# BimberLab/nimble-aligner

Hardware: AMD Instinct MI355X
Metric: reads/sec aligned (whole job), counts bit-exact vs the CPU path (higher is better)
Workload: dtype u64

## Files before the change

include/nimble_hip.h:

```cpp
#ifndef NIMBLE_HIP_H
#define NIMBLE_HIP_H
#include <stdint.h>

#ifdef __cplusplus
extern "C" {
#endif

#define NIMBLE_ABI_VERSION 1

enum {
  NIMBLE_OK = 0,
  NIMBLE_E_INVALID = -1,
  NIMBLE_E_NO_DEVICE = -2,
  NIMBLE_E_HIP = -3,
  NIMBLE_E_NOMEM = -4,
  NIMBLE_E_OVERFLOW = -5,
  NIMBLE_E_INTERNAL = -6
};

enum {
  NIMBLE_R_SCORE_BELOW_THRESHOLD = 0,
  NIMBLE_R_DISCARDED_MULTIPLE_MATCH = 1,
  NIMBLE_R_DISCARDED_NONZERO_MISMATCH = 2,
  NIMBLE_R_NO_MATCH = 3,
  NIMBLE_R_NOT_MATCHING_PAIR = 6,
  NIMBLE_R_SHORT_READ = 8,
  NIMBLE_R_HIGH_ENTROPY = 10,
  NIMBLE_R_SUCCESSFUL_MATCH = 11,
  NIMBLE_R_ABOVE_MISMATCH_THRESHOLD = 14,
  NIMBLE_R_SKIPPED_ALIGN_DUE_TO_UNPAIRED_DUMMY = 15,
  NIMBLE_R_NONE = 16
};

#define NIMBLE_CLASS_NONE 0xFFFFFFFFu

typedef struct nimble_align_params {
  double score_percent;
  uint64_t score_threshold;
  uint32_t num_mismatches;
  uint32_t discard_nonzero_mismatch;
  uint32_t discard_multiple_matches;
  uint32_t require_valid_pair;
  uint32_t min_read_length;
  uint32_t reserved;
} nimble_align_params;

typedef struct nimble_index nimble_index;
typedef struct nimble_ctx nimble_ctx;

int nimble_abi_version(void);
const char *nimble_last_error(void);
int nimble_device_count(int *count);

int nimble_index_build(const uint8_t *seqs, const uint64_t *seq_off, uint32_t n_seqs, int device,
                       nimble_index **out);
void nimble_index_free(nimble_index *);
int nimble_index_stats(const nimble_index *, uint64_t stats[8]);
int nimble_class_get(const nimble_index *, uint32_t class_id, uint32_t *ids, uint32_t cap, uint32_t *len);
int nimble_class_table_read(const nimble_index *, uint32_t first, uint32_t count, uint32_t *len, uint32_t *pool_off);
int nimble_class_pool_read(const nimble_index *, uint32_t pool_off, uint32_t count, uint32_t *ids);

int nimble_flat_index_stats(const uint8_t *seqs, const uint64_t *seq_off, uint32_t n_seqs, uint64_t stats[5]);
int nimble_flat_index_selfcheck(const uint8_t *seqs, const uint64_t *seq_off, uint32_t n_seqs, uint64_t *n_records);

int nimble_ctx_create(nimble_index *, void *stream, nimble_ctx **out);
void nimble_ctx_free(nimble_ctx *);
void *nimble_ctx_stream(nimble_ctx *);

enum {
  NIMBLE_OPT_COUNTERS = 1,
  NIMBLE_OPT_ALIGN_GRID_PCT = 2,
  NIMBLE_OPT_TAIL_ASIDE = 3
};
int nimble_ctx_set_option(nimble_ctx *, int option, int64_t value);

enum { NIMBLE_MEM_HOST = 0, NIMBLE_MEM_DEVICE = 1, NIMBLE_MEM_HOST_PINNED = 2 };

int nimble_call(nimble_ctx *, const nimble_align_params *, const uint8_t *r1, const uint64_t *r1_off,
                const uint8_t *r2, const uint64_t *r2_off, uint64_t n, uint32_t fixed_len, uint32_t max_len,
                int mem);

int nimble_call_words(nimble_ctx *, const nimble_align_params *, const uint64_t *r1_words, const uint32_t *r1_len,
                      uint32_t r1_stride, const uint64_t *r2_words, const uint32_t *r2_len, uint32_t r2_stride, uint64_t n,
                      uint32_t max_len, int mem);

typedef struct nimble_call_extra {
  const uint32_t *segment;
  uint32_t n_segments;
  uint32_t reserved;
  const uint8_t *qual[2];
  double trim_strictness;
  uint64_t trim_target_length;
  const uint8_t *skip[2];
} nimble_call_extra;
int nimble_call_ex(nimble_ctx *, const nimble_align_params *, const uint8_t *r1, const uint64_t *r1_off,
                   const uint8_t *r2, const uint64_t *r2_off, uint64_t n, uint32_t fixed_len, uint32_t max_len,
                   int mem, const nimble_call_extra *extra);
int nimble_histogram_seg(nimble_ctx *, uint32_t *segment, uint32_t *class_r1, uint32_t *class_r2, uint64_t *count,
                         uint32_t *representative, uint64_t cap, uint64_t *n_entries);
int nimble_read_align_len(nimble_ctx *, int mate, uint32_t *align_len, uint64_t n);

typedef struct nimble_packed {
  uint64_t *keys;
  uint32_t *len[2];
  uint64_t *hash;
  uint8_t *pre[2];
  uint32_t key_words;
  uint32_t paired;
} nimble_packed;
uint32_t nimble_key_words(uint32_t max_len, int paired);
int nimble_pack(nimble_ctx *, const nimble_align_params *, const uint8_t *r1, const uint64_t *r1_off,
                const uint8_t *r2, const uint64_t *r2_off, uint64_t n, uint32_t fixed_len, uint32_t max_len, int mem,
                const nimble_packed *out);
int nimble_call_packed(nimble_ctx *, const nimble_align_params *, const nimble_packed *in, uint64_t n,
                       uint32_t max_len);
int nimble_route_records(nimble_ctx *, const nimble_packed *in, uint64_t n, uint32_t world, uint64_t *records,
                         uint64_t *counts);
int nimble_unpack_records(nimble_ctx *, const uint64_t *records, uint64_t n, const nimble_packed *out);
int nimble_call_records(nimble_ctx *, const nimble_align_params *, const uint64_t *records, uint64_t n,
                        uint32_t max_len, int paired);

int nimble_ctx_defer_dedup(nimble_ctx *, uint32_t world, uint64_t *records, uint32_t *perm);
int nimble_route_counts(nimble_ctx *, uint64_t *counts);
int nimble_dedup_records(nimble_ctx *, const uint64_t *records, uint64_t n, uint32_t key_words, uint8_t *verdict);
int nimble_count_verdicts(nimble_ctx *, const uint8_t *verdict);

int nimble_stream_begin(nimble_ctx *, const nimble_align_params *, int paired, uint32_t max_len,
                        uint64_t capacity_hint);
int nimble_stream_append(nimble_ctx *, const uint8_t *r1, const uint64_t *r1_off, const uint8_t *r2,
                         const uint64_t *r2_off, uint64_t n, uint32_t fixed_len, int mem);
int nimble_stream_append_packed(nimble_ctx *, const uint64_t *r1_words, const uint32_t *r1_len, uint32_t r1_stride,
                                const uint64_t *r2_words, const uint32_t *r2_len, uint32_t r2_stride, uint64_t m);
int nimble_stream_end(nimble_ctx *);
int nimble_pinned_alloc(uint64_t bytes, void **out);
void nimble_pinned_free(void *);
int nimble_pinned_register(void *p, uint64_t bytes);
void nimble_pinned_unregister(void *p);

int nimble_histogram(nimble_ctx *, uint32_t *class_r1, uint32_t *class_r2, uint64_t *count, uint64_t cap,
                     uint64_t *n_entries);

int nimble_read_records(nimble_ctx *, int mate, int32_t *reason, int32_t *score, int32_t *mism, uint32_t *cls,
                        uint8_t *counted, uint64_t n);

int nimble_call_counters(nimble_ctx *, uint64_t c[8]);

int nimble_call_timing(nimble_ctx *, float ms[6]);
int nimble_ctx_synchronize(nimble_ctx *);

int nimble_histogram_dense_se(nimble_ctx *, int64_t *counts_dev, uint32_t n_classes);

typedef struct nimble_comm nimble_comm;
int nimble_comm_create(const int *devices, int n, nimble_comm **out);
void nimble_comm_free(nimble_comm *);
int nimble_comm_size(const nimble_comm *);
int nimble_comm_uses_rccl(const nimble_comm *);
void nimble_comm_abort(nimble_comm *);
int nimble_counts_allreduce(nimble_comm *, int rank, int64_t *counts_dev, uint64_t len, void *stream);
int nimble_counts_allreduce_host(nimble_comm *, int rank, int64_t *counts, uint64_t len);
int nimble_records_alltoall(nimble_comm *, int rank, const uint64_t *send, const uint64_t *send_counts,
                            uint32_t rec_words, uint64_t *recv, uint64_t recv_cap, uint64_t *n_recv, void *stream);
int nimble_sharded_begin(nimble_comm *, int rank, nimble_ctx *, const nimble_align_params *, int paired,
                         uint32_t max_len);
int nimble_sharded_append(nimble_comm *, int rank, const uint8_t *r1, const uint64_t *r1_off, const uint8_t *r2,
                          const uint64_t *r2_off, uint64_t n, uint32_t fixed_len, int mem);
int nimble_sharded_append_packed(nimble_comm *, int rank, const uint64_t *r1_words, const uint32_t *r1_len, uint32_t r1_stride,
                                 const uint64_t *r2_words, const uint32_t *r2_len, uint32_t r2_stride, uint64_t n);
int nimble_sharded_end(nimble_comm *, int rank, uint64_t *n_owned);
int nimble_sharded_grow(nimble_comm *, int rank, uint32_t max_len);
int nimble_sharded_abort(nimble_comm *, int rank);
int nimble_steps_begin(nimble_comm *, int rank, nimble_ctx *call0, nimble_ctx *call1, nimble_ctx *util,
                       const nimble_align_params *, int paired, uint32_t max_len);
int nimble_steps_submit(nimble_comm *, int rank, const uint8_t *r1, const uint64_t *r1_off, const uint8_t *r2,
                        const uint64_t *r2_off, uint64_t n, uint32_t fixed_len, int mem, nimble_ctx **launched);
int nimble_steps_flush(nimble_comm *, int rank, nimble_ctx **launched);
int nimble_steps_end(nimble_comm *, int rank);

#ifdef __cplusplus
}
#endif
#endif
```

nimble-aligner_amd/__init__.py:

```python
import ctypes as C
import os

import numpy as np

_HERE = os.path.dirname(os.path.abspath(__file__))
LIB_DIR = os.environ.get("NIMBLE_LIB_DIR") or os.path.join(_HERE, "lib")
HIP_LIB_PATH = os.environ.get("NIMBLE_HIP_LIB") or os.path.join(LIB_DIR, "libnimble_hip.so")
HOST_LIB_PATH = os.path.join(LIB_DIR, "libnimble_host.so")

CLASS_NONE = 0xFFFFFFFF
OPT_COUNTERS, OPT_ALIGN_GRID_PCT, OPT_TAIL_ASIDE = 1, 2, 3
MEM_HOST, MEM_DEVICE = 0, 1

REASONS = {
    0: "ScoreBelowThreshold", 1: "DiscardedMultipleMatch", 2: "DiscardedNonzeroMismatch", 3: "NoMatch",
    6: "NotMatchingPair", 8: "ShortRead", 10: "HighEntropy", 11: "SuccessfulMatch", 14: "AboveMismatchThreshold",
    16: "None",
}


class NimbleError(RuntimeError):
    def __init__(self, code, msg):
        super().__init__("nimble error %d: %s" % (code, msg))
        self.code = code


class AlignParams(C.Structure):
    _fields_ = [
        ("score_percent", C.c_double),
        ("score_threshold", C.c_uint64),
        ("num_mismatches", C.c_uint32),
        ("discard_nonzero_mismatch", C.c_uint32),
        ("discard_multiple_matches", C.c_uint32),
        ("require_valid_pair", C.c_uint32),
        ("min_read_length", C.c_uint32),
        ("reserved", C.c_uint32),
    ]

    @classmethod
    def make(cls, score_percent, score_threshold, num_mismatches=0, discard_nonzero_mismatch=False,
             discard_multiple_matches=False, require_valid_pair=False, min_read_length=40):
        return cls(float(score_percent), int(score_threshold), int(num_mismatches), int(discard_nonzero_mismatch),
                   int(discard_multiple_matches), int(require_valid_pair), int(min_read_length), 0)


class NimblePacked(C.Structure):
    _fields_ = [
        ("keys", C.c_void_p), ("len", C.c_void_p * 2), ("hash", C.c_void_p), ("pre", C.c_void_p * 2),
        ("key_words", C.c_uint32), ("paired", C.c_uint32),
    ]


class CallExtra(C.Structure):
    _fields_ = [("segment", C.c_void_p), ("n_segments", C.c_uint32), ("reserved", C.c_uint32),
                ("qual", C.c_void_p * 2), ("trim_strictness", C.c_double), ("trim_target_length", C.c_uint64),
                ("skip", C.c_void_p * 2)]


class UmiExtra(C.Structure):
    _fields_ = [("segment", C.c_void_p), ("n_segments", C.c_uint32), ("reserved", C.c_uint32),
                ("qual", C.c_void_p * 2), ("skip", C.c_void_p * 2)]


_hip = None

HIP_SYMBOLS = [
    "nimble_abi_version", "nimble_last_error", "nimble_device_count", "nimble_index_build", "nimble_index_free",
    "nimble_index_stats", "nimble_class_get", "nimble_ctx_create", "nimble_ctx_free", "nimble_ctx_synchronize",
    "nimble_call", "nimble_histogram", "nimble_histogram_dense_se", "nimble_read_records", "nimble_call_counters",
    "nimble_call_timing", "nimble_flat_index_stats", "nimble_flat_index_selfcheck", "nimble_ctx_set_option", "nimble_key_words", "nimble_pack",
    "nimble_call_packed", "nimble_call_words", "nimble_ctx_stream", "nimble_stream_begin", "nimble_stream_append", "nimble_stream_append_packed", "nimble_stream_end",
    "nimble_pinned_alloc", "nimble_pinned_free", "nimble_call_ex", "nimble_histogram_seg", "nimble_read_align_len",
    "nimble_route_records", "nimble_unpack_records", "nimble_pinned_register", "nimble_pinned_unregister",
    "nimble_ctx_defer_dedup", "nimble_route_counts", "nimble_dedup_records", "nimble_count_verdicts",
    "nimble_call_records", "nimble_comm_create", "nimble_comm_free", "nimble_comm_size", "nimble_comm_uses_rccl", "nimble_comm_abort",
    "nimble_counts_allreduce", "nimble_counts_allreduce_host", "nimble_records_alltoall", "nimble_sharded_begin",
    "nimble_sharded_append", "nimble_sharded_append_packed", "nimble_sharded_end", "nimble_sharded_grow", "nimble_sharded_abort",
    "nimble_class_table_read", "nimble_class_pool_read", "nimble_steps_begin", "nimble_steps_submit", "nimble_steps_flush", "nimble_steps_end",
]


def hip_lib():
    global _hip
    if _hip is None:
        if not os.path.exists(HIP_LIB_PATH):
            raise ImportError("nimble-aligner_amd: %s is missing; run `python -c 'import __graft_entry__ as g; "
                              "g.build()'` (needs hipcc)" % HIP_LIB_PATH)
        L = C.CDLL(HIP_LIB_PATH)
        vp, i32, u32, u64 = C.c_void_p, C.c_int, C.c_uint32, C.c_uint64
        L.nimble_abi_version.restype = i32
        L.nimble_last_error.restype = C.c_char_p
        L.nimble_device_count.argtypes = [C.POINTER(i32)]
        L.nimble_index_build.argtypes = [vp, vp, u32, i32, C.POINTER(vp)]
        L.nimble_index_free.argtypes = [vp]
        L.nimble_index_free.restype = None
        L.nimble_flat_index_stats.argtypes = [vp, vp, u32, C.POINTER(u64)]
        L.nimble_flat_index_selfcheck.argtypes = [vp, vp, u32, C.POINTER(u64)]
        L.nimble_index_stats.argtypes = [vp, C.POINTER(u64)]
        L.nimble_class_get.argtypes = [vp, u32, vp, u32, C.POINTER(u32)]
        L.nimble_ctx_create.argtypes = [vp, vp, C.POINTER(vp)]
        L.nimble_ctx_free.argtypes = [vp]
        L.nimble_ctx_free.restype = None
        L.nimble_ctx_synchronize.argtypes = [vp]
        L.nimble_ctx_set_option.argtypes = [vp, i32, C.c_int64]
        L.nimble_call.argtypes = [vp, C.POINTER(AlignParams), vp, vp, vp, vp, u64, u32, u32, i32]
        L.nimble_histogram.argtypes = [vp, vp, vp, vp, u64, C.POINTER(u64)]
        L.nimble_histogram_dense_se.argtypes = [vp, vp, u32]
        L.nimble_read_records.argtypes = [vp, i32, vp, vp, vp, vp, vp, u64]
        L.nimble_call_counters.argtypes = [vp, C.POINTER(u64)]
        L.nimble_call_timing.argtypes = [vp, C.POINTER(C.c_float)]
        L.nimble_key_words.argtypes = [u32, i32]
        L.nimble_key_words.restype = u32
        L.nimble_pack.argtypes = [vp, C.POINTER(AlignParams), vp, vp, vp, vp, u64, u32, u32, i32, C.POINTER(NimblePacked)]
        L.nimble_call_packed.argtypes = [vp, C.POINTER(AlignParams), C.POINTER(NimblePacked), u64, u32]
        L.nimble_stream_begin.argtypes = [vp, C.POINTER(AlignParams), i32, u32, u64]
        L.nimble_stream_append.argtypes = [vp, vp, vp, vp, vp, u64, u32, i32]
        L.nimble_stream_append_packed.argtypes = [vp, vp, vp, u32, vp, vp, u32, u64]
        L.nimble_call_words.argtypes = [vp, vp, vp, vp, u32, vp, vp, u32, u64, u32, i32]
        L.nimble_stream_end.argtypes = [vp]
        L.nimble_pinned_alloc.argtypes = [u64, C.POINTER(vp)]
        L.nimble_pinned_free.argtypes = [vp]
        L.nimble_pinned_free.restype = None
        L.nimble_pinned_register.argtypes = [vp, u64]
        L.nimble_pinned_unregister.argtypes = [vp]
        L.nimble_pinned_unregister.restype = None
        L.nimble_call_ex.argtypes = [vp, C.POINTER(AlignParams), vp, vp, vp, vp, u64, u32, u32, i32, C.POINTER(CallExtra)]
        L.nimble_histogram_seg.argtypes = [vp, vp, vp, vp, vp, vp, u64, C.POINTER(u64)]
        L.nimble_read_align_len.argtypes = [vp, i32, vp, u64]
        L.nimble_route_records.argtypes = [vp, C.POINTER(NimblePacked), u64, u32, vp, vp]
        L.nimble_unpack_records.argtypes = [vp, vp, u64, C.POINTER(NimblePacked)]
        L.nimble_ctx_defer_dedup.argtypes = [vp, u32, vp, vp]
        L.nimble_route_counts.argtypes = [vp, vp]
        L.nimble_dedup_records.argtypes = [vp, vp, u64, u32, vp]
        L.nimble_count_verdicts.argtypes = [vp, vp]
        L.nimble_call_records.argtypes = [vp, C.POINTER(AlignParams), vp, u64, u32, i32]
        L.nimble_ctx_stream.argtypes = [vp]
        L.nimble_ctx_stream.restype = vp
        L.nimble_comm_create.argtypes = [C.POINTER(i32), i32, C.POINTER(vp)]
        L.nimble_comm_free.argtypes = [vp]
        L.nimble_comm_free.restype = None
        L.nimble_comm_size.argtypes = [vp]
        L.nimble_comm_uses_rccl.argtypes = [vp]
        L.nimble_comm_abort.argtypes = [vp]
        L.nimble_comm_abort.restype = None
        L.nimble_counts_allreduce.argtypes = [vp, i32, vp, u64, vp]
        L.nimble_counts_allreduce_host.argtypes = [vp, i32, vp, u64]
        L.nimble_records_alltoall.argtypes = [vp, i32, vp, vp, u32, vp, u64, C.POINTER(u64), vp]
        L.nimble_sharded_begin.argtypes = [vp, i32, vp, C.POINTER(AlignParams), i32, u32]
        L.nimble_sharded_append.argtypes = [vp, i32, vp, vp, vp, vp, u64, u32, i32]
        L.nimble_sharded_append_packed.argtypes = [vp, i32, vp, vp, u32, vp, vp, u32, u64]
        L.nimble_sharded_end.argtypes = [vp, i32, C.POINTER(u64)]
        L.nimble_sharded_grow.argtypes = [vp, i32, u32]
        L.nimble_steps_begin.argtypes = [vp, i32, vp, vp, vp, C.POINTER(AlignParams), i32, u32]
        L.nimble_steps_submit.argtypes = [vp, i32, vp, vp, vp, vp, u64, u32, i32, C.POINTER(vp)]
        L.nimble_steps_flush.argtypes = [vp, i32, C.POINTER(vp)]
        L.nimble_steps_end.argtypes = [vp, i32]
        L.nimble_sharded_abort.argtypes = [vp, i32]
        _hip = L
    return _hip


def _check(rc):
    if rc != 0:
        raise NimbleError(rc, hip_lib().nimble_last_error().decode("utf-8", "replace"))


def device_count():
    n = C.c_int(0)
    rc = hip_lib().nimble_device_count(C.byref(n))
    return n.value if rc == 0 else 0


def pack_reads(reads):
    bs = [r.encode() if isinstance(r, str) else bytes(r) for r in reads]
    off = np.zeros(len(bs) + 1, dtype=np.uint64)
    if bs:
        off[1:] = np.cumsum([len(b) for b in bs], dtype=np.uint64)
    buf = np.frombuffer(b"".join(bs), dtype=np.uint8).copy() if bs else np.zeros(0, dtype=np.uint8)
    return buf, off


def _ptr(x):
    if x is None:
        return None
    if isinstance(x, int):
        return x
    if isinstance(x, np.ndarray):
        return x.ctypes.data
    if hasattr(x, "data_ptr"):
        return x.data_ptr()
    raise TypeError(type(x))


def _off(x):
    if x is None or isinstance(x, int):
        return x
    size = x.dtype.itemsize if isinstance(x, np.ndarray) else (x.element_size() if hasattr(x, "element_size") else 8)
    if size != 8:
        raise TypeError("read offsets must be 64-bit integers (n + 1 of them); got elements of %d bytes -- are the mates in "
                        "the place of the offsets?" % size)
    return _ptr(x)


def key_words(max_len, paired):
    return int(hip_lib().nimble_key_words(int(max_len), int(bool(paired))))


def flat_index_stats(sequences):
    buf, off = pack_reads(sequences)
    s = (C.c_uint64 * 5)()
    _check(hip_lib().nimble_flat_index_stats(buf.ctypes.data, off.ctypes.data, len(sequences), s))
    return dict(kmers=s[0], nodes=s[1], classes=s[2], unitig_bases=s[3], class_entries=s[4])


def flat_index_selfcheck(sequences):
    buf, off = pack_reads(sequences)
    n = C.c_uint64()
    _check(hip_lib().nimble_flat_index_selfcheck(buf.ctypes.data, off.ctypes.data, len(sequences), C.byref(n)))
    return int(n.value)


class Index:

    def __init__(self, sequences, device=0):
        buf, off = pack_reads(sequences)
        h = C.c_void_p()
        _check(hip_lib().nimble_index_build(buf.ctypes.data, off.ctypes.data, len(sequences), device, C.byref(h)))
        self.h = h
        self.device = device
        self._class_cache = {}

    def close(self):
        if getattr(self, "h", None):
            hip_lib().nimble_index_free(self.h)
            self.h = None

    def __del__(self):
        try:
            self.close()
        except Exception:
            pass

    def stats(self):
        s = (C.c_uint64 * 8)()
        _check(hip_lib().nimble_index_stats(self.h, s))
        return dict(kmers=s[0], nodes=s[1], classes=s[2], unitig_bases=s[3], class_entries=s[4], hash_slots=s[5],
                    device_bytes=s[6], dynamic_classes=s[7])

    def eq_class(self, class_id):
        class_id = int(class_id)
        got = self._class_cache.get(class_id)
        if got is None:
            n = C.c_uint32(0)
            _check(hip_lib().nimble_class_get(self.h, class_id, None, 0, C.byref(n)))
            a = np.zeros(max(n.value, 1), dtype=np.uint32)
            _check(hip_lib().nimble_class_get(self.h, class_id, a.ctypes.data, n.value, C.byref(n)))
            got = a[:n.value].tolist()
            self._class_cache[class_id] = got
        return got


class Context:

# ... 35 lines not shown
        self._keep = (r1, r1_off, r2, r2_off)
        _check(hip_lib().nimble_call(self.h, C.byref(params), _ptr(r1), _off(r1_off), _ptr(r2), _off(r2_off), n,
                                     fixed_len, max_len, mem))
        self.n = n

    def call_ex(self, params, r1, r1_off=None, r2=None, r2_off=None, n=None, fixed_len=0, max_len=0, mem=MEM_HOST,
                segment=None, n_segments=0, qual=(None, None), skip=(None, None), trim_strictness=0.0,
                trim_target_length=0):
        if r1_off is not None:
            n = int(len(r1_off) - 1) if n is None else n
        if max_len == 0:
            if r1_off is not None and isinstance(r1_off, np.ndarray):
                max_len = int(np.diff(r1_off.astype(np.int64)).max()) if n else 1
                if r2_off is not None:
                    max_len = max(max_len, int(np.diff(r2_off.astype(np.int64)).max()) if n else 1)
            else:
                max_len = fixed_len
        ex = CallExtra()
        ex.segment = _ptr(segment)
        ex.n_segments = n_segments
        for m in range(2):
            ex.qual[m] = _ptr(qual[m])
            ex.skip[m] = _ptr(skip[m])
        ex.trim_strictness = trim_strictness
        ex.trim_target_length = trim_target_length
        self._keep = (r1, r1_off, r2, r2_off, segment, qual, skip)
        _check(hip_lib().nimble_call_ex(self.h, C.byref(params), _ptr(r1), _off(r1_off), _ptr(r2), _off(r2_off), n,
                                        fixed_len, max_len, mem, C.byref(ex)))
        self.n = n

    def histogram_seg(self):
        ne = C.c_uint64()
        _check(hip_lib().nimble_histogram_seg(self.h, None, None, None, None, None, 0, C.byref(ne)))
        k = ne.value
        sg, c1, c2 = (np.zeros(max(k, 1), dtype=np.uint32) for _ in range(3))
        cnt = np.zeros(max(k, 1), dtype=np.uint64)
        rep = np.zeros(max(k, 1), dtype=np.uint32)
        if k:
            _check(hip_lib().nimble_histogram_seg(self.h, sg.ctypes.data, c1.ctypes.data, c2.ctypes.data,
                                                  cnt.ctypes.data, rep.ctypes.data, k, C.byref(ne)))
        return [(int(sg[i]), int(c1[i]), int(c2[i]), int(cnt[i]), int(rep[i])) for i in range(k)]

    def read_align_len(self, mate=0):
        out = np.zeros(max(self.n, 1), dtype=np.uint32)
        _check(hip_lib().nimble_read_align_len(self.h, mate, out.ctypes.data, self.n))
        return out[:self.n]

    def stream_begin(self, params, paired, max_len, capacity_hint=0):
        _check(hip_lib().nimble_stream_begin(self.h, C.byref(params), int(bool(paired)), max_len, capacity_hint))
        self.n = 0

    def stream_append(self, r1, r1_off=None, r2=None, r2_off=None, n=None, fixed_len=0, mem=MEM_HOST):
        if r1_off is not None and n is None:
            n = int(len(r1_off) - 1)
        self._keep = (r1, r1_off, r2, r2_off)
        _check(hip_lib().nimble_stream_append(self.h, _ptr(r1), _off(r1_off), _ptr(r2), _off(r2_off), n, fixed_len,
                                              mem))
        self.n += n

    def call_words(self, params, w1, len1, stride1, w2=None, len2=None, stride2=0, n=None, max_len=0, mem=MEM_HOST):
        if n is None:
            n = int(len(len1))
        self._keep = (w1, len1, w2, len2)
        _check(hip_lib().nimble_call_words(self.h, C.byref(params), _ptr(w1), _ptr(len1), stride1, _ptr(w2), _ptr(len2),
                                           stride2, n, max(max_len, 1), mem))
        self.n = n

    def stream_append_packed(self, w1, len1, stride1, w2=None, len2=None, stride2=0):
        n = int(len(len1))
        self._keep_packed = getattr(self, "_keep_packed", []) + [(w1, len1, w2, len2)]
        _check(hip_lib().nimble_stream_append_packed(self.h, _ptr(w1), _ptr(len1), stride1, _ptr(w2), _ptr(len2), stride2, n))
        self.n += n

    def stream_end(self):
        _check(hip_lib().nimble_stream_end(self.h))
        self._keep_packed = []

    def call_reads(self, params, reads, mates=None):
        b1, o1 = pack_reads(reads)
        if mates is not None:
            b2, o2 = pack_reads(mates)
            return self.call(params, b1, o1, b2, o2)
        return self.call(params, b1, o1)

    def synchronize(self):
        _check(hip_lib().nimble_ctx_synchronize(self.h))

    def set_option(self, option, value):
        _check(hip_lib().nimble_ctx_set_option(self.h, option, int(value)))

    def stream_ptr(self):
        return int(hip_lib().nimble_ctx_stream(self.h) or 0)

    def defer_dedup(self, world, records, perm):
        if not world:
            _check(hip_lib().nimble_ctx_defer_dedup(self.h, 0, None, None))
            return
        assert records.is_contiguous() and perm.is_contiguous() and perm.element_size() == 4
        self._defer_keep = (records, perm)
        _check(hip_lib().nimble_ctx_defer_dedup(self.h, world, C.c_void_p(records.data_ptr()),
                                                C.c_void_p(perm.data_ptr())))

    def route_counts(self, world):
        counts = np.zeros(256, dtype=np.uint64)
        _check(hip_lib().nimble_route_counts(self.h, counts.ctypes.data))
        return [int(c) for c in counts[:world]]

    def dedup_records(self, records, key_words, verdict):
        n = int(records.shape[0])
        assert records.is_contiguous() and verdict.is_contiguous() and verdict.numel() >= n
        assert n == 0 or records.shape[1] == key_words + 2
        self._dedup_keep = (records, verdict)
        _check(hip_lib().nimble_dedup_records(self.h, C.c_void_p(records.data_ptr()), n, key_words,
                                              C.c_void_p(verdict.data_ptr())))

    def count_verdicts(self, verdict):
        self._verdict_keep = verdict
        _check(hip_lib().nimble_count_verdicts(self.h, C.c_void_p(verdict.data_ptr())))

    def set_counters(self, on):
        _check(hip_lib().nimble_ctx_set_option(self.h, 1, int(bool(on))))

    def histogram(self):
        ne = C.c_uint64(0)
        _check(hip_lib().nimble_histogram(self.h, None, None, None, 0, C.byref(ne)))
        k = ne.value
        c1 = np.zeros(max(k, 1), dtype=np.uint32)
        c2 = np.zeros(max(k, 1), dtype=np.uint32)
        cnt = np.zeros(max(k, 1), dtype=np.uint64)
        if k:
            _check(hip_lib().nimble_histogram(self.h, c1.ctypes.data, c2.ctypes.data, cnt.ctypes.data, k,
                                              C.byref(ne)))
        return [(int(c1[i]), int(c2[i]), int(cnt[i])) for i in range(k)]

    def histogram_dense_se(self, counts_dev_ptr, n_classes):
        _check(hip_lib().nimble_histogram_dense_se(self.h, _ptr(counts_dev_ptr), n_classes))

    def read_records(self, mate=0):
        n = self.n
        reason = np.zeros(max(n, 1), dtype=np.int32)
        score = np.zeros(max(n, 1), dtype=np.int32)
        mism = np.zeros(max(n, 1), dtype=np.int32)
        cls = np.zeros(max(n, 1), dtype=np.uint32)
        counted = np.zeros(max(n, 1), dtype=np.uint8)
        _check(hip_lib().nimble_read_records(self.h, mate, reason.ctypes.data, score.ctypes.data, mism.ctypes.data,
                                             cls.ctypes.data, counted.ctypes.data, n))
        return dict(reason=reason[:n], score=score[:n], mismatches=mism[:n], cls=cls[:n], counted=counted[:n])

    def counters(self):
        c = (C.c_uint64 * 8)()
        _check(hip_lib().nimble_call_counters(self.h, c))
        return dict(reads=c[0], unique_keys=c[1], probes=c[2], nodes=c[3], class_entries=c[4], seeded=c[5],
                    prefiltered=c[6], dynamic_classes=c[7])

    def timing(self):
        t = (C.c_float * 6)()
        _check(hip_lib().nimble_call_timing(self.h, t))
        return dict(pack=t[0], align=t[1], intern=t[2], dedup=t[3], count=t[4], total=t[5])


CHEM = {"unstranded": 0, "fiveprime": 1, "threeprime": 2, "none": 3}

HOST_SYMBOLS = [
    "nimble_host_last_error", "nimble_library_load", "nimble_library_parse", "nimble_library_free",
    "nimble_library_get_config", "nimble_library_set_config", "nimble_library_n_rows", "nimble_library_n_cols",
    "nimble_library_group_on", "nimble_library_set_group_on", "nimble_library_sequence_name_idx",
    "nimble_library_sequence_idx", "nimble_library_header", "nimble_library_cell", "nimble_library_push_column", "nimble_library_from_table",
    "nimble_library_build_index", "nimble_library_index", "nimble_library_ctx", "nimble_score_call",
    "nimble_score_call_fastq", "nimble_rows_free", "nimble_rows_count", "nimble_rows_get", "nimble_fastq_process",
    "nimble_write_to_tsv", "nimble_multi_steps", "nimble_host_coerce", "nimble_host_parse_calls", "nimble_host_unmap", "nimble_host_feature_list",
    "nimble_host_reference_sequence_data", "nimble_host_sort_score_vector", "nimble_host_natural_lexical_cmp", "nimble_host_shannon_entropy",
    "nimble_host_revcomp", "nimble_host_maxinfo", "nimble_host_read_fastq", "nimble_host_filter_reason_text",
    "nimble_library_pack", "nimble_score_call_packed", "nimble_score_call_begin", "nimble_score_call_begin_words", "nimble_score_call_end",
    "nimble_library_ctx_slot", "nimble_library_pack_slot", "nimble_score_call_packed_begin",
    "nimble_score_call_records_begin", "nimble_rows_signature", "nimble_rows_counts", "nimble_host_read_fastq_batched", "nimble_host_read_fastq_packed", "nimble_score_call_umis", "nimble_umi_rows_free",
    "nimble_umi_rows_count", "nimble_umi_rows_get", "nimble_umi_rows_reads", "nimble_umi_rows_filter", "nimble_score_stream_begin", "nimble_score_stream_append", "nimble_score_stream_end",
    "nimble_fastq_process_sharded", "nimble_bam_process", "nimble_host_bam_dump", "nimble_host_pack_reads_2bit", "nimble_host_reverse_comp_if_needed",
    "nimble_host_parse_str_as_bool", "nimble_host_pgzip_decompress",
]


class HostConfig(C.Structure):
    _fields_ = [
        ("reference_genome_size", C.c_uint64), ("score_percent", C.c_double), ("score_threshold", C.c_uint64),
        ("num_mismatches", C.c_uint64), ("discard_nonzero_mismatch", C.c_int32),
        ("discard_multiple_matches", C.c_int32), ("score_filter", C.c_int32), ("intersect_level", C.c_int32),
        ("require_valid_pair", C.c_int32), ("strand_filter", C.c_int32), ("discard_multi_hits", C.c_uint64),
        ("max_hits_to_report", C.c_uint64), ("trim_strictness", C.c_double), ("trim_target_length", C.c_uint64),
    ]


_host = None


def host_lib():
    global _host
    if _host is None:
        if not os.path.exists(HOST_LIB_PATH):
            raise ImportError("nimble-aligner_amd: %s is missing; run __graft_entry__.build()" % HOST_LIB_PATH)
        hip_lib()
        L = C.CDLL(HOST_LIB_PATH)
        vp, i32, u32, u64, cp = C.c_void_p, C.c_int, C.c_uint32, C.c_uint64, C.c_char_p
        pp = C.POINTER(C.c_char_p)
        L.nimble_host_last_error.restype = cp
        L.nimble_library_load.argtypes = [cp, i32, C.POINTER(vp)]
        L.nimble_library_parse.argtypes = [cp, i32, C.POINTER(vp)]
        L.nimble_library_free.argtypes = [vp]
        L.nimble_library_free.restype = None
        L.nimble_library_get_config.argtypes = [vp, C.POINTER(HostConfig)]
        L.nimble_library_set_config.argtypes = [vp, C.POINTER(HostConfig)]
        for f in ("n_rows", "n_cols", "group_on", "sequence_name_idx", "sequence_idx"):
            getattr(L, "nimble_library_" + f).argtypes = [vp]
        L.nimble_library_set_group_on.argtypes = [vp, i32]
        L.nimble_library_set_group_on.restype = None
        L.nimble_library_header.argtypes = [vp, i32]
        L.nimble_library_header.restype = cp
        L.nimble_library_cell.argtypes = [vp, i32, i32]
        L.nimble_library_cell.restype = cp
        L.nimble_library_push_column.argtypes = [vp, cp, pp, i32]
        L.nimble_library_from_table.argtypes = [i32, pp, vp, pp, i32, i32, i32, C.POINTER(vp)]
        L.nimble_library_build_index.argtypes = [vp, i32]
        L.nimble_library_index.argtypes = [vp]
        L.nimble_library_index.restype = vp
        L.nimble_library_ctx.argtypes = [vp]
        L.nimble_library_ctx.restype = vp
        L.nimble_score_call.argtypes = [vp, vp, vp, vp, vp, u64, u32, u32, i32, C.POINTER(vp)]
        L.nimble_score_call_fastq.argtypes = [vp, cp, cp, C.POINTER(vp)]
        L.nimble_score_call_begin.argtypes = [vp, i32, vp, vp, vp, vp, u64, u32, u32, i32]
        L.nimble_score_call_begin_words.argtypes = [vp, i32, vp, vp, u32, vp, vp, u32, u64, u32, i32]
        L.nimble_score_call_end.argtypes = [vp, i32, C.POINTER(vp)]
        L.nimble_library_ctx_slot.argtypes = [vp, i32]
        L.nimble_score_stream_begin.argtypes = [vp, i32, u32, u64]
        L.nimble_library_pack_slot.argtypes = [vp, i32, vp, vp, vp, vp, u64, u32, u32, i32, C.POINTER(NimblePacked)]
        L.nimble_score_call_packed_begin.argtypes = [vp, i32, C.POINTER(NimblePacked), u64, u32]
        L.nimble_score_call_records_begin.argtypes = [vp, i32, vp, u64, u32, i32]
        L.nimble_rows_signature.argtypes = [vp]
        L.nimble_rows_signature.restype = u64
        L.nimble_rows_counts.argtypes = [vp, vp]
        L.nimble_rows_counts.restype = None
        L.nimble_score_call_umis.argtypes = [vp, vp, vp, vp, vp, u64, u32, u32, i32, C.POINTER(UmiExtra), i32,
                                             C.POINTER(vp)]
        L.nimble_umi_rows_free.argtypes = [vp]
        L.nimble_umi_rows_free.restype = None
        L.nimble_umi_rows_count.argtypes = [vp]
        L.nimble_umi_rows_count.restype = u64
        L.nimble_umi_rows_get.argtypes = [vp, u64, C.POINTER(u32), C.POINTER(i32), C.POINTER(u32)]
        L.nimble_umi_rows_get.restype = cp
        L.nimble_umi_rows_reads.argtypes = [vp]
        L.nimble_umi_rows_reads.restype = u64
        L.nimble_umi_rows_filter.argtypes = [vp, u64, C.POINTER(i32 * 5)]
        L.nimble_host_read_fastq_batched.argtypes = [cp, u64, C.POINTER(u64), C.POINTER(u64), C.POINTER(u32),
                                                     C.POINTER(u64), C.POINTER(u64)]
        L.nimble_host_read_fastq_packed.argtypes = [cp, u64, C.POINTER(u64), C.POINTER(u64), C.POINTER(u32),
                                                     C.POINTER(u64), C.POINTER(u64)]
        L.nimble_score_stream_append.argtypes = [vp, vp, vp, vp, vp, u64, u32, i32]
        L.nimble_score_stream_end.argtypes = [vp, C.POINTER(vp)]
        L.nimble_library_ctx_slot.restype = vp
        L.nimble_library_pack.argtypes = [vp, vp, vp, vp, vp, u64, u32, u32, i32, C.POINTER(NimblePacked)]
        L.nimble_score_call_packed.argtypes = [vp, C.POINTER(NimblePacked), u64, u32, C.POINTER(vp)]
        L.nimble_rows_free.argtypes = [vp]
        L.nimble_rows_free.restype = None
        L.nimble_rows_count.argtypes = [vp]
        L.nimble_rows_count.restype = u64
        L.nimble_rows_get.argtypes = [vp, u64, C.POINTER(C.c_int32)]
        L.nimble_rows_get.restype = cp
        L.nimble_fastq_process.argtypes = [i32, pp, i32, C.POINTER(vp), pp]
        L.nimble_fastq_process_sharded.argtypes = [i32, pp, vp, C.POINTER(i32), i32, cp]
        L.nimble_multi_steps.argtypes = [C.POINTER(vp), C.POINTER(i32), i32, C.POINTER(vp), C.POINTER(vp), i32, C.c_uint64,
                                         C.c_uint32, i32, i32, i32, C.POINTER(C.c_double), C.POINTER(i32), C.POINTER(vp)]
        L.nimble_bam_process.argtypes = [cp, i32, C.POINTER(vp), pp, i32, i32]
        L.nimble_host_bam_dump.argtypes = [cp, i32, cp]
        L.nimble_host_reverse_comp_if_needed.argtypes = [cp, i32, cp, u64]
        L.nimble_host_pack_reads_2bit.argtypes = [vp, vp, u64, u32, vp, vp]
        L.nimble_host_parse_str_as_bool.argtypes = [cp, C.POINTER(i32)]
        L.nimble_host_pgzip_decompress.argtypes = [cp, i32, cp, C.POINTER(u64)]
        L.nimble_write_to_tsv.argtypes = [vp, cp]
        L.nimble_host_coerce.argtypes = [vp, i32, vp, i32, i32, vp, i32, cp, i32]
        L.nimble_host_parse_calls.argtypes = [vp, cp, cp, i32]
        L.nimble_host_unmap.argtypes = [vp, cp, vp, i32]
        L.nimble_host_feature_list.argtypes = [vp, vp, i32, i32, cp, i32]
        L.nimble_host_reference_sequence_data.argtypes = [vp, cp, i32]
        L.nimble_host_sort_score_vector.argtypes = [cp, i32, vp]
        L.nimble_host_natural_lexical_cmp.argtypes = [cp, cp]
        L.nimble_host_shannon_entropy.argtypes = [cp]
        L.nimble_host_shannon_entropy.restype = C.c_double
        L.nimble_host_revcomp.argtypes = [cp, cp]
        L.nimble_host_maxinfo.argtypes = [cp, i32, u64, C.c_double]
        L.nimble_host_maxinfo.restype = u64
        L.nimble_host_read_fastq.argtypes = [cp, C.POINTER(u64), C.POINTER(u64), C.POINTER(u32)]
        L.nimble_host_filter_reason_text.argtypes = [i32]
        L.nimble_host_filter_reason_text.restype = cp
        _host = L
    return _host


class Panic(RuntimeError):
    """A Rust panic of the reference, surfaced with its message."""


def _hcheck(rc):
    if rc != 0:
        raise Panic(host_lib().nimble_host_last_error().decode("utf-8", "replace"))


def _cstrs(seq):
    arr = (C.c_char_p * len(seq))()
# ... 535 lines not shown
```

nimble-aligner_amd/csrc/capi.cpp:

```cpp
#include <hip/hip_runtime_api.h>
#include <rccl/rccl.h>

#include <algorithm>
#include <condition_variable>
#include <cmath>
#include <cstdlib>
#include <cstring>
#include <mutex>
#include <new>
#include <stdexcept>
#include <string>
#include <vector>

#include "flat_index.h"
#include "kernels.h"

using namespace nimble;

namespace {

thread_local std::string g_err;

int fail(int code, const std::string &msg) {
  g_err = msg;
// ... 1 lines not shown
}

#define HIPCHK(expr)                                                                                   \
  do {                                                                                                 \
    hipError_t e_ = (expr);                                                                            \
    if (e_ != hipSuccess)                                                                              \
      return fail(NIMBLE_E_HIP, std::string(#expr) + ": " + hipGetErrorString(e_));                    \
  } while (0)

#define DRAIN_STALE_HIP_ERROR() (void)hipGetLastError()

uint64_t env_u64(const char *name, uint64_t dflt) {
  const char *v = getenv(name);
  if (!v || !*v) return dflt;
  return strtoull(v, nullptr, 10);
}

uint64_t pow2_at_least(uint64_t x) {
  uint64_t p = 1;
  while (p < x) p <<= 1;
  return p;
}

struct DevBuf {
  void *p = nullptr;
  size_t cap = 0;
  int ensure(size_t bytes, uint64_t *total) {
    if (bytes <= cap) return NIMBLE_OK;
    if (p) {
      (void)hipFree(p);
      if (total) *total -= cap;
      p = nullptr;
      cap = 0;
    }
    size_t want = bytes + 64;
    hipError_t e = hipMalloc(&p, want);
    if (e != hipSuccess) return fail(NIMBLE_E_NOMEM, std::string("hipMalloc failed: ") + hipGetErrorString(e));
    cap = bytes;
    if (total) *total += cap;
    return NIMBLE_OK;
  }
  void release() {
    if (p) (void)hipFree(p);
    p = nullptr;
    cap = 0;
  }
  template <class T>
  T *as() const { return reinterpret_cast<T *>(p); }
};

}

struct nimble_index {
  int device = 0;
  hipStream_t copy_stream = nullptr;
  int n_ctx = 0;
  std::mutex intern_mu;
  hipEvent_t ev_intern = nullptr;
  bool intern_chained = false;
  hipStream_t intern_last = nullptr;
  bool released = false;
  DevIndex dev{};
  DevBuf b_ht, b_bitmap, b_l1, b_mleft, b_rec, b_ledge, b_unitig, b_cls_desc, b_cls_off, b_cls_ids, b_cls_bits, b_intern, b_dyn_state,
      b_srec, b_srec_first, b_srec_base, b_srec_many;
  uint64_t device_bytes = 0;
  uint64_t n_kmers = 0, n_nodes = 0, n_static = 0, unitig_bases = 0, static_entries = 0, ht_slots = 0;
  std::vector<uint32_t> h_col_off, h_col_ids;
  ~nimble_index() {
    if (copy_stream) (void)hipStreamDestroy(copy_stream);
    if (ev_intern) (void)hipEventDestroy(ev_intern);
    for (DevBuf *b : {&b_ht, &b_bitmap, &b_l1, &b_mleft, &b_rec, &b_ledge, &b_unitig, &b_cls_desc, &b_cls_off, &b_cls_ids, &b_cls_bits, &b_intern,
                      &b_dyn_state, &b_srec, &b_srec_first, &b_srec_base, &b_srec_many})
      b->release();
  }
};

struct nimble_ctx {
  nimble_index *ix = nullptr;
  hipStream_t stream = nullptr;
  bool own_stream = false;
  hipStream_t copy_stream = nullptr;
  uint64_t *p_state = nullptr;
  uint32_t *p_dyn = nullptr;
  CallBuffers cb{};
  uint64_t bytes = 0;
  bool streaming = false;
  uint64_t stream_n = 0, stream_cap = 0;
  uint32_t stream_max_len = 0;
  hipStream_t h2d_stream = nullptr;
  DevBuf b_stage[2][2], b_stage_off[2][2];
  hipEvent_t ev_h2d[2] = {}, ev_used[2] = {};
  bool stage_busy[2] = {false, false};
  int stage_k = 0;
  uint64_t align_from = 0;
  bool h2d_pending[2] = {false, false};
  DevBuf b_keys, b_len[2], b_hash, b_pre[2], b_reason[2], b_score[2], b_mism[2], b_cls[2], b_dyn_off[2], b_dyn_len[2],
      b_dyn_hash[2], b_dyn_pos[2], b_slot, b_counted, b_scratch, b_ws, b_dedup, b_hist_keys, b_hist_cnt, b_state;
  DevBuf b_tile_ctr;
  DevBuf b_in[2], b_in_off[2];
  DevBuf b_plog;
  uint32_t plog_max_len = 0;
  DevBuf b_min_cov;
  double min_cov_percent = -1.0;
  uint32_t min_cov_len = 0;
  DevBuf b_out_c1, b_out_c2, b_out_cnt, b_out_seg, b_out_rep;
  struct HostOut {
    void *base = nullptr;
    uint64_t cap = 0;
    uint32_t *c1 = nullptr, *c2 = nullptr, *seg = nullptr, *rep = nullptr;
    uint64_t *cnt = nullptr;
  } hout;
  bool out_pinned = false;
  bool tail_aside = false;
  uint32_t tail_aside_grid = 0;
  DevBuf b_route;
  struct Defer {
    uint32_t world = 0;
    uint32_t world_of_call = 0;
    uint32_t counts_world = 0;
    uint64_t *records = nullptr;
    uint32_t *perm = nullptr;
    const uint8_t *verdict = nullptr;
    bool active = false;
    bool routed = false;
    bool counted = false;
    hipEvent_t ev_route = nullptr;
    uint64_t *p_counts = nullptr;
  } defer;
  DevBuf b_seg, b_alen[2], b_skip[2], b_qual[2], b_trim_ls, b_trim_qp, b_hist_rep, b_hot;
  double trim_strictness = -1.0;
  uint64_t trim_target = ~0ULL;
  std::vector<uint32_t> h_seg, h_rep;
  uint64_t scratch_cap = 0;
  uint64_t hist_slots = 0;
  hipEvent_t ev[7] = {};
  bool have_events = false;
  bool called = false;
  int want_counters = 0;
  int align_grid_pct = 100;
  int stream_cus = 0;
  uint32_t dyn_before = 0, dyn_after = 0;
  nimble_align_params prm{};
  const uint8_t *in_r[2] = {nullptr, nullptr};
  const uint64_t *in_off[2] = {nullptr, nullptr};
  uint32_t in_fixed_len = 0, in_max_len = 0;
  const uint64_t *in_words[2] = {nullptr, nullptr};
  const uint32_t *in_len32[2] = {nullptr, nullptr};
  uint32_t in_stride[2] = {0, 0};
  uint64_t dslots = 0;
  uint64_t dedup_clean_slots = 0;
  bool finished = true;
  bool skip_pack = false;
  bool counted_marked = true;
  int attempt = 0;
  std::vector<uint64_t> h_state = std::vector<uint64_t>(16, 0);
  std::vector<uint32_t> h_c1, h_c2;
  std::vector<uint64_t> h_cnt;
  ~nimble_ctx() {
    for (DevBuf *b : {&b_keys, &b_len[0], &b_len[1], &b_hash, &b_pre[0], &b_pre[1], &b_reason[0], &b_reason[1],
                      &b_score[0], &b_score[1], &b_mism[0], &b_mism[1], &b_cls[0], &b_cls[1], &b_dyn_off[0],
                      &b_dyn_off[1], &b_dyn_len[0], &b_dyn_len[1], &b_dyn_hash[0], &b_dyn_hash[1], &b_dyn_pos[0],
                      &b_dyn_pos[1], &b_slot, &b_counted, &b_scratch, &b_ws, &b_dedup, &b_hist_keys, &b_hist_cnt,
                      &b_state, &b_tile_ctr, &b_in[0], &b_in[1], &b_in_off[0], &b_in_off[1], &b_plog, &b_min_cov, &b_out_c1, &b_out_c2,
                      &b_out_cnt, &b_out_seg, &b_out_rep, &b_seg, &b_alen[0], &b_alen[1], &b_skip[0], &b_skip[1], &b_qual[0],
                      &b_qual[1], &b_route, &b_trim_ls, &b_trim_qp, &b_hist_rep, &b_hot, &b_stage[0][0], &b_stage[0][1], &b_stage[1][0], &b_stage[1][1], &b_stage_off[0][0],
                      &b_stage_off[0][1], &b_stage_off[1][0], &b_stage_off[1][1]})
      b->release();
    if (h2d_stream) {
      (void)hipStreamDestroy(h2d_stream);
      for (int k = 0; k < 2; ++k) {
        (void)hipEventDestroy(ev_h2d[k]);
        (void)hipEventDestroy(ev_used[k]);
      }
    }
    if (have_events)
      for (auto &e : ev) (void)hipEventDestroy(e);
    if (own_stream && stream) (void)hipStreamDestroy(stream);
    if (p_state) (void)hipHostFree(p_state);
    if (hout.base) (void)hipHostFree(hout.base);
    if (p_dyn) (void)hipHostFree(p_dyn);
    if (defer.ev_route) (void)hipEventDestroy(defer.ev_route);
    if (defer.p_counts) (void)hipHostFree(defer.p_counts);
  }
};

namespace {

template <class T>
int upload(DevBuf &b, const std::vector<T> &v, uint64_t *total, size_t min_elems = 0) {
  size_t n = std::max(v.size(), min_elems);
  int rc = b.ensure(std::max<size_t>(n * sizeof(T), 16), total);
  if (rc) return rc;
  if (!v.empty()) HIPCHK(hipMemcpy(b.p, v.data(), v.size() * sizeof(T), hipMemcpyHostToDevice));
  return NIMBLE_OK;
}

int ensure_plog(nimble_ctx *c, uint32_t max_len) {
  if (c->b_plog.p && c->plog_max_len >= max_len) return NIMBLE_OK;
  uint32_t m = std::max<uint32_t>(max_len, 256);
  std::vector<double> t(((size_t)m + 1) * (m + 2) / 2, 0.0);
  for (uint32_t L = 1; L <= m; ++L) {
    double *row = t.data() + ((size_t)L * (L + 1)) / 2;
    for (uint32_t k = 1; k <= L; ++k) {
      double f = (double)k / (double)L;
      row[k] = f * std::log2(f);
    }
  }
  int rc = upload(c->b_plog, t, &c->bytes);
  if (rc) return rc;
  c->plog_max_len = m;
  return NIMBLE_OK;
}

int ensure_trim_tables(nimble_ctx *c, uint64_t target_length, double strictness) {
  if (c->b_trim_ls.p && c->trim_target == target_length && c->trim_strictness == strictness) return NIMBLE_OK;
  const size_t LONGEST_READ = 1000, MAXQUAL = 60;
  std::vector<double> ls(LONGEST_READ), qp(MAXQUAL + 1);
  for (size_t i = 0; i < LONGEST_READ; ++i) {
    const double pow1 = std::exp((double)target_length - (double)i - 1.0);
    ls[i] = std::log(1.0 / (1.0 + pow1)) + std::log((double)(i + 1)) * (1.0 - strictness);
  }
  for (size_t i = 0; i <= MAXQUAL; ++i)
    qp[i] = std::log(1.0 - std::pow(10.0, -((0.5 + (double)i) / 10.0))) * strictness;
  auto norm_ratio = [](const std::vector<double> &a, size_t margin) {
    double mx = std::fabs(a[0]);
    for (size_t i = 1; i < a.size(); ++i) mx = std::max(mx, std::fabs(a[i]));
    return (double)INT64_MAX / (mx * (double)margin);
  };
  auto as_i64 = [](double v) -> int64_t {
    if (std::isnan(v)) return 0;
    if (v >= 9223372036854775807.0) return INT64_MAX;
    if (v <= -9223372036854775808.0) return INT64_MIN;
    return (int64_t)v;
  };
  const double ratio = std::max(norm_ratio(ls, LONGEST_READ * 2), norm_ratio(qp, LONGEST_READ * 2));
  std::vector<int64_t> lsi(LONGEST_READ), qpi(MAXQUAL + 1);
  for (size_t i = 0; i < LONGEST_READ; ++i) lsi[i] = as_i64(ls[i] * ratio);
  for (size_t i = 0; i <= MAXQUAL; ++i) qpi[i] = as_i64(qp[i] * ratio);
  int rc = upload(c->b_trim_ls, lsi, &c->bytes);
  if (!rc) rc = upload(c->b_trim_qp, qpi, &c->bytes);
  if (rc) return rc;
  c->trim_target = target_length;
  c->trim_strictness = strictness;
  return NIMBLE_OK;
}

int ensure_min_cov(nimble_ctx *c, double percent, uint32_t max_len) {
  if (c->b_min_cov.p && c->min_cov_percent == percent && c->min_cov_len >= max_len) return NIMBLE_OK;
  uint32_t m = std::max<uint32_t>(max_len, 256);
  std::vector<uint32_t> t(m + 1, 0xFFFFFFFFu);
  for (uint32_t L = 1; L <= m; ++L) {
    uint32_t lo = 0, hi = 4 * L + 1;
    while (lo < hi) {
      uint32_t mid = lo + (hi - lo) / 2;
      if ((double)mid / (double)L >= percent) hi = mid;
      else lo = mid + 1;
    }
    t[L] = lo <= 4 * L ? lo : 0xFFFFFFFFu;
  }
  t[0] = percent <= 0.0 ? 0u : 0xFFFFFFFFu;
  int rc = upload(c->b_min_cov, t, &c->bytes);
  if (rc) return rc;
  c->min_cov_percent = percent;
  c->min_cov_len = m;
  return NIMBLE_OK;
}

int mark_done(nimble_ctx *c, hipStream_t on = nullptr) {
  hipStream_t s = on ? on : c->stream;
  launch_publish_state(s, c->b_state.as<uint64_t>(), c->p_state);
  HIPCHK(hipGetLastError());
  HIPCHK(hipEventRecord(c->ev[6], s));
  return NIMBLE_OK;
}

int fetch_state(nimble_ctx *c) {
  HIPCHK(hipEventSynchronize(c->ev[6]));
  std::copy(c->p_state, c->p_state + 16, c->h_state.begin());
  return NIMBLE_OK;
}

int ensure_host_out(nimble_ctx *c, uint64_t cap) {
  if (c->hout.cap >= cap) return NIMBLE_OK;
  HIPCHK(hipStreamSynchronize(c->stream));
  if (c->copy_stream) HIPCHK(hipStreamSynchronize(c->copy_stream));
  if (c->hout.base) (void)hipHostFree(c->hout.base);
  c->hout = nimble_ctx::HostOut();
  void *p = nullptr;
  if (hipHostMalloc(&p, cap * 24, hipHostMallocDefault) != hipSuccess)
    return fail(NIMBLE_E_NOMEM, "page-locked result buffer");
  c->hout.base = p;
  c->hout.cap = cap;
  c->hout.cnt = static_cast<uint64_t *>(p);
  c->hout.c1 = reinterpret_cast<uint32_t *>(c->hout.cnt + cap);
  c->hout.c2 = c->hout.c1 + cap;
  c->hout.seg = c->hout.c2 + cap;
  c->hout.rep = c->hout.seg + cap;
  return NIMBLE_OK;
}

int enqueue_compact(nimble_ctx *c, hipStream_t on = nullptr) {
  hipStream_t st = on ? on : c->stream;
  const uint64_t slots = c->hist_slots;
  c->out_pinned = slots <= (1ULL << 22);
  HIPCHK(hipMemsetAsync((uint64_t *)c->b_state.p + 11, 0, 8, st));
  if (c->out_pinned) {
    int rc = ensure_host_out(c, slots);
    if (rc) return rc;
    launch_hist_compact(st, c->cb, c->hout.c1, c->hout.c2, c->hout.cnt, slots, c->hout.seg, c->hout.rep);
    return NIMBLE_OK;
  }
  int rc = c->b_out_c1.ensure(slots * 4, &c->bytes);
  if (!rc) rc = c->b_out_c2.ensure(slots * 4, &c->bytes);
  if (!rc) rc = c->b_out_cnt.ensure(slots * 8, &c->bytes);
  if (!rc) rc = c->b_out_seg.ensure(slots * 4, &c->bytes);
  if (!rc) rc = c->b_out_rep.ensure(slots * 4, &c->bytes);
  if (rc) return rc;
  launch_hist_compact(st, c->cb, c->b_out_c1.as<uint32_t>(), c->b_out_c2.as<uint32_t>(),
                      c->b_out_cnt.as<uint64_t>(), slots, c->b_out_seg.as<uint32_t>(), c->b_out_rep.as<uint32_t>());
  return NIMBLE_OK;
}

int enqueue_count_verdicts(nimble_ctx *c) {
  hipStream_t s = c->stream;
  launch_count_verdicts(s, c->prm, c->cb, c->defer.perm, c->defer.verdict);
  HIPCHK(hipEventRecord(c->ev[4], s));
  HIPCHK(hipEventRecord(c->ev[5], s));
  c->counted_marked = true;
  int rc = enqueue_compact(c);
  if (rc) return rc;
  HIPCHK(hipGetLastError());
  return mark_done(c);
}

int enqueue_route(nimble_ctx *c) {
  const uint32_t world = c->defer.world_of_call;
  const uint64_t cells = (uint64_t)route_grid() * world;
  uint64_t *block_first = c->b_route.as<uint64_t>();
  uint64_t *totals = block_first + cells;
  uint32_t *block_counts = reinterpret_cast<uint32_t *>(totals + 256);
  launch_route(c->stream, c->cb, world, block_counts, block_first, totals, c->defer.records, c->defer.perm);
  HIPCHK(hipGetLastError());
  HIPCHK(hipMemcpyAsync(c->defer.p_counts, totals, world * 8, hipMemcpyDeviceToHost, c->stream));
  HIPCHK(hipMemcpyAsync(c->defer.p_counts + 256, (uint64_t *)c->b_state.p + 14, 8, hipMemcpyDeviceToHost, c->stream));
  HIPCHK(hipEventRecord(c->defer.ev_route, c->stream));
  c->defer.counts_world = world;
  c->defer.routed = true;
  return NIMBLE_OK;
}

int enqueue_intern_round(nimble_ctx *c, int round, hipStream_t on = nullptr) {
  nimble_index *ix = c->ix;
  hipStream_t s = on ? on : c->stream;
  std::lock_guard<std::mutex> lock(ix->intern_mu);
  if (!ix->ev_intern) HIPCHK(hipEventCreateWithFlags(&ix->ev_intern, hipEventDisableTiming));
  if (ix->intern_chained) HIPCHK(hipStreamWaitEvent(s, ix->ev_intern, 0));
  launch_intern_claim(s, ix->dev, c->cb, round);
  launch_intern_verify(s, ix->dev, c->cb);
  HIPCHK(hipEventRecord(ix->ev_intern, s));
  ix->intern_chained = true;
  ix->intern_last = s;
  return NIMBLE_OK;
}

int enqueue_head(nimble_ctx *c) {
  hipStream_t s = c->stream;
  CallBuffers &cb = c->cb;
  if (c->tail_aside) {
    HIPCHK(hipStreamWaitEvent(s, c->ev[6], 0));
    c->tail_aside = false;
  }
  if (c->dedup_clean_slots < c->dslots) HIPCHK(hipMemsetAsync(c->b_dedup.p, 0, c->dslots * 8, s));
  c->dedup_clean_slots = c->defer.active ? c->dslots : 0;
  launch_clear_call(s, cb, !c->skip_pack);
  HIPCHK(hipGetLastError());
  HIPCHK(hipEventRecord(c->ev[0], s));
  return NIMBLE_OK;
}

int enqueue_tail(nimble_ctx *c) {
  hipStream_t s = c->stream;
  CallBuffers &cb = c->cb;
  HIPCHK(hipEventRecord(c->ev[2], s));
  {
    int rc = enqueue_intern_round(c, 0);
    if (rc) return rc;
  }
  HIPCHK(hipEventRecord(c->ev[3], s));
  if (c->defer.active) {
    HIPCHK(hipGetLastError());
    return c->defer.counted ? enqueue_count_verdicts(c) : mark_done(c);
  }
  const uint32_t aside_grid = c->tail_aside_grid;
  hipStream_t t = s;
  c->tail_aside = aside_grid != 0 && c->ix->n_ctx > 1 && !c->streaming && c->copy_stream != nullptr;
  if (c->tail_aside) {
    t = c->copy_stream;
    HIPCHK(hipStreamWaitEvent(t, c->ev[3], 0));
  }
  launch_dedup(t, c->prm, cb, c->tail_aside ? aside_grid : 0u);
  HIPCHK(hipEventRecord(c->ev[4], t));
  if (!cb.fuse_count) launch_count(t, cb);
  c->counted_marked = !cb.fuse_count;
  HIPCHK(hipEventRecord(c->ev[5], t));
  int rc = enqueue_compact(c, t);
  if (rc) return rc;
  HIPCHK(hipGetLastError());
  return mark_done(c, t);
}

int enqueue_call(nimble_ctx *c) {
  hipStream_t s = c->stream;
  CallBuffers &cb = c->cb;
  int rc = enqueue_head(c);
  if (rc) return rc;
  if (!c->skip_pack) {
    if (c->in_words[0])
      launch_pack_words(s, c->in_words[0], c->in_len32[0], c->in_stride[0], c->in_words[1], c->in_len32[1], c->in_stride[1],
                        c->in_max_len, c->prm.min_read_length, c->b_plog.as<double>(), cb);
    else
      launch_pack(s, c->in_r[0], c->in_off[0], c->in_r[1], c->in_off[1], c->in_fixed_len, c->in_max_len,
                  c->prm.min_read_length, c->b_plog.as<double>(), c->plog_max_len, cb);
  }
  HIPCHK(hipEventRecord(c->ev[1], s));
  if (c->defer.active && !c->defer.routed) {
    rc = enqueue_route(c);
    if (rc) return rc;
  }
  launch_align(s, c->ix->dev, c->prm, cb, c->want_counters, c->align_grid_pct, c->stream_cus);
  return enqueue_tail(c);
}

int redo_dedup_count(nimble_ctx *c) {
  hipStream_t s = c->stream;
  if (c->cb.hot) HIPCHK(hipMemsetAsync(c->cb.hot, 0, (size_t)HOT_KEYS * 8, s));
  HIPCHK(hipMemsetAsync(c->b_dedup.p, 0, c->dslots * 8, s));
  HIPCHK(hipMemsetAsync(c->b_hist_keys.p, 0xFF, c->hist_slots * 8, s));
  HIPCHK(hipMemsetAsync(c->b_hist_cnt.p, 0, c->hist_slots * 8, s));
  if (c->cb.hist_rep) HIPCHK(hipMemsetAsync(c->cb.hist_rep, 0, c->hist_slots * 4, s));
  HIPCHK(hipMemsetAsync((uint64_t *)c->b_state.p + 10, 0, 8, s));
  HIPCHK(hipEventRecord(c->ev[3], s));
  if (c->defer.active) return enqueue_count_verdicts(c);
  launch_dedup(s, c->prm, c->cb);
  HIPCHK(hipEventRecord(c->ev[4], s));
  if (!c->cb.fuse_count) launch_count(s, c->cb);
  c->counted_marked = !c->cb.fuse_count;
  HIPCHK(hipEventRecord(c->ev[5], s));
  int rc = enqueue_compact(c);
  return rc ? rc : mark_done(c);
}

int finish_call(nimble_ctx *c) {
  if (c->finished) return NIMBLE_OK;
  if (c->defer.active && !c->defer.counted)
    return fail(NIMBLE_E_INVALID, "the call defers its dedup: nimble_count_verdicts has not been called yet");
  for (;;) {
    int rc = fetch_state(c);
    if (rc) return rc;
    const uint64_t err = c->h_state[10];
    if (c->h_state[14] != 0) {
      HIPCHK(hipMemsetAsync((uint64_t *)c->b_state.p + 14, 0, 8, c->stream));
      HIPCHK(hipStreamSynchronize(c->stream));
      c->finished = true;
      c->h_c1.clear();
      c->h_c2.clear();
      c->h_cnt.clear();
      c->h_seg.clear();
      c->h_rep.clear();
      return fail(NIMBLE_E_INVALID, "offsets not monotone or a read longer than max_len (found on the device)");
    }
    if (err & ERR_SCRATCH) {
      if (c->attempt >= 3 || c->scratch_cap >= 0xFFFFFF00ULL)
        return fail(NIMBLE_E_OVERFLOW, "class scratch pool overflow (raise NIMBLE_SCRATCH_PER_READ)");
      c->attempt++;
      c->scratch_cap = std::min<uint64_t>(c->scratch_cap * 4, 0xFFFFFF00ULL);
      rc = c->b_scratch.ensure(c->scratch_cap * 4, &c->bytes);
      if (rc) return rc;
      c->cb.scratch = c->b_scratch.as<uint32_t>();
      c->cb.scratch_cap = (uint32_t)c->scratch_cap;
      rc = enqueue_call(c);
      if (rc) return rc;
      continue;
    }
    if (err & ERR_CLASS_CAP) return fail(NIMBLE_E_OVERFLOW, "dynamic class table full (raise NIMBLE_DYN_CLASSES)");
    if (err & ERR_IDS_CAP) return fail(NIMBLE_E_OVERFLOW, "dynamic class id pool full (raise NIMBLE_DYN_IDS)");
    if (c->h_state[9] != 0) {
      for (int round = 1; c->h_state[9] != 0; ++round) {
        if (round > 64) return fail(NIMBLE_E_INTERNAL, "class interning did not converge");
        HIPCHK(hipMemsetAsync((uint64_t *)c->b_state.p + 9, 0, 8, c->stream));
        rc = enqueue_intern_round(c, round);
        if (!rc) rc = mark_done(c);
        if (!rc) rc = fetch_state(c);
        if (rc) return rc;
        if (c->h_state[10] & (ERR_CLASS_CAP | ERR_IDS_CAP))
          return fail(NIMBLE_E_OVERFLOW, "dynamic class table full (raise NIMBLE_DYN_CLASSES / NIMBLE_DYN_IDS)");
      }
      rc = redo_dedup_count(c);
      if (rc) return rc;
      continue;
    }
    if (err & ERR_HIST) {
      if (c->hist_slots >= (1ULL << 30)) return fail(NIMBLE_E_OVERFLOW, "histogram table overflow");
      c->hist_slots *= 16;
      rc = c->b_hist_keys.ensure(c->hist_slots * 8, &c->bytes);
      if (!rc) rc = c->b_hist_cnt.ensure(c->hist_slots * 8, &c->bytes);
      if (rc) return rc;
      c->cb.hist_keys = c->b_hist_keys.as<uint64_t>();
      c->cb.hist_cnt = c->b_hist_cnt.as<uint64_t>();
      c->cb.hist_mask = c->hist_slots - 1;
      if (c->cb.hist_rep) {
        rc = c->b_hist_rep.ensure(c->hist_slots * 4, &c->bytes);
        if (rc) return rc;
        c->cb.hist_rep = c->b_hist_rep.as<uint32_t>();
      }
      rc = redo_dedup_count(c);
      if (rc) return rc;
      continue;
    }
    break;
  }
  {
    const uint64_t ne = c->h_state[11];
    c->h_c1.resize(ne);
    c->h_c2.resize(ne);
    c->h_cnt.resize(ne);
    c->h_seg.resize(ne);
    c->h_rep.resize(ne);
    if (ne) {
      std::vector<uint32_t> a(ne), b(ne), sg(ne), rp(ne);
      std::vector<uint64_t> k(ne);
      if (c->out_pinned) {
        std::copy(c->hout.c1, c->hout.c1 + ne, a.begin());
        std::copy(c->hout.c2, c->hout.c2 + ne, b.begin());
        std::copy(c->hout.cnt, c->hout.cnt + ne, k.begin());
        std::copy(c->hout.seg, c->hout.seg + ne, sg.begin());
        std::copy(c->hout.rep, c->hout.rep + ne, rp.begin());
      } else {
        HIPCHK(hipMemcpyAsync(a.data(), c->b_out_c1.p, ne * 4, hipMemcpyDeviceToHost, c->copy_stream));
        HIPCHK(hipMemcpyAsync(b.data(), c->b_out_c2.p, ne * 4, hipMemcpyDeviceToHost, c->copy_stream));
        HIPCHK(hipMemcpyAsync(k.data(), c->b_out_cnt.p, ne * 8, hipMemcpyDeviceToHost, c->copy_stream));
        HIPCHK(hipMemcpyAsync(sg.data(), c->b_out_seg.p, ne * 4, hipMemcpyDeviceToHost, c->copy_stream));
        HIPCHK(hipMemcpyAsync(rp.data(), c->b_out_rep.p, ne * 4, hipMemcpyDeviceToHost, c->copy_stream));
        HIPCHK(hipStreamSynchronize(c->copy_stream));
      }
      std::vector<uint32_t> idx(ne), tmp(ne);
      for (uint64_t i = 0; i < ne; ++i) idx[i] = (uint32_t)i;
      const std::vector<uint32_t> *cols[3] = {&b, &a, &sg};
      std::vector<uint32_t> hist(65536);
      for (int col = 0; col < 3; ++col) {
        const std::vector<uint32_t> &v = *cols[col];
        for (int shift = 0; shift < 32; shift += 16) {
          std::fill(hist.begin(), hist.end(), 0u);
          for (uint64_t i = 0; i < ne; ++i) hist[(v[i] >> shift) & 0xFFFFu]++;
          if (hist[(v[0] >> shift) & 0xFFFFu] == ne) continue;
          uint32_t run = 0;
          for (uint32_t d = 0; d < 65536; ++d) {
            const uint32_t c0 = hist[d];
            hist[d] = run;
            run += c0;
          }
          for (uint64_t i = 0; i < ne; ++i) tmp[hist[(v[idx[i]] >> shift) & 0xFFFFu]++] = idx[i];
          idx.swap(tmp);
        }
      }
      for (uint64_t i = 0; i < ne; ++i) {
        c->h_c1[i] = a[idx[i]];
        c->h_c2[i] = b[idx[i]];
        c->h_cnt[i] = k[idx[i]];
        c->h_seg[i] = sg[idx[i]];
        c->h_rep[i] = rp[idx[i]];
      }
    }
  }
  c->dyn_before = c->p_dyn[0];
  c->finished = true;
  return NIMBLE_OK;
}

}

extern "C" {

int nimble_abi_version(void) { return NIMBLE_ABI_VERSION; }
const char *nimble_last_error(void) { return g_err.c_str(); }

int nimble_device_count(int *count) {
  if (!count) return fail(NIMBLE_E_INVALID, "count is NULL");
  int n = 0;
  hipError_t e = hipGetDeviceCount(&n);
  if (e != hipSuccess) {
    *count = 0;
    return fail(NIMBLE_E_NO_DEVICE, std::string("hipGetDeviceCount: ") + hipGetErrorString(e));
  }
  *count = n;
  return NIMBLE_OK;
// ... 354 lines not shown
          return fail(NIMBLE_E_INVALID, "nimble_call: offsets not monotone or a read longer than max_len");
    }
    int rc = c->b_in[m].ensure(std::max<uint64_t>(bytes, 16), &c->bytes);
    if (rc) return rc;
    const uint64_t lo = off && n ? off[0] : 0;
    if (bytes > lo) HIPCHK(hipMemcpyAsync(c->b_in[m].as<uint8_t>() + lo, src + lo, bytes - lo, hipMemcpyHostToDevice, c->stream));
    c->in_r[m] = c->b_in[m].as<uint8_t>();
    if (off) {
      rc = c->b_in_off[m].ensure((n + 1) * 8, &c->bytes);
      if (rc) return rc;
      HIPCHK(hipMemcpyAsync(c->b_in_off[m].p, off, (n + 1) * 8, hipMemcpyHostToDevice, c->stream));
      c->in_off[m] = c->b_in_off[m].as<uint64_t>();
    }
  }
  return NIMBLE_OK;
}

static int check_read_args(const uint8_t *r1, const uint64_t *r1_off, const uint8_t *r2, const uint64_t *r2_off,
                           uint64_t n, uint32_t fixed_len, uint32_t &max_len, int mem) {
  if (n && !r1) return fail(NIMBLE_E_INVALID, "nimble_call: r1 is NULL");
  if (!r1_off && fixed_len == 0 && n) return fail(NIMBLE_E_INVALID, "nimble_call: neither offsets nor fixed_len given");
  if (r2 && ((r1_off == nullptr) != (r2_off == nullptr)))
    return fail(NIMBLE_E_INVALID, "nimble_call: R1 and R2 must both use offsets or both be fixed length");
  if (n >= 0xFFFFFFF0ULL) return fail(NIMBLE_E_INVALID, "nimble_call: more than 2^32 reads in one call");
  if (!r1_off && fixed_len > max_len) max_len = fixed_len;
  if (max_len == 0) max_len = 1;
  if (max_len > 65535) return fail(NIMBLE_E_INVALID, "nimble_call: max_len above 65535 is not supported");
  if (mem != NIMBLE_MEM_HOST && mem != NIMBLE_MEM_DEVICE && mem != NIMBLE_MEM_HOST_PINNED)
    return fail(NIMBLE_E_INVALID, "nimble_call: bad mem");
  return NIMBLE_OK;
}

static int setup_call(nimble_ctx *c, const nimble_align_params *p, uint64_t n, bool paired, uint32_t max_len,
                      const nimble_packed *ext, const uint64_t *records = nullptr) {
  const int nm = paired ? 2 : 1;
  const uint32_t kw = (max_len * (uint32_t)nm + 31u) / 32u;
  const size_t window_bytes = c->ix->dev.all_local ? 0 : (size_t)c->ix->dev.window_words * 256 * 8;
  if ((size_t)(kw + 1) * 256 * 8 + (size_t)align_lds_cols() * 256 * 4 + 4096 + window_bytes > 160 * 1024)
    return fail(NIMBLE_E_INVALID, window_bytes ? "nimble_call: reads too long for the LDS-resident walk beside this index's row "
                                                 "window (set NIMBLE_LDS_WINDOW_WORDS lower, or NIMBLE_LDS_WINDOW=0)"
                                               : "nimble_call: reads too long for the LDS-resident walk (max_len * mates > ~2400)");
  if (ext && ext->key_words != kw) return fail(NIMBLE_E_INVALID, "packed buffers: key_words does not match max_len");
  CallBuffers &cb = c->cb;
  cb.n = n;
  cb.key_stride = n;
  cb.key_words = kw;
  cb.paired = paired ? 1 : 0;
  cb.fuse_count = paired ? 0u : 1u;
  const size_t nn = std::max<uint64_t>(n, 1);
  int rc = NIMBLE_OK;
  auto need = [&](DevBuf &b, size_t bytes) {
    if (rc == NIMBLE_OK) rc = b.ensure(bytes, &c->bytes);
  };
  if (!ext && !records) {
    need(c->b_keys, nn * kw * 8);
    need(c->b_hash, nn * 8);
  }
  need(c->b_slot, nn * 4);
  need(c->b_counted, nn);
  need(c->b_tile_ctr, (size_t)TILE_COUNTERS * TILE_COUNTER_STRIDE);
  for (int m = 0; m < 2; ++m) {
    if (!records && (!ext || (m == 1 && !ext->len[1]))) {
      need(c->b_len[m], nn * 4);
      need(c->b_pre[m], nn);
    }
    need(c->b_reason[m], nn);
    need(c->b_score[m], nn * 4);
    need(c->b_mism[m], nn * 4);
    need(c->b_cls[m], nn * 4);
    need(c->b_dyn_off[m], nn * 4);
    need(c->b_dyn_len[m], nn * 4);
    need(c->b_dyn_hash[m], nn * 8);
    need(c->b_dyn_pos[m], nn * 4);
  }
  if (c->scratch_cap == 0) c->scratch_cap = std::max<uint64_t>(1ULL << 20, env_u64("NIMBLE_SCRATCH_PER_READ", 4) * n);
  c->scratch_cap = std::min<uint64_t>(std::max<uint64_t>(c->scratch_cap, env_u64("NIMBLE_SCRATCH_PER_READ", 4) * n),
                                      0xFFFFFF00ULL);
  need(c->b_scratch, c->scratch_cap * 4);
  const uint32_t ws_rows = (!c->ix->dev.all_local && max_len > align_lds_cols()) ? max_len - align_lds_cols() : 0;
  need(c->b_ws, std::max<size_t>((size_t)ws_rows * align_ws_lanes() * 4, 16));
  static const uint64_t slots_pct = std::min<uint64_t>(std::max<uint64_t>(env_u64("NIMBLE_DEDUP_SLOTS_PCT", 150), 110), 400);
  const uint64_t dslots = std::min<uint64_t>(std::max<uint64_t>(n * slots_pct / 100, 1024), 0xFFFFFFF0ULL);
  {
    const void *before = c->b_dedup.p;
    need(c->b_dedup, dslots * 8);
    if (c->b_dedup.p != before) c->dedup_clean_slots = 0;
  }
  if (c->hist_slots == 0) c->hist_slots = pow2_at_least(env_u64("NIMBLE_HIST_SLOTS", 1ULL << 18));
  need(c->b_hist_keys, c->hist_slots * 8);
  need(c->b_hist_cnt, c->hist_slots * 8);
  {
    const void *before = c->b_state.p;
    need(c->b_state, 16 * 8);
    if (rc == NIMBLE_OK && c->b_state.p != before) HIPCHK(hipMemsetAsync(c->b_state.p, 0, 16 * 8, c->stream));
  }
  static const bool hot_keys = env_u64("NIMBLE_HOT_KEYS", 1) != 0;
  if (hot_keys) need(c->b_hot, (size_t)HOT_KEYS * 8);
  if (rc != NIMBLE_OK) return rc;
  rc = ensure_plog(c, max_len);
  if (rc != NIMBLE_OK) return rc;
  rc = ensure_min_cov(c, p->score_percent, max_len);
  if (rc != NIMBLE_OK) return rc;

  cb.rec = records;
  cb.rec_words = kw + 2;
  cb.keys = records ? nullptr : ext ? ext->keys : c->b_keys.as<uint64_t>();
  cb.key_hash = records ? nullptr : ext ? ext->hash : c->b_hash.as<uint64_t>();
  cb.slot = c->b_slot.as<uint32_t>();
  cb.counted = c->b_counted.as<uint8_t>();
  for (int m = 0; m < 2; ++m) {
    const bool use_ext = ext && ext->len[m];
    cb.len[m] = records ? nullptr : use_ext ? ext->len[m] : c->b_len[m].as<uint32_t>();
    cb.pre[m] = records ? nullptr : use_ext ? ext->pre[m] : c->b_pre[m].as<uint8_t>();
    cb.reason[m] = c->b_reason[m].as<uint8_t>();
    cb.score[m] = c->b_score[m].as<uint32_t>();
    cb.mism[m] = c->b_mism[m].as<uint32_t>();
    cb.cls[m] = c->b_cls[m].as<uint32_t>();
    cb.dyn_off[m] = c->b_dyn_off[m].as<uint32_t>();
    cb.dyn_len[m] = c->b_dyn_len[m].as<uint32_t>();
    cb.dyn_hash[m] = c->b_dyn_hash[m].as<uint64_t>();
    cb.dyn_pos[m] = c->b_dyn_pos[m].as<uint32_t>();
  }
  for (int m = 0; m < 2; ++m) {
    cb.alen[m] = cb.len[m];
    cb.skip[m] = nullptr;
  }
  cb.seg = nullptr;
  cb.cls_bits = 0;
  cb.hist_rep = nullptr;
  cb.min_cov = c->b_min_cov.as<uint32_t>();
  cb.scratch = c->b_scratch.as<uint32_t>();
  cb.scratch_cap = (uint32_t)c->scratch_cap;
  cb.ws_cols = c->b_ws.as<uint32_t>();
  cb.ws_rows = ws_rows;
  cb.ws_lanes = align_ws_lanes();
  cb.dedup = c->b_dedup.as<uint64_t>();
  cb.hot = c->b_hot.p ? c->b_hot.as<uint64_t>() : nullptr;
  cb.dedup_slots = (uint32_t)dslots;
  cb.hist_keys = c->b_hist_keys.as<uint64_t>();
  cb.hist_cnt = c->b_hist_cnt.as<uint64_t>();
  cb.hist_mask = c->hist_slots - 1;
  cb.state = c->b_state.as<uint64_t>();
  cb.tile_ctr = c->b_tile_ctr.as<uint64_t>();
  c->prm = *p;
  if (c->prm.min_read_length == 0) c->prm.min_read_length = 40;
  c->dslots = dslots;
  return NIMBLE_OK;
}

static int start_call(nimble_ctx *c) {
  HIPCHK(hipMemcpyAsync(c->p_dyn, c->ix->b_dyn_state.p, 4 * sizeof(uint32_t), hipMemcpyDeviceToHost, c->stream));
  c->finished = false;
  c->attempt = 0;
  c->defer.active = c->defer.world != 0;
  c->defer.routed = c->defer.counted = false;
  c->defer.verdict = nullptr;
  if (c->defer.active) {
    if (c->streaming || c->cb.seg || !c->cb.fuse_count) {
      c->defer.active = false;
      c->defer.world = 0;
      return fail(NIMBLE_E_INVALID, "deferred dedup needs a plain call whose classes follow from the key "
                                    "(single-end or fixed-length mates)");
    }
    c->defer.world_of_call = c->defer.world;
    c->defer.world = 0;
  }
  int rc = enqueue_call(c);
  if (rc) return rc;
  c->called = true;
  return NIMBLE_OK;
}

int nimble_call(nimble_ctx *c, const nimble_align_params *p, const uint8_t *r1, const uint64_t *r1_off,
                const uint8_t *r2, const uint64_t *r2_off, uint64_t n, uint32_t fixed_len, uint32_t max_len, int mem) {
  DRAIN_STALE_HIP_ERROR();
  if (!c || !p) return fail(NIMBLE_E_INVALID, "nimble_call: NULL argument");
  int rc = check_read_args(r1, r1_off, r2, r2_off, n, fixed_len, max_len, mem);
  if (rc) return rc;
  HIPCHK(hipSetDevice(c->ix->device));
  rc = stage_inputs(c, r1, r1_off, r2, r2_off, n, fixed_len, max_len, mem);
  if (rc) return rc;
  rc = setup_call(c, p, n, r2 != nullptr, max_len, nullptr);
  if (rc) return rc;
  c->cb.fuse_count = (!r2 || !r1_off) ? 1u : 0u;
  c->skip_pack = false;
  return start_call(c);
}

int nimble_call_words(nimble_ctx *c, const nimble_align_params *p, const uint64_t *r1_words, const uint32_t *r1_len,
                      uint32_t r1_stride, const uint64_t *r2_words, const uint32_t *r2_len, uint32_t r2_stride, uint64_t n,
                      uint32_t max_len, int mem) {
  DRAIN_STALE_HIP_ERROR();
  if (!c || !p) return fail(NIMBLE_E_INVALID, "nimble_call_words: NULL argument");
  if (mem == NIMBLE_MEM_HOST_PINNED) mem = NIMBLE_MEM_HOST;
  if (mem != NIMBLE_MEM_HOST && mem != NIMBLE_MEM_DEVICE) return fail(NIMBLE_E_INVALID, "nimble_call_words: bad mem");
  const bool paired = r2_words != nullptr;
  if ((r2_len != nullptr) != paired) return fail(NIMBLE_E_INVALID, "nimble_call_words: mate words and mate lengths go together");
  if (n && (!r1_words || !r1_len || r1_stride == 0 || (paired && r2_stride == 0)))
    return fail(NIMBLE_E_INVALID, "nimble_call_words: NULL buffer or zero stride");
  if (n >= 0xFFFFFFF0ULL) return fail(NIMBLE_E_INVALID, "nimble_call_words: more than 2^32 reads in one call");
  if (max_len == 0) max_len = 1;
  if (max_len > 65535) return fail(NIMBLE_E_INVALID, "nimble_call_words: max_len above 65535 is not supported");
  HIPCHK(hipSetDevice(c->ix->device));
  c->in_r[0] = c->in_r[1] = nullptr;
  c->in_off[0] = c->in_off[1] = nullptr;
  c->in_fixed_len = 0;
  c->in_max_len = max_len;
  const uint64_t *w[2] = {r1_words, r2_words};
  const uint32_t *l[2] = {r1_len, r2_len};
  const uint32_t st[2] = {r1_stride, r2_stride};
  for (int m = 0; m < (paired ? 2 : 1); ++m) {
    if (mem == NIMBLE_MEM_HOST) {
      const uint64_t cap = std::min<uint64_t>(max_len, 32ULL * st[m]);
      for (uint64_t i = 0; i < n; ++i)
        if (l[m][i] > cap) return fail(NIMBLE_E_INVALID, "nimble_call_words: a read longer than max_len or than its words");
      int rc = c->b_in[m].ensure(std::max<uint64_t>(n * st[m] * 8, 16), &c->bytes);
      if (rc) return rc;
      rc = c->b_in_off[m].ensure(std::max<uint64_t>(n * 4, 16), &c->bytes);
      if (rc) return rc;
      if (n) {
        HIPCHK(hipMemcpyAsync(c->b_in[m].p, w[m], n * st[m] * 8, hipMemcpyHostToDevice, c->stream));
        HIPCHK(hipMemcpyAsync(c->b_in_off[m].p, l[m], n * 4, hipMemcpyHostToDevice, c->stream));
      }
      c->in_words[m] = c->b_in[m].as<uint64_t>();
      c->in_len32[m] = c->b_in_off[m].as<uint32_t>();
    } else {
      c->in_words[m] = w[m];
      c->in_len32[m] = l[m];
    }
    c->in_stride[m] = st[m];
  }
  if (!paired) {
    c->in_words[1] = nullptr;
    c->in_len32[1] = nullptr;
    c->in_stride[1] = 0;
  }
  int rc = setup_call(c, p, n, paired, max_len, nullptr);
  if (rc) return rc;
  c->cb.fuse_count = paired ? 0u : 1u;
  c->skip_pack = false;
  return start_call(c);
}

int nimble_call_ex(nimble_ctx *c, const nimble_align_params *p, const uint8_t *r1, const uint64_t *r1_off,
                   const uint8_t *r2, const uint64_t *r2_off, uint64_t n, uint32_t fixed_len, uint32_t max_len, int mem,
                   const nimble_call_extra *ex) {
  DRAIN_STALE_HIP_ERROR();
  if (!ex) return nimble_call(c, p, r1, r1_off, r2, r2_off, n, fixed_len, max_len, mem);
  if (!c || !p) return fail(NIMBLE_E_INVALID, "nimble_call_ex: NULL argument");
  int rc = check_read_args(r1, r1_off, r2, r2_off, n, fixed_len, max_len, mem);
  if (rc) return rc;
  if (!r2 && (ex->qual[1] || ex->skip[1])) return fail(NIMBLE_E_INVALID, "nimble_call_ex: mate extras without mates");
  HIPCHK(hipSetDevice(c->ix->device));
  rc = stage_inputs(c, r1, r1_off, r2, r2_off, n, fixed_len, max_len, mem);
  if (rc) return rc;
  rc = setup_call(c, p, n, r2 != nullptr, max_len, nullptr);
  if (rc) return rc;
  CallBuffers &cb = c->cb;
  const size_t nn = std::max<uint64_t>(n, 1);
  const bool host = mem == NIMBLE_MEM_HOST;
  auto stage = [&](DevBuf &b, const void *src, size_t bytes, const void *&dev) -> int {
    if (!host) {
      dev = src;
      return NIMBLE_OK;
    }
    int r = b.ensure(std::max<size_t>(bytes, 16), &c->bytes);
    if (r) return r;
    if (bytes) HIPCHK(hipMemcpyAsync(b.p, src, bytes, hipMemcpyHostToDevice, c->stream));
    dev = b.p;
    return NIMBLE_OK;
  };
  if (ex->segment) {
    uint64_t nseg = ex->n_segments;
    if (nseg == 0) {
      if (!host) return fail(NIMBLE_E_INVALID, "nimble_call_ex: n_segments is required for device-resident segment ids");
      for (uint64_t i = 0; i < n; ++i) nseg = std::max<uint64_t>(nseg, (uint64_t)ex->segment[i] + 1);
    }
    uint32_t b = 1;
    while (b < 32 && (1ULL << b) <= (uint64_t)c->ix->dev.cls_cap) ++b;
    if (2 * b >= 64 || nseg >= (1ULL << (64 - 2 * b)))
      return fail(NIMBLE_E_OVERFLOW, "nimble_call_ex: too many segments for one call (split the batch)");
    const void *dev = nullptr;
    rc = stage(c->b_seg, ex->segment, n * 4, dev);
    if (rc) return rc;
    cb.seg = (const uint32_t *)dev;
    cb.cls_bits = b;
  }
  rc = c->b_hist_rep.ensure(c->hist_slots * 4, &c->bytes);
  if (rc) return rc;
  cb.hist_rep = c->b_hist_rep.as<uint32_t>();
  for (int m = 0; m < (r2 ? 2 : 1); ++m)
    if (ex->skip[m]) {
      const void *dev = nullptr;
      rc = stage(c->b_skip[m], ex->skip[m], n, dev);
      if (rc) return rc;
      cb.skip[m] = (const uint8_t *)dev;
    }
  bool trimmed = false;
  for (int m = 0; m < (r2 ? 2 : 1); ++m)
    if (ex->qual[m]) {
      rc = ensure_trim_tables(c, ex->trim_target_length, ex->trim_strictness);
      if (rc) return rc;
      const uint64_t *off_h = m ? r2_off : r1_off;
      const uint64_t bytes = !host ? 0 : (off_h ? off_h[n] : n * (uint64_t)fixed_len);
      const void *dev = nullptr;
      rc = stage(c->b_qual[m], ex->qual[m], bytes, dev);
// ... 143 lines not shown
    HIPCHK(hipMemsetAsync((uint64_t *)c->b_state.p + 14, 0, 8, c->stream));
    return fail(NIMBLE_E_INVALID, "offsets not monotone or a read longer than max_len (found on the device)");
  }
  return NIMBLE_OK;
}

int nimble_dedup_records(nimble_ctx *c, const uint64_t *records, uint64_t n, uint32_t key_words, uint8_t *verdict) {
  DRAIN_STALE_HIP_ERROR();
  if (!c || (n && (!records || !verdict))) return fail(NIMBLE_E_INVALID, "nimble_dedup_records: NULL argument");
  if (n >= 0xFFFFFFF0ULL) return fail(NIMBLE_E_INVALID, "nimble_dedup_records: more than 2^32 records");
  if (key_words == 0) return fail(NIMBLE_E_INVALID, "nimble_dedup_records: key_words is 0");
  if (c->called && !c->finished)
    return fail(NIMBLE_E_INVALID, "nimble_dedup_records: the context holds a call in flight (use another context)");
  HIPCHK(hipSetDevice(c->ix->device));
  const uint64_t slots = std::max<uint64_t>(n + n / 2, 1024);
  int rc = c->b_dedup.ensure(slots * 8, &c->bytes);
  if (rc) return rc;
  c->dedup_clean_slots = 0;
  HIPCHK(hipMemsetAsync(c->b_dedup.p, 0, slots * 8, c->stream));
  launch_dedup_records(c->stream, records, n, key_words, c->b_dedup.as<uint64_t>(), (uint32_t)slots, verdict);
  HIPCHK(hipGetLastError());
  return NIMBLE_OK;
}

int nimble_count_verdicts(nimble_ctx *c, const uint8_t *verdict) {
  DRAIN_STALE_HIP_ERROR();
  if (!c) return fail(NIMBLE_E_INVALID, "nimble_count_verdicts: NULL context");
  if (!c->defer.active || c->finished)
    return fail(NIMBLE_E_INVALID, "nimble_count_verdicts: no call with deferred dedup in flight");
  if (c->defer.counted) return fail(NIMBLE_E_INVALID, "nimble_count_verdicts: already called for this call");
  if (c->cb.n && !verdict) return fail(NIMBLE_E_INVALID, "nimble_count_verdicts: NULL verdicts");
  HIPCHK(hipSetDevice(c->ix->device));
  c->defer.verdict = verdict;
  c->defer.counted = true;
  return enqueue_count_verdicts(c);
}

int nimble_call_packed(nimble_ctx *c, const nimble_align_params *p, const nimble_packed *in, uint64_t n,
                       uint32_t max_len) {
  DRAIN_STALE_HIP_ERROR();
  if (!c || !p || !in) return fail(NIMBLE_E_INVALID, "nimble_call_packed: NULL argument");
  if (n && (!in->keys || !in->hash || !in->len[0] || !in->pre[0]))
    return fail(NIMBLE_E_INVALID, "nimble_call_packed: packed arrays missing");
  if (n >= 0xFFFFFFF0ULL) return fail(NIMBLE_E_INVALID, "nimble_call_packed: more than 2^32 reads in one call");
  if (max_len == 0 || max_len > 65535) return fail(NIMBLE_E_INVALID, "nimble_call_packed: bad max_len");
  HIPCHK(hipSetDevice(c->ix->device));
  int rc = setup_call(c, p, n, in->paired != 0, max_len, in);
  if (rc) return rc;
  c->cb.fuse_count = in->paired ? 0u : 1u;
  c->skip_pack = true;
  return start_call(c);
}


static int stream_grow(nimble_ctx *c, uint64_t newcap) {
  HIPCHK(hipStreamSynchronize(c->stream));
  const uint64_t oldcap = c->stream_cap, used = c->stream_n;
  const uint32_t kw = c->cb.key_words;
  auto fresh = [&](DevBuf &nb, size_t bytes) -> int {
    int rc = nb.ensure(std::max<size_t>(bytes, 16), &c->bytes);
    if (rc) return rc;
    HIPCHK(hipMemset(nb.p, 0, bytes));
    return NIMBLE_OK;
  };
  auto swap_in = [&](DevBuf &b, DevBuf &nb) {
    if (c->bytes >= b.cap) c->bytes -= b.cap;
    b.release();
    b = nb;
    nb.p = nullptr;
    nb.cap = 0;
  };
  {
    DevBuf nk;
    int rc = fresh(nk, newcap * kw * 8);
    if (rc) return rc;
    if (used)
      HIPCHK(hipMemcpy2D(nk.p, newcap * 8, c->b_keys.p, oldcap * 8, used * 8, kw, hipMemcpyDeviceToDevice));
    swap_in(c->b_keys, nk);
  }
  auto regrow = [&](DevBuf &b, size_t elem) -> int {
    DevBuf nb;
    int rc = fresh(nb, newcap * elem);
    if (rc) return rc;
    if (used) HIPCHK(hipMemcpy(nb.p, b.p, used * elem, hipMemcpyDeviceToDevice));
    swap_in(b, nb);
    return NIMBLE_OK;
  };
  int rc = regrow(c->b_hash, 8);
  for (int m = 0; m < 2 && !rc; ++m) {
    rc = regrow(c->b_len[m], 4);
    if (!rc) rc = regrow(c->b_pre[m], 1);
    if (!rc) rc = regrow(c->b_reason[m], 1);
    if (!rc) rc = regrow(c->b_score[m], 4);
    if (!rc) rc = regrow(c->b_mism[m], 4);
    if (!rc) rc = regrow(c->b_cls[m], 4);
    if (!rc) rc = regrow(c->b_dyn_off[m], 4);
    if (!rc) rc = regrow(c->b_dyn_len[m], 4);
    if (!rc) rc = regrow(c->b_dyn_hash[m], 8);
    if (!rc) rc = regrow(c->b_dyn_pos[m], 4);
  }
  if (rc) return rc;
  {
    const uint64_t want = std::min<uint64_t>(std::max<uint64_t>(c->scratch_cap, env_u64("NIMBLE_SCRATCH_PER_READ", 4) * newcap),
                                             0xFFFFFF00ULL);
    if (want > c->scratch_cap) {
      DevBuf nb;
      rc = fresh(nb, want * 4);
      if (rc) return rc;
      HIPCHK(hipMemcpy(nb.p, c->b_scratch.p, c->scratch_cap * 4, hipMemcpyDeviceToDevice));
      swap_in(c->b_scratch, nb);
      c->scratch_cap = want;
    }
  }
  rc = setup_call(c, &c->prm, newcap, c->cb.paired != 0, c->stream_max_len, nullptr);
  if (rc) return rc;
  HIPCHK(hipMemsetAsync(c->b_dedup.p, 0, c->dslots * 8, c->stream));
  c->dedup_clean_slots = 0;
  c->stream_cap = newcap;
  return NIMBLE_OK;
}

int nimble_stream_begin(nimble_ctx *c, const nimble_align_params *p, int paired, uint32_t max_len,
                        uint64_t capacity_hint) {
  DRAIN_STALE_HIP_ERROR();
  if (!c || !p) return fail(NIMBLE_E_INVALID, "nimble_stream_begin: NULL argument");
  if (c->streaming) return fail(NIMBLE_E_INVALID, "nimble_stream_begin: a streamed call is already open");
  if (max_len == 0 || max_len > 65535) return fail(NIMBLE_E_INVALID, "nimble_stream_begin: bad max_len");
  HIPCHK(hipSetDevice(c->ix->device));
  if (!c->h2d_stream) {
    HIPCHK(hipStreamCreateWithFlags(&c->h2d_stream, hipStreamNonBlocking));
    for (int k = 0; k < 2; ++k) {
      HIPCHK(hipEventCreateWithFlags(&c->ev_h2d[k], hipEventDisableTiming));
      HIPCHK(hipEventCreateWithFlags(&c->ev_used[k], hipEventDisableTiming));
    }
  }
  const uint64_t cap = std::min<uint64_t>(std::max<uint64_t>(capacity_hint, 1ULL << 16), 0xFFFFFFEFULL);
  int rc = setup_call(c, p, cap, paired != 0, max_len, nullptr);
  if (rc) return rc;
  c->prm = *p;
  c->stream_cap = cap;
  c->stream_n = 0;
  c->stream_max_len = max_len;
  c->stage_busy[0] = c->stage_busy[1] = false;
  c->stage_k = 0;
  c->h2d_pending[0] = c->h2d_pending[1] = false;
  c->align_from = 0;
  HIPCHK(hipMemcpyAsync(c->p_dyn, c->ix->b_dyn_state.p, 4 * sizeof(uint32_t), hipMemcpyDeviceToHost, c->stream));
  c->defer.active = false;
  c->defer.world = 0;
  c->skip_pack = false;
  rc = enqueue_head(c);
  if (rc) return rc;
  c->streaming = true;
  c->finished = true;
  c->called = false;
  return NIMBLE_OK;
}

static CallBuffers stream_view(const nimble_ctx *c, uint64_t from, uint64_t count) {
  CallBuffers v = c->cb;
  v.n = count;
  v.key_stride = c->stream_cap;
  v.keys += from;
  v.key_hash += from;
  v.slot += from;
  v.counted += from;
  for (int mt = 0; mt < 2; ++mt) {
    v.len[mt] += from;
    v.alen[mt] += from;
    v.pre[mt] += from;
    v.reason[mt] += from;
    v.score[mt] += from;
    v.mism[mt] += from;
    v.cls[mt] += from;
    v.dyn_off[mt] += from;
    v.dyn_len[mt] += from;
    v.dyn_hash[mt] += from;
    v.dyn_pos[mt] += from;
  }
  return v;
}

constexpr uint64_t STREAM_ALIGN_READS = 1u << 18;
static int stream_flush_align(nimble_ctx *c, bool force) {
  const uint64_t pending = c->stream_n - c->align_from;
  if (pending == 0 || (!force && pending < STREAM_ALIGN_READS)) return NIMBLE_OK;
  launch_align(c->stream, c->ix->dev, c->prm, stream_view(c, c->align_from, pending), c->want_counters, c->align_grid_pct, c->stream_cus);
  HIPCHK(hipGetLastError());
  c->align_from = c->stream_n;
  return NIMBLE_OK;
}

int nimble_stream_append(nimble_ctx *c, const uint8_t *r1, const uint64_t *r1_off, const uint8_t *r2,
                         const uint64_t *r2_off, uint64_t m, uint32_t fixed_len, int mem) {
  DRAIN_STALE_HIP_ERROR();
  if (!c) return fail(NIMBLE_E_INVALID, "nimble_stream_append: NULL context");
  if (!c->streaming) return fail(NIMBLE_E_INVALID, "nimble_stream_append: no streamed call is open");
  if ((r2 != nullptr) != (c->cb.paired != 0))
    return fail(NIMBLE_E_INVALID, "nimble_stream_append: mates given for a single-end stream or missing for a paired one");
  uint32_t max_len = c->stream_max_len;
  if (!r1_off && fixed_len > max_len)
    return fail(NIMBLE_E_INVALID, "nimble_stream_append: a read longer than the stream's max_len");
  int rc = check_read_args(r1, r1_off, r2, r2_off, m, fixed_len, max_len, mem);
  if (rc) return rc;
  if (m == 0) return NIMBLE_OK;
  if (c->stream_n + m >= 0xFFFFFFF0ULL) return fail(NIMBLE_E_INVALID, "nimble_stream_append: more than 2^32 reads");
  HIPCHK(hipSetDevice(c->ix->device));
  if (c->stream_n + m > c->stream_cap) {
    rc = stream_grow(c, std::min<uint64_t>(std::max<uint64_t>(2 * c->stream_cap, c->stream_n + m), 0xFFFFFFEFULL));
    if (rc) return rc;
  }
  const uint8_t *in_r[2] = {r1, r2};
  const uint64_t *in_off[2] = {r1_off, r2_off};
  const int k = c->stage_k;
  const bool lazy = mem == NIMBLE_MEM_HOST_PINNED;
  for (int q = 0; q < 2; ++q)
    if (c->h2d_pending[q] && (q == k || !lazy)) {
      HIPCHK(hipEventSynchronize(c->ev_h2d[q]));
      c->h2d_pending[q] = false;
    }
  if (lazy) mem = NIMBLE_MEM_HOST;
  if (mem == NIMBLE_MEM_HOST) {
    if (c->stage_busy[k]) HIPCHK(hipEventSynchronize(c->ev_used[k]));
    for (int mt = 0; mt < (r2 ? 2 : 1); ++mt) {
      const uint64_t *off = in_off[mt];
      const uint64_t bytes = off ? off[m] - off[0] : m * (uint64_t)fixed_len;
      if (off)
        for (uint64_t i = 0; i < m; ++i)
          if (off[i + 1] < off[i] || off[i + 1] - off[i] > max_len)
            return fail(NIMBLE_E_INVALID, "nimble_stream_append: offsets not monotone or a read longer than max_len");
      rc = c->b_stage[k][mt].ensure(std::max<uint64_t>((off ? off[m] : bytes), 16), &c->bytes);
      if (rc) return rc;
      const uint64_t lo = off ? off[0] : 0;
      if (bytes)
        HIPCHK(hipMemcpyAsync(c->b_stage[k][mt].as<uint8_t>() + lo, in_r[mt] + lo, bytes, hipMemcpyHostToDevice,
                              c->h2d_stream));
      in_r[mt] = c->b_stage[k][mt].as<uint8_t>();
      if (off) {
        rc = c->b_stage_off[k][mt].ensure((m + 1) * 8, &c->bytes);
        if (rc) return rc;
        HIPCHK(hipMemcpyAsync(c->b_stage_off[k][mt].p, off, (m + 1) * 8, hipMemcpyHostToDevice, c->h2d_stream));
        in_off[mt] = c->b_stage_off[k][mt].as<uint64_t>();
      }
    }
    HIPCHK(hipEventRecord(c->ev_h2d[k], c->h2d_stream));
    HIPCHK(hipStreamWaitEvent(c->stream, c->ev_h2d[k], 0));
  }
  const CallBuffers v = stream_view(c, c->stream_n, m);
  launch_pack(c->stream, in_r[0], in_off[0], in_r[1], in_off[1], fixed_len, max_len, c->prm.min_read_length,
              c->b_plog.as<double>(), c->plog_max_len, v);
  HIPCHK(hipGetLastError());
  if (mem == NIMBLE_MEM_HOST) {
    HIPCHK(hipEventRecord(c->ev_used[k], c->stream));
    c->stage_busy[k] = true;
    c->stage_k ^= 1;
    if (lazy) c->h2d_pending[k] = true;
    else HIPCHK(hipEventSynchronize(c->ev_h2d[k]));
  }
  c->stream_n += m;
  return stream_flush_align(c, false);
}

int nimble_stream_append_packed(nimble_ctx *c, const uint64_t *r1_words, const uint32_t *r1_len, uint32_t r1_stride,
                                const uint64_t *r2_words, const uint32_t *r2_len, uint32_t r2_stride, uint64_t m) {
  DRAIN_STALE_HIP_ERROR();
  if (!c) return fail(NIMBLE_E_INVALID, "nimble_stream_append_packed: NULL context");
  if (!c->streaming) return fail(NIMBLE_E_INVALID, "nimble_stream_append_packed: no streamed call is open");
  const bool paired = c->cb.paired != 0;
  if ((r2_words != nullptr) != paired || (r2_len != nullptr) != paired)
    return fail(NIMBLE_E_INVALID, "nimble_stream_append_packed: mates given for a single-end stream or missing for a paired one");
  if (m == 0) return NIMBLE_OK;
  if (!r1_words || !r1_len || r1_stride == 0 || (paired && r2_stride == 0))
    return fail(NIMBLE_E_INVALID, "nimble_stream_append_packed: NULL buffer or zero stride");
  const uint32_t max_len = c->stream_max_len;
  for (int mt = 0; mt < (paired ? 2 : 1); ++mt) {
    const uint32_t *len = mt ? r2_len : r1_len;
    const uint64_t cap = std::min<uint64_t>(max_len, 32ULL * (mt ? r2_stride : r1_stride));
    for (uint64_t i = 0; i < m; ++i)
      if (len[i] > cap)
        return fail(NIMBLE_E_INVALID, "nimble_stream_append_packed: a read longer than the stream's max_len or than its words");
  }
  if (c->stream_n + m >= 0xFFFFFFF0ULL) return fail(NIMBLE_E_INVALID, "nimble_stream_append_packed: more than 2^32 reads");
  HIPCHK(hipSetDevice(c->ix->device));
  int rc;
  if (c->stream_n + m > c->stream_cap) {
    rc = stream_grow(c, std::min<uint64_t>(std::max<uint64_t>(2 * c->stream_cap, c->stream_n + m), 0xFFFFFFEFULL));
    if (rc) return rc;
  }
  const int k = c->stage_k;
  if (c->h2d_pending[k]) {
    HIPCHK(hipEventSynchronize(c->ev_h2d[k]));
    c->h2d_pending[k] = false;
  }
  if (c->stage_busy[k]) HIPCHK(hipEventSynchronize(c->ev_used[k]));
  const uint64_t *d_words[2] = {nullptr, nullptr};
  const uint32_t *d_len[2] = {nullptr, nullptr};
  for (int mt = 0; mt < (paired ? 2 : 1); ++mt) {
    const uint64_t wbytes = m * (uint64_t)(mt ? r2_stride : r1_stride) * 8;
    rc = c->b_stage[k][mt].ensure(std::max<uint64_t>(wbytes, 16), &c->bytes);
    if (rc) return rc;
    rc = c->b_stage_off[k][mt].ensure(std::max<uint64_t>(m * 4, 16), &c->bytes);
    if (rc) return rc;
    HIPCHK(hipMemcpyAsync(c->b_stage[k][mt].p, mt ? r2_words : r1_words, wbytes, hipMemcpyHostToDevice, c->h2d_stream));
    HIPCHK(hipMemcpyAsync(c->b_stage_off[k][mt].p, mt ? r2_len : r1_len, m * 4, hipMemcpyHostToDevice, c->h2d_stream));
    d_words[mt] = c->b_stage[k][mt].as<uint64_t>();
    d_len[mt] = c->b_stage_off[k][mt].as<uint32_t>();
// ... 53 lines not shown
int nimble_pinned_register(void *p, uint64_t bytes) {
  if (!p || !bytes) return fail(NIMBLE_E_INVALID, "nimble_pinned_register: NULL argument");
  hipError_t e = hipHostRegister(p, bytes, hipHostRegisterDefault);
  if (e != hipSuccess) {
    (void)hipGetLastError();
    return fail(NIMBLE_E_HIP, std::string("hipHostRegister failed: ") + hipGetErrorString(e));
  }
  return NIMBLE_OK;
}

void nimble_pinned_unregister(void *p) {
  if (p && hipHostUnregister(p) != hipSuccess) (void)hipGetLastError();
}

static int finish_count_stage(nimble_ctx *c) { return finish_call(c); }

int nimble_histogram(nimble_ctx *c, uint32_t *class_r1, uint32_t *class_r2, uint64_t *count, uint64_t cap,
                     uint64_t *n_entries) {
  DRAIN_STALE_HIP_ERROR();
  if (!c || !n_entries) return fail(NIMBLE_E_INVALID, "nimble_histogram: NULL argument");
  if (!c->called) return fail(NIMBLE_E_INVALID, "nimble_histogram: no call has been made on this context");
  HIPCHK(hipSetDevice(c->ix->device));
  int rc = finish_count_stage(c);
  if (rc) return rc;
  const uint64_t ne = c->h_cnt.size();
  *n_entries = ne;
  if (cap == 0 || ne == 0) return NIMBLE_OK;
  if (!class_r1 || !class_r2 || !count) return fail(NIMBLE_E_INVALID, "nimble_histogram: NULL output");
  const uint64_t m = std::min(ne, cap);
  memcpy(class_r1, c->h_c1.data(), m * 4);
  memcpy(class_r2, c->h_c2.data(), m * 4);
  memcpy(count, c->h_cnt.data(), m * 8);
  return NIMBLE_OK;
}

int nimble_histogram_seg(nimble_ctx *c, uint32_t *segment, uint32_t *class_r1, uint32_t *class_r2, uint64_t *count,
                         uint32_t *representative, uint64_t cap, uint64_t *n_entries) {
  DRAIN_STALE_HIP_ERROR();
  if (!c || !n_entries) return fail(NIMBLE_E_INVALID, "nimble_histogram_seg: NULL argument");
  if (!c->called) return fail(NIMBLE_E_INVALID, "nimble_histogram_seg: no call has been made on this context");
  HIPCHK(hipSetDevice(c->ix->device));
  int rc = finish_count_stage(c);
  if (rc) return rc;
  const uint64_t ne = c->h_cnt.size();
  *n_entries = ne;
  if (cap == 0 || ne == 0) return NIMBLE_OK;
  const uint64_t m = std::min(ne, cap);
  if (segment) memcpy(segment, c->h_seg.data(), m * 4);
  if (class_r1) memcpy(class_r1, c->h_c1.data(), m * 4);
  if (class_r2) memcpy(class_r2, c->h_c2.data(), m * 4);
  if (count) memcpy(count, c->h_cnt.data(), m * 8);
  if (representative) memcpy(representative, c->h_rep.data(), m * 4);
  return NIMBLE_OK;
}

int nimble_read_align_len(nimble_ctx *c, int mate, uint32_t *align_len, uint64_t n) {
  DRAIN_STALE_HIP_ERROR();
  if (!c || !align_len) return fail(NIMBLE_E_INVALID, "nimble_read_align_len: NULL argument");
  if (!c->called || n != c->cb.n) return fail(NIMBLE_E_INVALID, "nimble_read_align_len: n does not match the last call");
  if (mate < 0 || mate > 1) return fail(NIMBLE_E_INVALID, "nimble_read_align_len: mate must be 0 or 1");
  HIPCHK(hipSetDevice(c->ix->device));
  int rc = finish_count_stage(c);
  if (rc) return rc;
  if (n == 0) return NIMBLE_OK;
  if (mate == 1 && !c->cb.paired) {
    memset(align_len, 0, n * 4);
    return NIMBLE_OK;
  }
  if (c->cb.rec) return fail(NIMBLE_E_INVALID, "nimble_read_align_len: the call read exchange records (lengths are in them)");
  HIPCHK(hipMemcpy(align_len, c->cb.alen[mate], n * 4, hipMemcpyDeviceToHost));
  return NIMBLE_OK;
}

int nimble_histogram_dense_se(nimble_ctx *c, int64_t *counts_dev, uint32_t n_classes) {
  DRAIN_STALE_HIP_ERROR();
  if (!c || !counts_dev) return fail(NIMBLE_E_INVALID, "nimble_histogram_dense_se: NULL argument");
  if (!c->called) return fail(NIMBLE_E_INVALID, "nimble_histogram_dense_se: no call has been made");
  HIPCHK(hipSetDevice(c->ix->device));
  int rc = finish_count_stage(c);
  if (rc) return rc;
  if (c->cb.cls_bits) return fail(NIMBLE_E_INVALID, "nimble_histogram_dense_se: the last call was segmented");
  HIPCHK(hipMemsetAsync(counts_dev, 0, (size_t)n_classes * 8, c->stream));
  launch_hist_dense_se(c->stream, c->cb, counts_dev, n_classes);
  HIPCHK(hipGetLastError());
  return NIMBLE_OK;
}

int nimble_read_records(nimble_ctx *c, int mate, int32_t *reason, int32_t *score, int32_t *mism, uint32_t *cls,
                        uint8_t *counted, uint64_t n) {
  DRAIN_STALE_HIP_ERROR();
  if (!c) return fail(NIMBLE_E_INVALID, "NULL context");
  if (!c->called || n != c->cb.n) return fail(NIMBLE_E_INVALID, "nimble_read_records: n does not match the last call");
  if (mate < 0 || mate > 1) return fail(NIMBLE_E_INVALID, "nimble_read_records: mate must be 0 or 1");
  HIPCHK(hipSetDevice(c->ix->device));
  int rc = finish_count_stage(c);
  if (rc) return rc;
  if (n == 0) return NIMBLE_OK;
  if (counted && !c->counted_marked) {
    launch_count(c->stream, c->cb);
    HIPCHK(hipStreamSynchronize(c->stream));
    c->counted_marked = true;
  }
  if (mate == 1 && !c->cb.paired) {
    for (uint64_t i = 0; i < n; ++i) {
      if (reason) reason[i] = NIMBLE_R_SUCCESSFUL_MATCH;
      if (score) score[i] = 0;
      if (mism) mism[i] = 0;
      if (cls) cls[i] = NIMBLE_CLASS_NONE;
    }
    if (counted) HIPCHK(hipMemcpy(counted, c->cb.counted, n, hipMemcpyDeviceToHost));
    return NIMBLE_OK;
  }
  if (reason) {
    std::vector<uint8_t> t(n);
    HIPCHK(hipMemcpy(t.data(), c->cb.reason[mate], n, hipMemcpyDeviceToHost));
    for (uint64_t i = 0; i < n; ++i) reason[i] = t[i];
  }
  if (score) HIPCHK(hipMemcpy(score, c->cb.score[mate], n * 4, hipMemcpyDeviceToHost));
  if (mism) HIPCHK(hipMemcpy(mism, c->cb.mism[mate], n * 4, hipMemcpyDeviceToHost));
  if (cls) HIPCHK(hipMemcpy(cls, c->cb.cls[mate], n * 4, hipMemcpyDeviceToHost));
  if (counted) HIPCHK(hipMemcpy(counted, c->cb.counted, n, hipMemcpyDeviceToHost));
  return NIMBLE_OK;
}

extern "C" int nimble_debug_sections(uint64_t out[16], int reset) { return debug_sections(out, reset); }
extern "C" int nimble_debug_stale_error(void) { return (int)hipSetDevice(999); }

extern "C" int nimble_debug_state(nimble_ctx *c, uint64_t out[16]) {
  if (!c || !out || !c->called) return NIMBLE_E_INVALID;
  int rc = finish_count_stage(c);
  if (rc) return rc;
  for (int i = 0; i < 16; ++i) out[i] = c->h_state[i];
  return NIMBLE_OK;
}

int nimble_call_counters(nimble_ctx *c, uint64_t out[8]) {
  DRAIN_STALE_HIP_ERROR();
  if (!c || !out) return fail(NIMBLE_E_INVALID, "NULL argument");
  if (!c->called) return fail(NIMBLE_E_INVALID, "nimble_call_counters: no call has been made");
  HIPCHK(hipSetDevice(c->ix->device));
  int rc = finish_count_stage(c);
  if (rc) return rc;
  uint64_t ne = 0;
  rc = nimble_histogram(c, nullptr, nullptr, nullptr, 0, &ne);
  if (rc) return rc;
  uint64_t uniq = 0;
  for (uint64_t v : c->h_cnt) uniq += v;
  uint32_t dst[4];
  HIPCHK(hipMemcpy(dst, c->ix->b_dyn_state.p, sizeof(dst), hipMemcpyDeviceToHost));
  out[0] = c->cb.n;
  out[1] = uniq;
  for (int i = 2; i <= 6; ++i) out[i] = c->h_state[i];
  out[7] = dst[0] - c->dyn_before;
  return NIMBLE_OK;
}

int nimble_call_timing(nimble_ctx *c, float ms[6]) {
  if (!c || !ms) return fail(NIMBLE_E_INVALID, "NULL argument");
  if (!c->called) return fail(NIMBLE_E_INVALID, "nimble_call_timing: no call has been made");
  HIPCHK(hipSetDevice(c->ix->device));
  HIPCHK(hipEventSynchronize(c->ev[5]));
  for (int i = 0; i < 5; ++i) HIPCHK(hipEventElapsedTime(&ms[i], c->ev[i], c->ev[i + 1]));
  HIPCHK(hipEventElapsedTime(&ms[5], c->ev[0], c->ev[5]));
  return NIMBLE_OK;
}

}

struct nimble_comm {
  int n = 0;
  std::vector<int> devices;
  bool rccl = false;
  std::vector<ncclComm_t> comms;
  std::mutex mu;
  std::condition_variable cv;
  int arrived = 0;
  uint64_t generation = 0;
  std::vector<uint64_t> counts;
  std::vector<const uint64_t *> send_ptr;
  std::vector<void *> vec_ptr;
  std::vector<int> status;
  struct Shard {
    nimble_ctx *ctx = nullptr;
    nimble_align_params prm{};
    int paired = 0;
    uint32_t max_len = 0, rec_words = 0;
    DevBuf send, acc, vec;
    uint64_t n_acc = 0, acc_cap = 0;
    bool open = false;
    struct Steps {
      bool open = false;
      nimble_ctx *call[2] = {nullptr, nullptr}, *util = nullptr;
      hipStream_t xstream = nullptr;
      hipEvent_t ev_routed = nullptr, ev_x[2] = {nullptr, nullptr};
      DevBuf send[2], recv[2];
      uint64_t recv_cap[2] = {0, 0}, n_recv[2] = {0, 0};
      uint64_t *p_counts = nullptr;
      uint64_t b = 0;
      bool pending = false;
    } st;
  };
  std::vector<Shard> shard;
  bool aborted = false;
  void barrier() {
    std::unique_lock<std::mutex> lock(mu);
    if (aborted) return;
    const uint64_t gen = generation;
    if (++arrived == n) {
      arrived = 0;
      ++generation;
      cv.notify_all();
    } else {
      cv.wait(lock, [&] { return generation != gen || aborted; });
    }
  }
  int agree(int rank, int rc) {
    status[rank] = rc;
    barrier();
    int worst = NIMBLE_OK;
    for (int r = 0; r < n; ++r)
      if (status[r] != NIMBLE_OK) worst = status[r];
    barrier();
    {
      std::lock_guard<std::mutex> lock(mu);
      if (aborted && worst == NIMBLE_OK) worst = NIMBLE_E_INTERNAL;
    }
    return worst;
  }
};

#define NCCLCHK(expr)                                                                                  \
  do {                                                                                                 \
    ncclResult_t r_ = (expr);                                                                          \
    if (r_ != ncclSuccess) return fail(NIMBLE_E_HIP, std::string(#expr) + ": " + ncclGetErrorString(r_)); \
  } while (0)

extern "C" {

int nimble_comm_create(const int *devices, int n, nimble_comm **out) {
  if (!devices || !out || n < 1 || n > 256) return fail(NIMBLE_E_INVALID, "nimble_comm_create: bad argument");
  *out = nullptr;
  int ndev = 0;
  if (hipGetDeviceCount(&ndev) != hipSuccess || ndev <= 0)
    return fail(NIMBLE_E_NO_DEVICE, "nimble_comm_create: no HIP device (this library has no CPU path)");
  std::vector<int> sorted(devices, devices + n);
  for (int d : sorted)
    if (d < 0 || d >= ndev) return fail(NIMBLE_E_INVALID, "nimble_comm_create: bad device ordinal");
  std::sort(sorted.begin(), sorted.end());
  const bool distinct = std::adjacent_find(sorted.begin(), sorted.end()) == sorted.end();
  if (!distinct && sorted.front() != sorted.back())
    return fail(NIMBLE_E_INVALID, "nimble_comm_create: ranks must be on distinct devices, or all on one");
  nimble_comm *c = new (std::nothrow) nimble_comm();
  if (!c) return fail(NIMBLE_E_NOMEM, "out of memory");
  c->n = n;
  c->devices.assign(devices, devices + n);
  c->rccl = distinct;
  c->counts.assign((size_t)n * n, 0);
  c->send_ptr.assign(n, nullptr);
  c->vec_ptr.assign(n, nullptr);
  c->status.assign(n, NIMBLE_OK);
  c->shard.resize(n);
  if (c->rccl) {
    c->comms.resize(n);
    ncclResult_t r = ncclCommInitAll(c->comms.data(), n, c->devices.data());
    if (r != ncclSuccess) {
      delete c;
      return fail(NIMBLE_E_HIP, std::string("ncclCommInitAll: ") + ncclGetErrorString(r));
    }
  }
  *out = c;
  return NIMBLE_OK;
}

void nimble_comm_free(nimble_comm *c) {
  if (!c) return;
  for (int r = 0; r < c->n; ++r) {
    (void)hipSetDevice(c->devices[r]);
    c->shard[r].send.release();
    c->shard[r].acc.release();
    c->shard[r].vec.release();
    nimble_comm::Shard::Steps &st = c->shard[r].st;
    for (int k = 0; k < 2; ++k) {
      st.send[k].release();
      st.recv[k].release();
      if (st.ev_x[k]) (void)hipEventDestroy(st.ev_x[k]);
    }
    if (st.ev_routed) (void)hipEventDestroy(st.ev_routed);
    if (st.xstream) (void)hipStreamDestroy(st.xstream);
    if (st.p_counts) (void)hipHostFree(st.p_counts);
  }
  for (ncclComm_t m : c->comms) (void)ncclCommDestroy(m);
  delete c;
}

int nimble_comm_size(const nimble_comm *c) { return c ? c->n : 0; }
void nimble_comm_abort(nimble_comm *c) {
  if (!c) return;
  {
    std::lock_guard<std::mutex> lock(c->mu);
    c->aborted = true;
  }
  c->cv.notify_all();
}
int nimble_comm_uses_rccl(const nimble_comm *c) { return c && c->rccl ? 1 : 0; }

int nimble_counts_allreduce(nimble_comm *c, int rank, int64_t *counts_dev, uint64_t len, void *stream) {
// ... 473 lines not shown
```

nimble-aligner_amd/csrc/kernels.h:

```cpp
#pragma once
#include <hip/hip_runtime_api.h>

#include <cstdint>

#include "../../include/nimble_hip.h"

namespace nimble {

constexpr uint32_t CLS_NONE = 0xFFFFFFFFu;
constexpr uint32_t CLS_PENDING = 0xFFFFFFFEu;
constexpr uint32_t SLOT_NONE = 0xFFFFFFFFu;
constexpr uint32_t HOT_KEYS = 4096;
constexpr uint64_t HIST_EMPTY = ~0ULL;
constexpr uint32_t R_TODO = 255;

struct DevIndex {
  const uint4 *ht;
  uint64_t ht_mask;
  uint32_t ht_log2;
  const uint4 *bitmap;
  uint32_t bm_lines_log2;
  const uint32_t *l1;
  const uint64_t *mleft;
  uint32_t mleft_log2;
  const uint4 *node_rec;
  const uint4 *node_ledge;
  const uint4 *srec;
  const uint32_t *srec_node;
  const uint32_t *srec_base;
  const uint4 *srec_many;
  const uint64_t *unitig;
  uint4 *cls_desc;
  uint32_t *cls_off;
  uint32_t *cls_ids;
  const uint64_t *cls_bits;
  uint32_t all_local;
  uint32_t uniform_windows;
  uint32_t all_bitmaps;
  uint32_t window_words;
  uint32_t n_static;
  uint32_t cls_cap;
  uint32_t ids_cap;
  uint64_t *intern;
  uint64_t intern_mask;
  uint32_t *dyn_state;
};

struct CallBuffers {
  uint64_t n;
  uint64_t key_stride;
  uint32_t key_words;
  uint32_t paired;
  uint64_t *keys;
  const uint64_t *rec;
  uint32_t rec_words;
  uint32_t *len[2];
  uint32_t *alen[2];
  const uint8_t *skip[2];
  const uint32_t *seg;
  uint32_t cls_bits;
  uint32_t *hist_rep;
  uint64_t *key_hash;
  uint8_t *pre[2];
  const uint32_t *min_cov;
  uint8_t *reason[2];
  uint32_t *score[2];
  uint32_t *mism[2];
  uint32_t *cls[2];
  uint32_t *dyn_off[2];
  uint32_t *dyn_len[2];
  uint64_t *dyn_hash[2];
  uint32_t *dyn_pos[2];
  uint32_t *slot;
  uint8_t *counted;
  uint32_t fuse_count;
  uint32_t *scratch;
  uint32_t scratch_cap;
  uint32_t *ws_cols;
  uint32_t ws_rows;
  uint32_t ws_lanes;
  uint64_t *dedup;
  uint64_t *hot;
  uint32_t dedup_slots;
  uint64_t *hist_keys;
  uint64_t *hist_cnt;
  uint64_t hist_mask;
  uint64_t *state;
  uint64_t *tile_ctr;
};
constexpr uint32_t TILE_COUNTERS = 64, TILE_COUNTER_STRIDE = 128;

enum { ERR_SCRATCH = 1, ERR_CLASS_CAP = 2, ERR_IDS_CAP = 4, ERR_HIST = 8 };

void launch_pack(hipStream_t s, const uint8_t *r1, const uint64_t *off1, const uint8_t *r2, const uint64_t *off2,
                 uint32_t fixed_len, uint32_t max_len, uint32_t min_len, const double *plog, uint32_t plog_max_len,
                 const CallBuffers &cb);
void launch_pack_words(hipStream_t s, const uint64_t *w1, const uint32_t *len1, uint32_t stride1, const uint64_t *w2,
                       const uint32_t *len2, uint32_t stride2, uint32_t max_len, uint32_t min_len, const double *plog,
                       const CallBuffers &cb);
void launch_align(hipStream_t s, const DevIndex &ix, const nimble_align_params &p, const CallBuffers &cb,
                  int want_counters, int grid_pct = 100, int n_cus = 0);
void launch_intern_claim(hipStream_t s, const DevIndex &ix, const CallBuffers &cb, int round);
void launch_intern_verify(hipStream_t s, const DevIndex &ix, const CallBuffers &cb);
void launch_dedup(hipStream_t s, const nimble_align_params &p, const CallBuffers &cb, uint32_t grid = 0);
void launch_count(hipStream_t s, const CallBuffers &cb);
void launch_hist_compact(hipStream_t s, const CallBuffers &cb, uint32_t *c1, uint32_t *c2, uint64_t *cnt,
                         uint64_t cap, uint32_t *seg = nullptr, uint32_t *rep = nullptr);
void launch_maxinfo(hipStream_t s, const uint8_t *qual, const uint64_t *off, uint32_t fixed_len, uint64_t n,
                    const int64_t *length_scores, const int64_t *qual_probs, uint32_t *out);
void launch_hist_dense_se(hipStream_t s, const CallBuffers &cb, int64_t *counts, uint32_t n_classes);
uint32_t route_grid();
void launch_route(hipStream_t s, const CallBuffers &cb, uint32_t world, uint32_t *block_counts, uint64_t *block_first,
                  uint64_t *totals, uint64_t *rec, uint32_t *perm = nullptr);
void launch_dedup_records(hipStream_t s, const uint64_t *rec, uint64_t n, uint32_t key_words, uint64_t *table,
                          uint32_t slots, uint8_t *verdict);
void launch_count_verdicts(hipStream_t s, const nimble_align_params &p, const CallBuffers &cb, const uint32_t *perm,
                           const uint8_t *verdict);
void launch_records_unpack(hipStream_t s, const uint64_t *rec, const CallBuffers &cb);
void launch_clear_call(hipStream_t s, const CallBuffers &cb, bool clear_latch);
void launch_publish_state(hipStream_t s, const uint64_t *state, uint64_t *host);
void launch_fill_u64(hipStream_t s, uint64_t *p, uint64_t v, uint64_t n);

int debug_sections(uint64_t out[16], int reset);
uint32_t align_ws_lanes();
uint32_t align_lds_cols();

}
```

nimble-aligner_amd/csrc/kernels.hip:

```cpp
#include <hip/hip_runtime.h>

#include <cstdlib>
#include <map>
#include <mutex>
#include <tuple>

#include "flat_index.h"
#include "kernels.h"

namespace nimble {

namespace {

#ifndef NIMBLE_TENT
#define NIMBLE_TENT 1
#endif
constexpr int PACK_BLOCK = 256;
#ifndef NIMBLE_ALIGN_BLOCK
#define NIMBLE_ALIGN_BLOCK 256
#endif
constexpr int ALIGN_BLOCK = NIMBLE_ALIGN_BLOCK;
constexpr int ALIGN_GRID = 2048 * 256 / ALIGN_BLOCK;
constexpr int LDS_COLS = 4;
constexpr int ALIGN_LDS_EXTRA = 16 + 64 + ALIGN_BLOCK * 2 + ALIGN_BLOCK * 8;
// ... 1155 lines not shown
  }
  if (bitmaps) {
    for (uint32_t row0 = lo; lo <= hi && row0 <= hi; row0 += 64u) {
      uint64_t acc = hi - row0 >= 63u ? ~0ULL : ((1ULL << (hi - row0 + 1u)) - 1ULL);
      for (uint32_t j = 0; j < n_cols && acc; ++j) {
        const uint32_t c = j < LDS_COLS ? lc[j * ALIGN_BLOCK] : ws[(uint64_t)(j - LDS_COLS) * ws_lanes];
        acc &= class_rows64(cls_desc[c], cls_bits, row0);
      }
      for (; acc; acc &= acc - 1) {
        const uint32_t id = row0 + (uint32_t)__ffsll((long long)acc) - 1u;
        if (out) out[count] = id;
        h = class_hash_step(h, id);
        if (count == 0) first_id = id;
        last_id = id;
        if (id - first_id < 64u) gmask |= 1ULL << (id - first_id);
        ++count;
      }
      if (row0 > 0xFFFFFFFFu - 64u) break;
    }
  } else {
    const uint32_t *bids = cls_ids + cls_off[best];
    for (uint32_t t = 0; t < bl; ++t) {
      const uint32_t id = bids[t];
      bool ok = true;
      for (uint32_t j = 0; j < n_cols && ok; ++j) {
        const uint32_t c = j < LDS_COLS ? lc[j * ALIGN_BLOCK] : ws[(uint64_t)(j - LDS_COLS) * ws_lanes];
        if (c == best) continue;
        const uint4 d = cls_desc[c];
        if (desc_is_mask(d)) {
          const uint32_t off = id - d.y;
          ok = id >= d.y && off < 64u && ((desc_mask(d) >> off) & 1ULL);
        } else {
          const uint32_t len = desc_len(d);
          const uint32_t *__restrict__ ids = cls_ids + cls_off[c];
          uint32_t blo = 0, bhi = len;
          while (blo < bhi) {
            uint32_t mid = (blo + bhi) >> 1;
            if (ids[mid] < id) blo = mid + 1;
            else bhi = mid;
          }
          ok = blo < len && ids[blo] == id;
        }
      }
      if (ok) {
        if (out) out[count] = id;
        h = class_hash_step(h, id);
        if (count == 0) first_id = id;
        last_id = id;
        if (id - first_id < 64u) gmask |= 1ULL << (id - first_id);
        ++count;
      }
    }
  }
  IRes r;
  r.count = count;
  r.hash = class_hash_final(h, count);
  if (count && last_id - first_id < 64u) r.hash = class_hash_mask(count, first_id, gmask);
  return r;
}

struct MaskRes {
  bool is_mask;
  uint32_t base;
  uint64_t mask;
};
template <bool WIDE>
__device__ uint32_t finish_class(const DevIndex &ix, const Lane &ln, uint64_t &hash, uint32_t *out, MaskRes &mr) {
  mr.is_mask = !WIDE || ln.all_mask;
  mr.base = 0;
  mr.mask = 0;
  if (WIDE && !ln.all_mask) {
    if (ln.window_ok) {
      uint32_t count = 0, first_id = 0, last_id = 0;
      uint64_t gmask = 0;
      uint64_t h = class_hash_init();
      auto take = [&](uint32_t q, uint64_t word) {
        for (uint64_t m = word; m; m &= m - 1) {
          const uint32_t id = ln.wbase + 64u * q + (uint32_t)__ffsll((long long)m) - 1u;
          if (out) out[count] = id;
          h = class_hash_step(h, id);
          if (count == 0) first_id = id;
          last_id = id;
          if (id - first_id < 64u) gmask |= 1ULL << (id - first_id);
          ++count;
        }
      };
      if (ln.wl) {
        for (uint32_t q = 0; q < ln.wn; ++q) take(q, ln.wl[q * ALIGN_BLOCK]);
      } else {
#pragma unroll
        for (int q = 0; q < 4; ++q) take((uint32_t)q, ln.wacc[q]);
      }
      hash = class_hash_final(h, count);
      if (count && last_id - first_id < 64u) {
        hash = class_hash_mask(count, first_id, gmask);
        mr.is_mask = true;
        mr.base = first_id;
        mr.mask = gmask;
      }
      return count;
    }
    const IRes r = intersect_general(ix.cls_desc, ix.cls_off, ix.cls_ids, ix.cls_bits, ln.lc, ln.ws, ln.ws_lanes, ln.n_cols,
                                     ln.min_col, ln.min_len, out);
    hash = r.hash;
    return r.count;
  }
  const uint64_t acc = ln.acc;
  const uint32_t count = (uint32_t)__popcll(acc);
  if (acc) {
    const uint32_t tz = (uint32_t)__ffsll((long long)acc) - 1u;
    mr.base = ln.fbase + tz;
    mr.mask = acc >> tz;
  }
  hash = class_hash_mask(count, mr.base, mr.mask);
  if (out) {
    uint32_t k = 0;
    for (uint64_t m = acc; m; m &= m - 1) out[k++] = ln.fbase + (uint32_t)__ffsll((long long)m) - 1u;
  }
  return count;
}

__device__ __forceinline__ uint32_t window_count(const Lane &ln) {
  if (ln.wl) {
    uint32_t c = 0;
    for (uint32_t q = 0; q < ln.wn; ++q) c += (uint32_t)__popcll(ln.wl[q * ALIGN_BLOCK]);
    return c;
  }
  return (uint32_t)(__popcll(ln.wacc[0]) + __popcll(ln.wacc[1]) + __popcll(ln.wacc[2]) + __popcll(ln.wacc[3]));
}
__device__ __forceinline__ bool window_equals_class(const DevIndex &ix, const Lane &ln, uint32_t id, uint32_t count) {
  const uint32_t *__restrict__ ids = ix.cls_ids + ix.cls_off[id];
  if (ln.wl) {
    for (uint32_t t = 0; t < count; ++t) {
      const uint32_t off = ids[t] - ln.wbase, q = off >> 6;
      if (q >= ln.wn || !((ln.wl[q * ALIGN_BLOCK] >> (off & 63u)) & 1ULL)) return false;
    }
    return true;
  }
  for (uint32_t t = 0; t < count; ++t) {
    const uint32_t off = ids[t] - ln.wbase;
    const uint32_t q = off >> 6;
    const uint64_t w = q == 0 ? ln.wacc[0] : (q == 1 ? ln.wacc[1] : (q == 2 ? ln.wacc[2] : ln.wacc[3]));
    if (off >= WIDE_ROWS || !((w >> (off & 63u)) & 1ULL)) return false;
  }
  return true;
}

#ifndef NIMBLE_ALIGN_WAVES
#define NIMBLE_ALIGN_WAVES 8
#endif
#ifndef NIMBLE_RESULT_STAGED
#define NIMBLE_RESULT_STAGED 1
#endif
template <bool PAIRED, bool COUNTERS, bool WIDE, int MODE>
#ifndef NIMBLE_FAST_WAVES
#define NIMBLE_FAST_WAVES 7
#endif
#ifndef NIMBLE_WIDE_WAVES
#define NIMBLE_WIDE_WAVES ((NIMBLE_ALIGN_WAVES * 3) / 4)
#endif
#ifndef NIMBLE_FAST_WAVES_PAIRED
#define NIMBLE_FAST_WAVES_PAIRED (NIMBLE_FAST_WAVES - 2)
#endif
__global__ __launch_bounds__(ALIGN_BLOCK, MODE == 1 ? (COUNTERS ? NIMBLE_FAST_WAVES / 2 : (PAIRED ? NIMBLE_FAST_WAVES_PAIRED : NIMBLE_FAST_WAVES))
                                                    : (WIDE ? NIMBLE_WIDE_WAVES : NIMBLE_ALIGN_WAVES)) void k_align(DevIndex ix, nimble_align_params p,
                                                                           CallBuffers cb) {
  static_assert(!(WIDE && MODE == 1), "the fast walk is for indexes whose classes all have the mask form");
  constexpr int want_counters = COUNTERS ? 1 : 0;
  extern __shared__ __attribute__((aligned(16))) uint64_t lds64[];
  const uint32_t tid = threadIdx.x;
  const uint32_t kw = cb.key_words;
  uint64_t *col = lds64 + tid;
  constexpr int nm = PAIRED ? 2 : 1;
  const uint32_t krows = kw + 1u > (uint32_t)nm + 1u ? kw + 1u : (uint32_t)nm + 1u;
  constexpr int LIST_COLS = MODE == 1 ? 0 : LDS_COLS;
  Lane ln;
  ln.rd = col;
  ln.lc = reinterpret_cast<uint32_t *>(lds64 + (size_t)krows * ALIGN_BLOCK) + tid;
  ln.ws_lanes = cb.ws_lanes;
  ln.ws_rows = cb.ws_rows;
  ln.ws = cb.ws_cols + ((uint64_t)blockIdx.x * ALIGN_BLOCK + tid);
  ln.want_counters = want_counters;
  ln.probes = ln.nodes = 0;
  ln.entries = 0;
  ln.overflow = 0;
  ln.n_cols = ln.last_col = ln.walk_nodes = 0;
  ln.acc = 0;
  ln.fbase = ln.min_len = ln.min_col = 0;
  ln.last_rec = 0;
  ln.all_mask = true;
  ln.keep_list = WIDE;
  ln.window_ok = false;
  ln.use_window = WIDE && ix.all_bitmaps != 0;
  ln.uniform = !WIDE && ix.uniform_windows != 0;
  ln.wbase = 0;
  ln.wacc[0] = ln.wacc[1] = ln.wacc[2] = ln.wacc[3] = 0;
  ln.wcap = WIDE ? ix.window_words : 0u;
  ln.wn = 0;
  ln.wl = ln.wcap ? reinterpret_cast<uint64_t *>(reinterpret_cast<uint8_t *>(reinterpret_cast<uint32_t *>(lds64 + (size_t)krows * ALIGN_BLOCK) + LIST_COLS * ALIGN_BLOCK) + ALIGN_LDS_EXTRA) + tid
                  : nullptr;
  ln.cls_bits = ix.cls_bits;
  uint32_t c_seeded = 0, c_pre = 0;
  const uint64_t n = cb.n;
  const uint64_t n_tiles = (n + ALIGN_BLOCK - 1) / ALIGN_BLOCK;
  unsigned long long *const tile_counter = (unsigned long long *)cb.tile_ctr;

  uint8_t *extra = reinterpret_cast<uint8_t *>(reinterpret_cast<uint32_t *>(lds64 + (size_t)krows * ALIGN_BLOCK) +
                                               LIST_COLS * ALIGN_BLOCK);
  unsigned long long &s_tile = *reinterpret_cast<unsigned long long *>(extra);
  uint32_t *s_cnt = reinterpret_cast<uint32_t *>(extra + 16);
  uint64_t *s_seed = reinterpret_cast<uint64_t *>(extra + 16 + 64);
  uint16_t *s_perm = reinterpret_cast<uint16_t *>(extra + 16 + 64 + ALIGN_BLOCK * 8);
  uint64_t *s_meta = reinterpret_cast<uint64_t *>(extra + 16 + 64 + ALIGN_BLOCK * 8 + ALIGN_BLOCK * 2);
  uint64_t prev_tile = ~0ULL;
  const unsigned long long tiles_per_counter = (n_tiles + TILE_COUNTERS - 1) / TILE_COUNTERS;
  unsigned long long &s_next = *reinterpret_cast<unsigned long long *>(extra + 8);
  constexpr unsigned long long NO_TILE = (1ULL << 48) - 1ULL;
  auto fetch_tile = [&](bool first_call) {
    uint32_t my_counter = first_call ? blockIdx.x % TILE_COUNTERS : (uint32_t)(s_next >> 48) & 0xFFu;
    uint32_t counters_tried = first_call ? 0u : (uint32_t)(s_next >> 56);
    unsigned long long got = NO_TILE;
    while (counters_tried < TILE_COUNTERS) {
      const unsigned long long first = (unsigned long long)my_counter * tiles_per_counter;
      if (first < n_tiles) {
        const unsigned long long t = atomicAdd(tile_counter + (size_t)my_counter * (TILE_COUNTER_STRIDE / 8), 1ULL);
        if (t < tiles_per_counter && first + t < n_tiles) {
          got = first + t;
          break;
        }
      }
      my_counter = my_counter + 1 == TILE_COUNTERS ? 0u : my_counter + 1;
      ++counters_tried;
    }
    s_next = got | ((unsigned long long)my_counter << 48) | ((unsigned long long)counters_tried << 56);
  };
  static_assert(TILE_COUNTERS <= 128, "the counter's number and the count of used-up ones share 16 bits of a word");
#ifndef NIMBLE_STATIC_TILES
  if (tid == 0) fetch_tile(true);
#endif
  PROF_DECL
  for (;;) {
    PROF(7)
    __syncthreads();
    PROF(0)
#if NIMBLE_RESULT_STAGED
    if (prev_tile != ~0ULL) {
      const uint64_t rp = prev_tile * ALIGN_BLOCK + tid;
#ifndef NIMBLE_SKEL_NOSTORE
      if (rp < n) {
        const uint64_t rs = col[nm * ALIGN_BLOCK];
#pragma unroll
        for (int m = 0; m < nm; ++m) {
          const uint64_t v = col[m * ALIGN_BLOCK];
          st_stream(&cb.reason[m][rp], (uint8_t)(rs >> (8 * m)));
          st_stream(&cb.score[m][rp], (uint32_t)(v & 0xFFFFu));
          st_stream(&cb.mism[m][rp], (uint32_t)((v >> 16) & 0xFFFFu));
          st_stream(&cb.cls[m][rp], (uint32_t)(v >> 32));
        }
      }
#endif
    }
#endif
    if (tid == 0) {
#ifdef NIMBLE_STATIC_TILES
      s_tile = prev_tile == ~0ULL ? (unsigned long long)blockIdx.x : prev_tile + gridDim.x;
      (void)tile_counter;
#else
      s_tile = (s_next & NO_TILE) == NO_TILE ? n_tiles : (s_next & NO_TILE);
#endif
    }
    __syncthreads();
    const uint64_t tile = s_tile;
    PROF(0)
    if (tile >= n_tiles) break;
    WCOUNT(0)
#ifndef NIMBLE_STATIC_TILES
    if (tid == 0) fetch_tile(false);
#endif
    prev_tile = tile;
    const uint64_t r_own = tile * ALIGN_BLOCK + tid;
    uint32_t kind = 2;
    uint64_t seedv = ~0ULL;
    uint64_t metav = 0;
    if (r_own < n) {
      const uint32_t pre0 = rd_pre(cb, 0, r_own);
      const uint32_t k0 = rd_len(cb, 0, r_own);
      const uint32_t l1 = nm == 2 ? rd_len(cb, 1, r_own) : 0u;
      const uint32_t l0 = rd_alen(cb, 0, r_own);
      metav = (uint64_t)l0 | ((uint64_t)k0 << 32) | ((uint64_t)pre0 << 48);
      if (nm == 2) metav |= ((uint64_t)rd_alen(cb, 1, r_own) << 16) | ((uint64_t)rd_pre(cb, 1, r_own) << 56);
      constexpr uint32_t KCH = 8;
      const uint64_t *row = cb.rec ? cb.rec + r_own * cb.rec_words : nullptr;
      for (uint32_t w0 = 0; w0 < kw; w0 += KCH) {
        uint64_t v[KCH];
#pragma unroll
        for (uint32_t j = 0; j < KCH; ++j)
#ifdef NIMBLE_SKEL_NOKEYS
          v[j] = 0ULL;
#else
          v[j] = w0 + j < kw ? (row ? row[w0 + j] : ld_stream(cb.keys + (uint64_t)(w0 + j) * cb.key_stride + r_own)) : 0ULL;
#endif
        const uint32_t nw = (k0 + l1 + 31u) >> 5;
#pragma unroll
        for (uint32_t j = 0; j < KCH; ++j)
          if (w0 + j < kw) col[(w0 + j) * ALIGN_BLOCK] = w0 + j < nw ? v[j] : 0ULL;
      }
      col[kw * ALIGN_BLOCK] = 0ULL;
      if (pre0 == R_TODO && l0 >= KMER) {
        uint32_t nd = 0, of = 0;
        ln.rd = col;
        if (probe_direct(ix, ln, 0u, 0u, nd, of, MODE != 1)) {
          kind = 1;
          seedv = u64of(of, nd);
        } else {
          kind = 0;
        }
      }
    }
    PROF(1)
    s_seed[tid] = seedv;
    if (MODE == 1) s_meta[tid] = metav;
    {
      const uint64_t b0 = __ballot(kind == 0), b1 = __ballot(kind == 1);
      const uint32_t wv = tid >> 6, lane = tid & 63u;
      if (lane == 0) {
        s_cnt[wv * 2] = (uint32_t)__popcll(b0);
        s_cnt[wv * 2 + 1] = (uint32_t)__popcll(b1);
      }
      __syncthreads();
      uint32_t tot0 = 0, tot1 = 0, pre0 = 0, pre1 = 0;
#pragma unroll
      for (uint32_t w = 0; w < ALIGN_BLOCK / 64; ++w) {
        const uint32_t c0 = s_cnt[w * 2], c1 = s_cnt[w * 2 + 1];
        if (w < wv) { pre0 += c0; pre1 += c1; }
        tot0 += c0;
        tot1 += c1;
      }
      const uint64_t below = (1ULL << lane) - 1ULL;
      const uint32_t r0 = (uint32_t)__popcll(b0 & below), r1 = (uint32_t)__popcll(b1 & below);
      const uint32_t r2 = lane - r0 - r1;
      const uint32_t pre2 = wv * 64u - pre0 - pre1;
      const uint32_t pos = kind == 0 ? pre0 + r0 : (kind == 1 ? tot0 + pre1 + r1 : tot0 + tot1 + pre2 + r2);
      s_perm[pos] = (uint16_t)tid;
      __syncthreads();
    }
    PROF(2)
    const uint32_t slot = s_perm[tid];
    const uint64_t r = tile * ALIGN_BLOCK + slot;
    const bool active = r < n;
    ln.rd = lds64 + slot;
    const uint64_t pre_seed = s_seed[slot];
    uint32_t L[2] = {0, 0};
    uint32_t mate1_at = 0;
    uint64_t meta = 0;
    if (MODE == 1) {
      meta = s_meta[slot];
    } else if (active) {
      meta = (uint64_t)rd_alen(cb, 0, r) | ((uint64_t)rd_pre(cb, 0, r) << 48);
      if (nm == 2)
        meta |= ((uint64_t)rd_alen(cb, 1, r) << 16) | ((uint64_t)rd_len(cb, 0, r) << 32) | ((uint64_t)rd_pre(cb, 1, r) << 56);
    }
    if (active) {
      L[0] = (uint32_t)meta & 0xFFFFu;
      if (nm == 2) {
        L[1] = (uint32_t)(meta >> 16) & 0xFFFFu;
        mate1_at = (uint32_t)(meta >> 32) & 0xFFFFu;
      }
    }
    bool any_walk = false;
    uint64_t res_v[2] = {0, 0}, res_r = 0;
    for (int m = 0; m < nm; ++m) {
      uint32_t reason = NIMBLE_R_NONE, score = 0, mm = 0, cls = CLS_NONE;
      uint32_t need = 0, best_col = 0, best_len = 0;
      uint64_t dhash = 0;
      MaskRes mres;
      mres.is_mask = false;
      mres.base = 0;
      mres.mask = 0;
      if (active) {
        const uint32_t pre = (uint32_t)(meta >> (48 + 8 * m)) & 0xFFu;
        if (pre != R_TODO) {
          reason = pre;
          if (m == 0) c_pre++;
        } else {
          uint32_t cov = 0, mis = 0;
          const uint32_t pre_state = m == 0 ? (pre_seed != ~0ULL ? 2u : 1u) : 0u;
          PROF(3)
          bool some;
          if (MODE == 1) {
            const uint32_t base0 = m ? mate1_at : 0u;
            some = p.num_mismatches == 0 ? walk_fast<true>(ix, ln, base0, L[m], 0u, pre_state, pre_seed, cov, mis PROF_PASS)
                                         : walk_fast<false>(ix, ln, base0, L[m], p.num_mismatches, pre_state, pre_seed, cov, mis PROF_PASS);
          } else {
            some = walk(ix, ln, m ? mate1_at : 0u, L[m], p.num_mismatches, cov, mis, pre_state, pre_seed PROF_PASS);
          }
          PROF(3)
          if (!some) {
            reason = NIMBLE_R_NO_MATCH;
          } else {
            any_walk = true;
            score = cov;
            mm = mis;
            uint32_t count;
            best_col = ln.min_col;
            best_len = ln.min_len;
            const bool windowed = WIDE && !ln.all_mask && ln.window_ok;
            count = MODE == 1 ? (uint32_t)__popcll(ln.acc)
                              : (windowed ? window_count(ln) : finish_class<WIDE>(ix, ln, dhash, nullptr, mres));
            if (p.discard_nonzero_mismatch && mis != 0) {
              reason = NIMBLE_R_DISCARDED_NONZERO_MISMATCH;
            } else if ((uint64_t)cov >= p.score_threshold && cov >= cb.min_cov[L[m]] && count != 0) {
              if (p.discard_multiple_matches && count > 1) reason = NIMBLE_R_DISCARDED_MULTIPLE_MATCH;
              else if (mis > p.num_mismatches) reason = NIMBLE_R_ABOVE_MISMATCH_THRESHOLD;
              else {
                reason = NIMBLE_R_SUCCESSFUL_MATCH;
                if (count == best_len) {
                  cls = best_col;
                } else {
                  cls = CLS_PENDING;
                  if (MODE == 1) {
                    WCOUNT(13)
                    ln.fbase = ix.srec_base[ln.last_rec];
                    finish_class<WIDE>(ix, ln, dhash, nullptr, mres);
                  }
                  if (windowed) finish_class<WIDE>(ix, ln, dhash, nullptr, mres);
                  if (mres.is_mask || windowed) {
                    const uint32_t tag = intern_tag(dhash);
                    uint64_t pos = dhash & ix.intern_mask;
                    for (;;) {
                      const uint64_t slot = ix.intern[pos];
                      WCOUNT(14)
                      if (slot == 0) break;
                      const uint32_t id = (uint32_t)slot;
                      if ((uint32_t)(slot >> 32) == tag && id != INTERN_PENDING && id < ix.cls_cap) {
                        const uint4 d = ix.cls_desc[id];
                        if (mres.is_mask) {
                          if (d.x == (count | CLS_MASK_FLAG) && d.y == mres.base && desc_mask(d) == mres.mask) {
                            cls = id;
                            break;
                          }
                        } else if (d.x == count && window_equals_class(ix, ln, id, count)) {
                          cls = id;
                          break;
                        }
                      }
                      pos = (pos + 1) & ix.intern_mask;
                    }
                  }
                  if (cls == CLS_PENDING) need = count;
                }
              }
            } else {
              reason = NIMBLE_R_SCORE_BELOW_THRESHOLD;
            }
          }
        }
      }
      PROF(6)
      uint32_t total;
      uint32_t ofs = wave_excl_scan(need, total);
      unsigned long long base = 0;
      if (total) {
        if ((tid & 63u) == 0) base = atomicAdd((unsigned long long *)&cb.state[8], (unsigned long long)total);
        base = __shfl(base, 0, 64);
      }
      if (need) {
        if (base + ofs + need <= (unsigned long long)cb.scratch_cap) {
          uint64_t hh;
          MaskRes m2;
          finish_class<WIDE>(ix, ln, hh, cb.scratch + base + ofs, m2);
          cb.dyn_off[m][r] = (uint32_t)base + ofs;
          cb.dyn_len[m][r] = need;
          cb.dyn_hash[m][r] = dhash;
        } else {
          atomicOr((unsigned long long *)&cb.state[10], (unsigned long long)ERR_SCRATCH);
          cls = CLS_NONE;
        }
      }
#if NIMBLE_RESULT_STAGED
      res_v[m] = (uint64_t)score | ((uint64_t)mm << 16) | ((uint64_t)cls << 32);
      res_r |= (uint64_t)reason << (8 * m);
#else
      if (active) {
        st_stream(&cb.reason[m][r], (uint8_t)reason);
        st_stream(&cb.score[m][r], score);
        st_stream(&cb.mism[m][r], mm);
        st_stream(&cb.cls[m][r], cls);
      }
#endif
    }
#if NIMBLE_RESULT_STAGED
    if (active) {
      uint64_t *c = lds64 + slot;
#pragma unroll
      for (int m = 0; m < nm; ++m) c[m * ALIGN_BLOCK] = res_v[m];
      c[nm * ALIGN_BLOCK] = res_r;
    }
#endif
    if (any_walk) c_seeded++;
  }
#if NIMBLE_PROFILE_SECTIONS == 1
  if ((tid & 63u) == 0)
    for (int i = 0; i < 10; ++i) atomicAdd(&g_prof[i], prof_acc[i]);
#endif
  if (ln.overflow) atomicOr((unsigned long long *)&cb.state[10], (unsigned long long)ERR_SCRATCH);
  if (want_counters) {
    uint64_t v2 = wave_sum64(ln.probes), v3 = wave_sum64(ln.nodes), v4 = wave_sum64(ln.entries);
    uint64_t v5 = wave_sum64(c_seeded), v6 = wave_sum64(c_pre);
    if ((tid & 63u) == 0) {
      atomicAdd((unsigned long long *)&cb.state[2], (unsigned long long)v2);
      atomicAdd((unsigned long long *)&cb.state[3], (unsigned long long)v3);
      atomicAdd((unsigned long long *)&cb.state[4], (unsigned long long)v4);
      atomicAdd((unsigned long long *)&cb.state[5], (unsigned long long)v5);
      atomicAdd((unsigned long long *)&cb.state[6], (unsigned long long)v6);
    }
  }
}

__device__ void intern_claim_one(const DevIndex &ix, const CallBuffers &cb, int round, uint64_t i, int m) {
  if (cb.cls[m][i] != CLS_PENDING) return;
  const uint64_t h = cb.dyn_hash[m][i];
  const uint32_t tag = intern_tag(h);
  uint64_t pos = round == 0 ? (h & ix.intern_mask) : (((uint64_t)cb.dyn_pos[m][i] + 1) & ix.intern_mask);
  for (;;) {
    uint64_t cur = atomicCAS((unsigned long long *)&ix.intern[pos], 0ULL,
                             ((unsigned long long)tag << 32) | INTERN_PENDING);
    if (cur == 0) {
      const uint32_t len = cb.dyn_len[m][i];
      uint32_t id = atomicAdd(&ix.dyn_state[0], 1u);
      uint32_t off = atomicAdd(&ix.dyn_state[1], len);
      if (id >= ix.cls_cap || (uint64_t)off + len > ix.ids_cap) {
        atomicOr((unsigned long long *)&cb.state[10],
                 (unsigned long long)(id >= ix.cls_cap ? ERR_CLASS_CAP : ERR_IDS_CAP));
        ix.intern[pos] = ((uint64_t)tag << 32) | 0u;
        cb.dyn_pos[m][i] = (uint32_t)pos;
        return;
      }
      const uint32_t *src = cb.scratch + cb.dyn_off[m][i];
      for (uint32_t t = 0; t < len; ++t) ix.cls_ids[off + t] = src[t];
      uint32_t desc[4];
      make_class_desc(src, len, desc);
      ix.cls_off[id] = off;
      ix.cls_desc[id] = make_uint4(desc[0], desc[1], desc[2], desc[3]);
      __threadfence();
      __hip_atomic_store(&ix.intern[pos], ((uint64_t)tag << 32) | id, __ATOMIC_RELAXED, __HIP_MEMORY_SCOPE_AGENT);
      cb.dyn_pos[m][i] = (uint32_t)pos;
      return;
    }
    if ((uint32_t)(cur >> 32) == tag) {
      cb.dyn_pos[m][i] = (uint32_t)pos;
      return;
    }
    pos = (pos + 1) & ix.intern_mask;
  }
}

__global__ void k_intern_claim(DevIndex ix, CallBuffers cb, int round) {
  if (cb.state[8] == 0) return;
  const int m = (int)blockIdx.y;
  for (uint64_t i = (uint64_t)blockIdx.x * blockDim.x + threadIdx.x; i < cb.n; i += (uint64_t)gridDim.x * blockDim.x)
    intern_claim_one(ix, cb, round, i, m);
}

__device__ void intern_verify_one(const DevIndex &ix, const CallBuffers &cb, uint64_t i, int m) {
  if (cb.cls[m][i] != CLS_PENDING) return;
  const uint32_t id = (uint32_t)__hip_atomic_load(&ix.intern[cb.dyn_pos[m][i]], __ATOMIC_RELAXED, __HIP_MEMORY_SCOPE_AGENT);
  if (id == INTERN_PENDING) {
    cb.dyn_pos[m][i] = (uint32_t)(((uint64_t)cb.dyn_pos[m][i] + ix.intern_mask) & ix.intern_mask);
    atomicAdd((unsigned long long *)&cb.state[9], 1ULL);
    return;
  }
  const uint32_t len = cb.dyn_len[m][i];
  uint4 d0 = make_uint4(0, 0, 0, 0);
  if (id < ix.cls_cap) d0 = ix.cls_desc[id];
  bool same = id < ix.cls_cap && desc_len(d0) == len;
  if (same) {
    const uint32_t *a = cb.scratch + cb.dyn_off[m][i];
    const uint32_t *b = ix.cls_ids + ix.cls_off[id];
    for (uint32_t t = 0; t < len; ++t)
      if (a[t] != b[t]) { same = false; break; }
  }
  if (same) cb.cls[m][i] = id;
  else atomicAdd((unsigned long long *)&cb.state[9], 1ULL);
}

__global__ void k_intern_verify(DevIndex ix, CallBuffers cb) {
  if (cb.state[8] == 0) return;
  const int m = (int)blockIdx.y;
  for (uint64_t i = (uint64_t)blockIdx.x * blockDim.x + threadIdx.x; i < cb.n; i += (uint64_t)gridDim.x * blockDim.x)
    intern_verify_one(ix, cb, i, m);
}

__device__ __forceinline__ uint64_t hist_key(const CallBuffers &cb, uint32_t seg, uint32_t c1, uint32_t c2) {
  if (cb.cls_bits == 0) return ((uint64_t)c1 << 32) | c2;
  const uint32_t b = cb.cls_bits;
  return ((uint64_t)seg << (2u * b)) | ((uint64_t)(uint32_t)(c1 + 1u) << b) | (uint64_t)(uint32_t)(c2 + 1u);
}

__device__ __forceinline__ void hist_add_n(const CallBuffers &cb, uint64_t key, uint64_t count, uint32_t read) {
  uint64_t pos = mix64(key) & cb.hist_mask;
  for (uint64_t probes = 0; probes <= cb.hist_mask; ++probes) {
    uint64_t cur = cb.hist_keys[pos];
    if (cur != key)
      cur = atomicCAS((unsigned long long *)&cb.hist_keys[pos], (unsigned long long)HIST_EMPTY, (unsigned long long)key);
    if (cur == HIST_EMPTY || cur == key) {
      atomicAdd((unsigned long long *)&cb.hist_cnt[pos], (unsigned long long)count);
      if (cb.hist_rep) atomicMax(&cb.hist_rep[pos], read);
      return;
    }
    pos = (pos + 1) & cb.hist_mask;
  }
  atomicOr((unsigned long long *)&cb.state[10], (unsigned long long)ERR_HIST);
}

__device__ __forceinline__ void hist_add(const CallBuffers &cb, uint32_t seg, uint32_t c1, uint32_t c2, uint32_t read) {
  hist_add_n(cb, hist_key(cb, seg, c1, c2), 1ULL, read);
}

constexpr uint32_t HCLS_ENTRIES = 64;
struct HotCls {
  uint32_t state, pad;
  uint64_t key;
  unsigned long long count;
};
__device__ __forceinline__ void hist_add_block(const CallBuffers &cb, HotCls *hcls, uint32_t seg, uint32_t c1,
                                               uint32_t c2, uint32_t read) {
  const uint64_t key = hist_key(cb, seg, c1, c2);
  if (hcls) {
    volatile HotCls *e = hcls + (mix64(key) & (uint64_t)(HCLS_ENTRIES - 1));
    uint32_t st = e->state;
    if (st == 0u && atomicCAS((uint32_t *)&e->state, 0u, 1u) == 0u) {
      e->key = key;
      e->count = 1ULL;
      __threadfence_block();
      e->state = 2u;
      return;
    }
    if (st == 2u && e->key == key) {
      atomicAdd((unsigned long long *)&e->count, 1ULL);
      return;
    }
  }
  hist_add_n(cb, key, 1ULL, read);
}

constexpr uint32_t HC_ENTRIES = 64, HC_WORDS = 10;
struct HotEntry {
  uint32_t state, j, pos, total;
  uint64_t h;
  uint32_t seg, pad;
  uint64_t key[HC_WORDS];
};

__device__ __forceinline__ void dedup_one(const nimble_align_params &p, const CallBuffers &cb, uint64_t i,
                                          HotEntry *hc, HotCls *hcls, int mode) {
  uint32_t c1 = cb.cls[0][i];
  uint32_t c2 = cb.paired ? cb.cls[1][i] : CLS_NONE;
  cb.counted[i] = 0;
  if (cb.paired && p.require_valid_pair) {
    if (!(c1 != CLS_NONE && c2 != CLS_NONE && c1 == c2)) {
      cb.reason[0][i] = NIMBLE_R_NOT_MATCHING_PAIR;
      cb.reason[1][i] = NIMBLE_R_NOT_MATCHING_PAIR;
      cb.slot[i] = SLOT_NONE;
      return;
    }
  }
  if (c1 == CLS_NONE && c2 == CLS_NONE) {
    cb.slot[i] = SLOT_NONE;
    return;
  }
  const uint32_t seg = cb.seg ? cb.seg[i] : 0u;
  const uint64_t h0 = rd_hash(cb, i);
  const uint64_t h = cb.seg ? mix64(h0 ^ ((uint64_t)seg * 0x9E3779B97F4A7C15ULL)) : h0;
  const uint32_t tag = (uint32_t)(h >> 32) | 1u;
  const uint64_t mine = ((uint64_t)tag << 32) | (uint32_t)i;
  const uint32_t total = rd_len(cb, 0, i) + (cb.paired ? rd_len(cb, 1, i) : 0u);
  const uint32_t nw = (total + 31u) >> 5;
  uint32_t pos = __umulhi((uint32_t)h, cb.dedup_slots);
  const uint64_t hot_slot = h & (uint64_t)(HOT_KEYS - 1);
  volatile HotEntry *he = hc ? hc + (h & (uint64_t)(HC_ENTRIES - 1)) : nullptr;
  if (he && nw <= HC_WORDS && he->state == 2u && he->h == h && he->total == total && he->seg == seg && he->j > i) {
    uint64_t diff = 0;
    for (uint32_t w = 0; w < nw; ++w) diff |= rd_key(cb, w, i) ^ he->key[w];
    if (diff == 0) {
      cb.slot[i] = he->pos;
      return;
    }
  }
  bool look = mode == 2 && cb.hot[hot_slot] == h;
  for (;;) {
    uint64_t cur;
    if (look) cur = cb.dedup[pos];
    else cur = atomicCAS((unsigned long long *)&cb.dedup[pos], 0ULL, (unsigned long long)mine);
    if (cur == 0) {
      if (look) {
        look = false;
        continue;
      }
      if (cb.fuse_count) hist_add_block(cb, hcls, seg, c1, c2, (uint32_t)i);
      break;
    }
    if ((uint32_t)(cur >> 32) == tag) {
      const uint64_t j = (uint32_t)cur;
      uint64_t diff = (uint64_t)((rd_len(cb, 0, j) + (cb.paired ? rd_len(cb, 1, j) : 0u)) ^ total);
      if (cb.seg) diff |= (uint64_t)(cb.seg[j] ^ seg);
      for (uint32_t w = 0; w < nw; ++w) diff |= rd_key(cb, w, i) ^ rd_key(cb, w, j);
      if (diff == 0) {
        if (mode == 1) {
          const unsigned long long was = atomicExch((unsigned long long *)&cb.hot[hot_slot], (unsigned long long)h);
          if (was == h) atomicAdd((unsigned long long *)&cb.state[13], 1ULL);
          atomicAdd((unsigned long long *)&cb.state[15], 1ULL);
        } else if (mode != 0 && !look) {
          cb.hot[hot_slot] = h;
        }
        if (j < i) atomicMax((unsigned long long *)&cb.dedup[pos], (unsigned long long)mine);
        else if (look && he && nw <= HC_WORDS && atomicCAS((uint32_t *)&he->state, 0u, 1u) == 0u) {
          he->h = h;
          he->total = total;
          he->seg = seg;
          he->j = (uint32_t)j;
          he->pos = pos;
          for (uint32_t w = 0; w < nw; ++w) he->key[w] = rd_key(cb, w, i);
          __threadfence_block();
          he->state = 2u;
        }
        break;
      }
    }
    pos = pos + 1 == cb.dedup_slots ? 0u : pos + 1;
  }
  cb.slot[i] = (uint32_t)pos;
}

__global__ __launch_bounds__(256) void k_dedup(nimble_align_params p, CallBuffers cb, uint64_t g_begin,
                                               uint64_t g_end, int block_counters) {
  __shared__ HotEntry s_hot[HC_ENTRIES];
  for (uint32_t e = threadIdx.x; e < HC_ENTRIES; e += blockDim.x) s_hot[e].state = 0u;
  __syncthreads();
  const uint64_t n = cb.n;
  const bool is_sample = cb.hot && g_begin == 0 && g_end < n;
  const int mode = !cb.hot ? 0 : is_sample ? 1 : (g_begin != 0 && cb.state[13] >= 4 ? 2 : 0);
  HotEntry *hc = mode == 2 ? s_hot : nullptr;
  __shared__ HotCls s_cls[HCLS_ENTRIES];
  HotCls *hcls = (block_counters && cb.fuse_count && !cb.hist_rep && !is_sample) ? s_cls : nullptr;
  for (uint32_t e = threadIdx.x; e < HCLS_ENTRIES; e += blockDim.x) s_cls[e].state = 0u;
  __syncthreads();
  for (uint64_t g = g_begin + (uint64_t)blockIdx.x * blockDim.x + threadIdx.x; g < g_end;
       g += (uint64_t)gridDim.x * blockDim.x)
    dedup_one(p, cb, n - 1 - g, hc, hcls, mode);
  if (hcls) {
    __syncthreads();
    for (uint32_t e = threadIdx.x; e < HCLS_ENTRIES; e += blockDim.x)
      if (s_cls[e].state == 2u) hist_add_n(cb, s_cls[e].key, s_cls[e].count, 0u);
  }
}

__global__ void k_count(CallBuffers cb) {
  const uint64_t i = (uint64_t)blockIdx.x * blockDim.x + threadIdx.x;
  if (i >= cb.n) return;
  const uint32_t s = cb.slot[i];
  if (s == SLOT_NONE) return;
  if ((uint32_t)cb.dedup[s] != (uint32_t)i) return;
  cb.counted[i] = 1;
  if (cb.fuse_count) return;
  hist_add(cb, cb.seg ? cb.seg[i] : 0u, cb.cls[0][i], cb.paired ? cb.cls[1][i] : CLS_NONE, (uint32_t)i);
}

__global__ void k_hist_compact(CallBuffers cb, uint32_t *c1, uint32_t *c2, uint64_t *cnt, uint64_t cap, uint32_t *seg,
                               uint32_t *rep) {
  const uint64_t i = (uint64_t)blockIdx.x * blockDim.x + threadIdx.x;
  if (i > cb.hist_mask) return;
  const uint64_t key = cb.hist_keys[i];
  if (key == HIST_EMPTY) return;
  uint64_t o = atomicAdd((unsigned long long *)&cb.state[11], 1ULL);
  if (o < cap) {
    if (cb.cls_bits == 0) {
      c1[o] = (uint32_t)(key >> 32);
      c2[o] = (uint32_t)key;
      if (seg) seg[o] = 0;
    } else {
      const uint32_t b = cb.cls_bits;
      const uint64_t m = (1ULL << b) - 1ULL;
      c1[o] = (uint32_t)((key >> b) & m) - 1u;
      c2[o] = (uint32_t)(key & m) - 1u;
      if (seg) seg[o] = (uint32_t)(key >> (2u * b));
    }
    cnt[o] = cb.hist_cnt[i];
    if (rep) rep[o] = cb.hist_rep ? cb.hist_rep[i] : 0u;
  }
}

__global__ void k_maxinfo(const uint8_t *__restrict__ qual, const uint64_t *__restrict__ off, uint32_t fixed_len,
                          uint64_t n, const int64_t *__restrict__ length_scores, const int64_t *__restrict__ qual_probs,
                          uint32_t *__restrict__ out) {
  const uint64_t r = (uint64_t)blockIdx.x * blockDim.x + threadIdx.x;
  if (r >= n) return;
  const uint64_t s = off ? off[r] : r * fixed_len;
  const uint32_t len = off ? (uint32_t)(off[r + 1] - s) : fixed_len;
  const uint8_t *q = qual + s;
  int64_t accum = 0;
  double max_score = -1.7976931348623157e308;
  uint32_t pos = 0;
  for (uint32_t i = 0; i < len; ++i) {
    uint32_t c = q[i];
    c = c > 60u ? 60u : c;
    accum += qual_probs[c];
    const int64_t score = (i < 1000u ? length_scores[i] : 0) + accum;
    const double sf = (double)score;
    if (sf >= max_score) {
      max_score = sf;
      pos = i + 1;
    }
  }
  uint32_t t;
  if (pos < 1 || max_score == 0.0) t = 0;
  else t = pos < len ? pos : len;
  out[r] = t;
}

__global__ void k_hist_dense_se(CallBuffers cb, int64_t *counts, uint32_t n_classes) {
  const uint64_t i = (uint64_t)blockIdx.x * blockDim.x + threadIdx.x;
  if (i > cb.hist_mask) return;
  const uint64_t key = cb.hist_keys[i];
  if (key == HIST_EMPTY) return;
  const uint32_t c1 = (uint32_t)(key >> 32), c2 = (uint32_t)key;
  if (c2 == CLS_NONE && c1 < n_classes) counts[c1] = (int64_t)cb.hist_cnt[i];
}

__device__ __forceinline__ uint32_t route_of(uint64_t h, uint32_t world) {
  return (uint32_t)((h & 0x7FFFFFFFFFFFFFFFULL) % world);
}

constexpr uint32_t ROUTE_GRID = 2048;

__global__ void k_route_count(const uint64_t *__restrict__ hash, uint64_t n, uint32_t world, uint32_t *block_counts) {
  __shared__ uint32_t s_c[256];
  if (threadIdx.x < world) s_c[threadIdx.x] = 0;
  __syncthreads();
  const uint32_t lane = threadIdx.x & 63u;
  for (uint64_t tile = blockIdx.x; tile * 256 < n; tile += gridDim.x) {
    const uint64_t i = tile * 256 + threadIdx.x;
    const uint32_t d = i < n ? route_of(hash[i], world) : 0xFFFFFFFFu;
    for (uint32_t t = 0; t < world; ++t) {
      const uint64_t m = __ballot(d == t);
      if (lane == 0 && m) atomicAdd(&s_c[t], (uint32_t)__popcll(m));
    }
  }
  __syncthreads();
  if (threadIdx.x < world) block_counts[(uint64_t)blockIdx.x * world + threadIdx.x] = s_c[threadIdx.x];
}

__global__ void k_route_scan(const uint32_t *__restrict__ block_counts, uint32_t n_blocks, uint32_t world,
                             uint64_t *totals, uint64_t *block_first) {
  __shared__ uint64_t s_part[256];
  __shared__ uint64_t s_start;
  const uint32_t j = threadIdx.x;
  const uint32_t per = (n_blocks + 255u) / 256u;
  if (j == 0) s_start = 0;
  __syncthreads();
  for (uint32_t t = 0; t < world; ++t) {
    uint64_t mine = 0;
    for (uint32_t k = 0; k < per; ++k) {
      const uint32_t b = j * per + k;
      if (b < n_blocks) mine += block_counts[(uint64_t)b * world + t];
    }
    s_part[j] = mine;
    __syncthreads();
    for (uint32_t d = 1; d < 256; d <<= 1) {
      const uint64_t v = j >= d ? s_part[j - d] : 0;
      __syncthreads();
      s_part[j] += v;
      __syncthreads();
    }
    uint64_t run = s_start + s_part[j] - mine;
    for (uint32_t k = 0; k < per; ++k) {
      const uint32_t b = j * per + k;
      if (b < n_blocks) {
        block_first[(uint64_t)b * world + t] = run;
        run += block_counts[(uint64_t)b * world + t];
      }
    }
    __syncthreads();
    if (j == 255) {
      totals[t] = s_part[255];
      s_start += s_part[255];
    }
    __syncthreads();
  }
}

__global__ void k_route_scatter(CallBuffers cb, uint32_t world, const uint64_t *__restrict__ block_first,
                                uint64_t *__restrict__ rec, uint32_t *__restrict__ perm) {
  __shared__ unsigned long long s_cur[256];
  if (threadIdx.x < world) s_cur[threadIdx.x] = block_first[(uint64_t)blockIdx.x * world + threadIdx.x];
  __syncthreads();
  const uint32_t kw = cb.key_words;
  const uint32_t lane = threadIdx.x & 63u;
  for (uint64_t tile = blockIdx.x; tile * 256 < cb.n; tile += gridDim.x) {
    const uint64_t i = tile * 256 + threadIdx.x;
    const bool live = i < cb.n;
    const uint64_t h = live ? cb.key_hash[i] : 0;
    const uint32_t d = live ? route_of(h, world) : 0xFFFFFFFFu;
// ... 98 lines not shown
}


template <bool STAGED>
__global__ void k_dedup_records(const uint64_t *__restrict__ rec, uint64_t n, uint32_t kw, uint64_t *table,
                                uint32_t slots, uint8_t *__restrict__ verdict) {
  extern __shared__ __attribute__((aligned(16))) uint64_t s_rec[];
  const uint32_t rw = kw + 2;
  const uint64_t first_rec = (uint64_t)blockIdx.x * blockDim.x;
  const uint64_t j = first_rec + threadIdx.x;
  const uint64_t *o = rec + j * rw;
  if (STAGED) {
    const uint64_t live = n - first_rec < blockDim.x ? n - first_rec : blockDim.x;
    const uint64_t *src = rec + first_rec * rw;
    for (uint64_t w = threadIdx.x; w < live * rw; w += blockDim.x) s_rec[w] = src[w];
    __syncthreads();
    o = s_rec + (uint64_t)threadIdx.x * rw;
  }
  if (j >= n) return;
  const uint64_t h = o[kw];
  const uint64_t meta = o[kw + 1];
  const uint32_t total = (uint32_t)(meta & 0xFFFF) + (uint32_t)((meta >> 16) & 0xFFFF);
  const uint32_t nw = (total + 31u) >> 5;
  const uint32_t tag = (uint32_t)(h >> 32) | 1u;
  const uint64_t mine = ((uint64_t)tag << 32) | (uint32_t)j;
  uint32_t pos = __umulhi((uint32_t)h, slots);
  uint8_t first = 0;
  bool look = true;
  for (;;) {
    uint64_t cur;
    if (look) cur = table[pos];
    else cur = atomicCAS((unsigned long long *)&table[pos], 0ULL, (unsigned long long)mine);
    if (cur == 0) {
      if (look) {
        look = false;
        continue;
      }
      first = 1;
      break;
    }
    look = true;
    if ((uint32_t)(cur >> 32) == tag) {
      const uint64_t *q = rec + (uint64_t)(uint32_t)cur * rw;
      const uint64_t m2 = q[kw + 1];
      bool same = ((uint32_t)(m2 & 0xFFFF) + (uint32_t)((m2 >> 16) & 0xFFFF)) == total;
      for (uint32_t w = 0; same && w < nw; ++w) same = q[w] == o[w];
      if (same) break;
    }
    pos = pos + 1 == slots ? 0u : pos + 1;
  }
  verdict[j] = first;
}

__global__ void k_count_verdicts(nimble_align_params p, CallBuffers cb, const uint32_t *__restrict__ perm,
                                 const uint8_t *__restrict__ verdict) {
  const uint64_t i = (uint64_t)blockIdx.x * blockDim.x + threadIdx.x;
  if (i >= cb.n) return;
  const uint32_t c1 = cb.cls[0][i];
  const uint32_t c2 = cb.paired ? cb.cls[1][i] : CLS_NONE;
  uint8_t counted = 0;
  bool live = true;
  if (cb.paired && p.require_valid_pair) {
    if (!(c1 != CLS_NONE && c2 != CLS_NONE && c1 == c2)) {
      cb.reason[0][i] = NIMBLE_R_NOT_MATCHING_PAIR;
      cb.reason[1][i] = NIMBLE_R_NOT_MATCHING_PAIR;
      live = false;
    }
  }
  if (live && !(c1 == CLS_NONE && c2 == CLS_NONE) && verdict[perm[i]]) {
    counted = 1;
    hist_add(cb, 0u, c1, c2, (uint32_t)i);
  }
  cb.counted[i] = counted;
}

__global__ void k_clear_call(CallBuffers cb, int clear_latch) {
  const uint64_t i = (uint64_t)blockIdx.x * blockDim.x + threadIdx.x;
  if (i <= cb.hist_mask) {
    cb.hist_keys[i] = HIST_EMPTY;
    cb.hist_cnt[i] = 0;
    if (cb.hist_rep) cb.hist_rep[i] = 0;
  }
  if (i < 16 && (i != 14 || clear_latch)) cb.state[i] = 0;
  if (cb.hot && i < HOT_KEYS) cb.hot[i] = 0;
}

__global__ void k_publish_state(const uint64_t *__restrict__ state, uint64_t *__restrict__ host) {
  if (threadIdx.x < 16) host[threadIdx.x] = state[threadIdx.x];
}

__global__ void k_fill_u64(uint64_t *p, uint64_t v, uint64_t n) {
  uint64_t i = (uint64_t)blockIdx.x * blockDim.x + threadIdx.x;
  const uint64_t stride = (uint64_t)gridDim.x * blockDim.x;
  for (; i < n; i += stride) p[i] = v;
}

inline uint32_t blocks_for(uint64_t n, uint32_t b) { return (uint32_t)((n + b - 1) / b); }

}

int debug_sections(uint64_t out[16], int reset) {
#if NIMBLE_PROFILE_SECTIONS
  unsigned long long h[16];
  if (hipMemcpyFromSymbol(h, HIP_SYMBOL(g_prof), sizeof(h)) != hipSuccess) return -1;
  for (int i = 0; i < 16; ++i) out[i] = h[i];
  if (reset) {
    for (int i = 0; i < 16; ++i) h[i] = 0;
    if (hipMemcpyToSymbol(HIP_SYMBOL(g_prof), h, sizeof(h)) != hipSuccess) return -1;
  }
  return 1;
#else
  (void)out;
  (void)reset;
  return 0;
#endif
}

uint32_t align_ws_lanes() { return (uint32_t)ALIGN_GRID * ALIGN_BLOCK; }
uint32_t align_lds_cols() { return LDS_COLS; }

void launch_pack(hipStream_t s, const uint8_t *r1, const uint64_t *off1, const uint8_t *r2, const uint64_t *off2,
                 uint32_t fixed_len, uint32_t max_len, uint32_t min_len, const double *plog, uint32_t plog_max_len,
                 const CallBuffers &cb) {
  (void)plog_max_len;
  if (cb.n == 0) return;
  const uint32_t budget = 64 * 1024;
  const uint32_t nm = cb.paired ? 2 : 1;
  uint32_t rpb = PACK_BLOCK;
  while (rpb > 1 && (uint64_t)nm * ((uint64_t)rpb * max_len + 48) > budget) rpb >>= 1;
  uint32_t tile_bytes = (uint32_t)((((uint64_t)rpb * max_len + 32) + 15) & ~15ULL);
  uint32_t grid = blocks_for(cb.n, rpb);
  hipLaunchKernelGGL(k_pack, dim3(grid), dim3(PACK_BLOCK), nm * tile_bytes, s, r1, off1, r2, off2, fixed_len, max_len,
                     rpb, tile_bytes, min_len, plog, cb);
}

void launch_pack_words(hipStream_t s, const uint64_t *w1, const uint32_t *len1, uint32_t stride1, const uint64_t *w2,
                       const uint32_t *len2, uint32_t stride2, uint32_t max_len, uint32_t min_len, const double *plog,
                       const CallBuffers &cb) {
  if (cb.n == 0) return;
  hipLaunchKernelGGL(k_pack_words, dim3(blocks_for(cb.n, 256)), dim3(256), 0, s, w1, len1, stride1, w2, len2, stride2, max_len,
                     min_len, plog, cb);
}

static int resident_blocks(const void *fn, size_t lds, int *cus_out) {
  int per_cu = 0, dev = 0, cus = 0;
  (void)hipGetDevice(&dev);
  (void)hipDeviceGetAttribute(&cus, hipDeviceAttributeMultiprocessorCount, dev);
  if (hipOccupancyMaxActiveBlocksPerMultiprocessor(&per_cu, fn, ALIGN_BLOCK, lds) != hipSuccess || per_cu < 1) per_cu = 4;
  if (cus < 1) cus = 256;
  *cus_out = cus;
  return per_cu;
}

static const void *align_kernel(bool paired, bool counters, bool wide, int mode) {
#define NIMBLE_PICK(P, C)                                    \
  (mode == 1 ? (const void *)k_align<P, C, false, 1>          \
             : (wide ? (const void *)k_align<P, C, true, 0> : (const void *)k_align<P, C, false, 0>))
  return paired ? (counters ? NIMBLE_PICK(true, true) : NIMBLE_PICK(true, false))
                : (counters ? NIMBLE_PICK(false, true) : NIMBLE_PICK(false, false));
#undef NIMBLE_PICK
}

static void launch_align_kernel(hipStream_t s, const void *fn, size_t lds, const DevIndex &ix, const nimble_align_params &p,
                                const CallBuffers &cb, uint64_t tiles, int grid_pct, int n_cus, uint64_t want_blocks) {
  int dev = 0;
  (void)hipGetDevice(&dev);
  static std::mutex mu;
  static std::map<std::tuple<int, const void *, size_t>, std::pair<int, int>> resident_cache;
  int resident_blocks_now;
  {
    std::lock_guard<std::mutex> g(mu);
    auto key = std::make_tuple(dev, fn, lds);
    auto it = resident_cache.find(key);
    if (it == resident_cache.end()) {
      if (lds > 48 * 1024) (void)hipFuncSetAttribute(fn, hipFuncAttributeMaxDynamicSharedMemorySize, 160 * 1024);
      int cus = 0;
      const int per_cu = resident_blocks(fn, lds, &cus);
      it = resident_cache.emplace(key, std::make_pair(per_cu, cus)).first;
    }
    const int cus = n_cus > 0 && n_cus < it->second.second ? n_cus : it->second.second;
    resident_blocks_now = it->second.first * cus;
    if (resident_blocks_now > ALIGN_GRID) resident_blocks_now = ALIGN_GRID;
  }
  uint64_t resident = (uint64_t)resident_blocks_now * (uint64_t)(grid_pct < 10 ? 10 : (grid_pct > 100 ? 100 : grid_pct)) / 100;
  if (resident < 1) resident = 1;
  uint64_t grid = tiles < resident ? tiles : resident;
  if (want_blocks && grid > want_blocks) grid = want_blocks;
  void *args[] = {(void *)&ix, (void *)&p, (void *)&cb};
  (void)hipLaunchKernel(fn, dim3((uint32_t)grid), dim3(ALIGN_BLOCK), args, lds, s);
}

static size_t align_lds(const DevIndex &ix, const CallBuffers &cb, bool fast) {
  const bool wide = ix.all_local == 0;
  const uint32_t nm = cb.paired ? 2u : 1u;
  const uint32_t min_rows = nm + 1u;
  const uint32_t krows = cb.key_words + 1 > min_rows ? cb.key_words + 1 : min_rows;
  return (size_t)krows * ALIGN_BLOCK * 8 + (size_t)(fast ? 0 : LDS_COLS) * ALIGN_BLOCK * 4 + ALIGN_LDS_EXTRA + (fast ? ALIGN_LDS_META : 0) +
         (wide ? (size_t)ix.window_words * ALIGN_BLOCK * 8 : 0);
}

void launch_align(hipStream_t s, const DevIndex &ix, const nimble_align_params &p, const CallBuffers &cb,
                  int want_counters, int grid_pct, int n_cus) {
  if (cb.n == 0) return;
  const uint64_t tiles = (cb.n + ALIGN_BLOCK - 1) / ALIGN_BLOCK;
  const bool wide = ix.all_local == 0;
  static const bool fast_on = !(getenv("NIMBLE_FAST_ALIGN") && atoi(getenv("NIMBLE_FAST_ALIGN")) == 0);
  const bool fast = fast_on && !wide && ix.srec && ix.mleft;
  (void)hipMemsetAsync(cb.tile_ctr, 0, (size_t)TILE_COUNTERS * TILE_COUNTER_STRIDE, s);
  launch_align_kernel(s, align_kernel(cb.paired != 0, want_counters != 0, wide, fast ? 1 : 0), align_lds(ix, cb, fast), ix, p, cb, tiles,
                      grid_pct, n_cus, 0);
}

void launch_intern_claim(hipStream_t s, const DevIndex &ix, const CallBuffers &cb, int round) {
  if (cb.n == 0) return;
  const uint32_t full = blocks_for(cb.n, 256);
  hipLaunchKernelGGL(k_intern_claim, dim3(full < 1024u ? full : 1024u, cb.paired ? 2 : 1), dim3(256), 0, s, ix, cb, round);
}
void launch_intern_verify(hipStream_t s, const DevIndex &ix, const CallBuffers &cb) {
  if (cb.n == 0) return;
  const uint32_t full = blocks_for(cb.n, 256);
  hipLaunchKernelGGL(k_intern_verify, dim3(full < 1024u ? full : 1024u, cb.paired ? 2 : 1), dim3(256), 0, s, ix, cb);
}
void launch_dedup(hipStream_t s, const nimble_align_params &p, const CallBuffers &cb, uint32_t grid) {
  if (cb.n == 0) return;
  static const uint64_t min_reads = getenv("NIMBLE_HOT_MIN_READS") ? strtoull(getenv("NIMBLE_HOT_MIN_READS"), nullptr, 10)
                                                                     : (1ull << 18);
  const uint64_t sample = cb.hot && cb.n > min_reads && cb.n >= 8 ? (cb.n / 4 < (1u << 14) ? cb.n / 4 : (1u << 14)) : 0;
  if (sample)
    hipLaunchKernelGGL(k_dedup, dim3(blocks_for(sample, 256)), dim3(256), 0, s, p, cb, (uint64_t)0, sample, 0);
  const uint32_t full = blocks_for(cb.n - sample, 256);
  static const uint32_t persistent = (uint32_t)(getenv("NIMBLE_DEDUP_GRID") ? atoi(getenv("NIMBLE_DEDUP_GRID")) : 4096);
  const uint32_t cap = grid ? grid : persistent;
  static const uint32_t min_tiles = (uint32_t)(getenv("NIMBLE_HCLS_MIN_TILES") ? atoi(getenv("NIMBLE_HCLS_MIN_TILES")) : 4);
  const uint32_t blocks = cap < full ? cap : full;
  hipLaunchKernelGGL(k_dedup, dim3(blocks), dim3(256), 0, s, p, cb, sample, cb.n,
                     (uint64_t)blocks * min_tiles <= (uint64_t)full ? 1 : 0);
}
void launch_count(hipStream_t s, const CallBuffers &cb) {
  if (cb.n == 0) return;
  hipLaunchKernelGGL(k_count, dim3(blocks_for(cb.n, 256)), dim3(256), 0, s, cb);
}
void launch_hist_compact(hipStream_t s, const CallBuffers &cb, uint32_t *c1, uint32_t *c2, uint64_t *cnt,
                         uint64_t cap, uint32_t *seg, uint32_t *rep) {
  hipLaunchKernelGGL(k_hist_compact, dim3(blocks_for(cb.hist_mask + 1, 256)), dim3(256), 0, s, cb, c1, c2, cnt, cap,
                     seg, rep);
}
void launch_maxinfo(hipStream_t s, const uint8_t *qual, const uint64_t *off, uint32_t fixed_len, uint64_t n,
                    const int64_t *length_scores, const int64_t *qual_probs, uint32_t *out) {
  if (n == 0) return;
  hipLaunchKernelGGL(k_maxinfo, dim3(blocks_for(n, 256)), dim3(256), 0, s, qual, off, fixed_len, n, length_scores,
                     qual_probs, out);
}
void launch_hist_dense_se(hipStream_t s, const CallBuffers &cb, int64_t *counts, uint32_t n_classes) {
  hipLaunchKernelGGL(k_hist_dense_se, dim3(blocks_for(cb.hist_mask + 1, 256)), dim3(256), 0, s, cb, counts,
                     n_classes);
}
uint32_t route_grid() { return ROUTE_GRID; }
void launch_route(hipStream_t s, const CallBuffers &cb, uint32_t world, uint32_t *block_counts, uint64_t *block_first,
                  uint64_t *totals, uint64_t *rec, uint32_t *perm) {
  hipLaunchKernelGGL(k_route_count, dim3(ROUTE_GRID), dim3(256), 0, s, cb.key_hash, cb.n, world, block_counts);
  hipLaunchKernelGGL(k_route_scan, dim3(1), dim3(256), 0, s, block_counts, ROUTE_GRID, world, totals, block_first);
  if (cb.n == 0) return;
  const size_t lds = (size_t)256 * (cb.key_words + 2) * 8;
  if (lds <= 56 * 1024)
    hipLaunchKernelGGL(k_route_scatter_lds, dim3(ROUTE_GRID), dim3(256), lds, s, cb, world, block_first, rec, perm);
  else
    hipLaunchKernelGGL(k_route_scatter, dim3(ROUTE_GRID), dim3(256), 0, s, cb, world, block_first, rec, perm);
}
void launch_dedup_records(hipStream_t s, const uint64_t *rec, uint64_t n, uint32_t key_words, uint64_t *table,
                          uint32_t slots, uint8_t *verdict) {
  if (n == 0) return;
  const size_t lds = (size_t)256 * (key_words + 2) * 8;
  if (lds <= 48 * 1024)
    hipLaunchKernelGGL(k_dedup_records<true>, dim3(blocks_for(n, 256)), dim3(256), lds, s, rec, n, key_words, table,
                       slots, verdict);
  else
    hipLaunchKernelGGL(k_dedup_records<false>, dim3(blocks_for(n, 256)), dim3(256), 0, s, rec, n, key_words, table,
                       slots, verdict);
}
void launch_count_verdicts(hipStream_t s, const nimble_align_params &p, const CallBuffers &cb, const uint32_t *perm,
                           const uint8_t *verdict) {
  if (cb.n == 0) return;
  hipLaunchKernelGGL(k_count_verdicts, dim3(blocks_for(cb.n, 256)), dim3(256), 0, s, p, cb, perm, verdict);
}
void launch_records_unpack(hipStream_t s, const uint64_t *rec, const CallBuffers &cb) {
  if (cb.n == 0) return;
  hipLaunchKernelGGL(k_records_unpack, dim3(blocks_for(cb.n, 256)), dim3(256), 0, s, rec, cb);
}
void launch_clear_call(hipStream_t s, const CallBuffers &cb, bool clear_latch) {
  const uint64_t items = cb.hist_mask + 1 > HOT_KEYS ? cb.hist_mask + 1 : HOT_KEYS;
  hipLaunchKernelGGL(k_clear_call, dim3(blocks_for(items, 256)), dim3(256), 0, s, cb, clear_latch ? 1 : 0);
}
void launch_publish_state(hipStream_t s, const uint64_t *state, uint64_t *host) {
  hipLaunchKernelGGL(k_publish_state, dim3(1), dim3(64), 0, s, state, host);
}
void launch_fill_u64(hipStream_t s, uint64_t *p, uint64_t v, uint64_t n) {
  if (n == 0) return;
  uint32_t grid = blocks_for(n, 256);
  if (grid > 4096) grid = 4096;
  hipLaunchKernelGGL(k_fill_u64, dim3(grid), dim3(256), 0, s, p, v, n);
}

}
```

Baseline: 5.358 billion.

## Fuse dedup claims and histogram counting into the single-end align kernel

For eligible single-end calls, the align kernel now elects one representative per key hash within each tile in LDS. It claims that read's dedup hash slot directly and adds its class to a small LDS histogram cache that is flushed at block end, with the dedup probe prefetched in fast mode. The following dedup pass becomes a sweep that handles only reads still marked TODO and counts how many it processed, which is exposed through a new residual-reads API. This is meant to cut most of the separate dedup/count pass over memory, at the cost of extra LDS use, possible occupancy loss and more complex atomics inside the align kernel.

```diff
diff --git a/include/nimble_hip.h b/include/nimble_hip.h
--- a/include/nimble_hip.h
+++ b/include/nimble_hip.h
@@ -145,6 +145,8 @@
 
 int nimble_call_counters(nimble_ctx *, uint64_t c[8]);
 
+int nimble_residual_dedup_reads(nimble_ctx *, uint64_t *reads, int *claimed);
+
 int nimble_call_timing(nimble_ctx *, float ms[6]);
 int nimble_ctx_synchronize(nimble_ctx *);
 
diff --git a/nimble-aligner_amd/__init__.py b/nimble-aligner_amd/__init__.py
--- a/nimble-aligner_amd/__init__.py
+++ b/nimble-aligner_amd/__init__.py
@@ -77,6 +77,7 @@
     "nimble_counts_allreduce", "nimble_counts_allreduce_host", "nimble_records_alltoall", "nimble_sharded_begin",
     "nimble_sharded_append", "nimble_sharded_append_packed", "nimble_sharded_end", "nimble_sharded_grow", "nimble_sharded_abort",
     "nimble_class_table_read", "nimble_class_pool_read", "nimble_steps_begin", "nimble_steps_submit", "nimble_steps_flush", "nimble_steps_end",
+    "nimble_residual_dedup_reads",
 ]
 
 
@@ -109,6 +110,7 @@
         L.nimble_read_records.argtypes = [vp, i32, vp, vp, vp, vp, vp, u64]
         L.nimble_call_counters.argtypes = [vp, C.POINTER(u64)]
         L.nimble_call_timing.argtypes = [vp, C.POINTER(C.c_float)]
+        L.nimble_residual_dedup_reads.argtypes = [vp, C.POINTER(u64), C.POINTER(i32)]
         L.nimble_key_words.argtypes = [u32, i32]
         L.nimble_key_words.restype = u32
         L.nimble_pack.argtypes = [vp, C.POINTER(AlignParams), vp, vp, vp, vp, u64, u32, u32, i32, C.POINTER(NimblePacked)]
@@ -450,6 +452,11 @@
         _check(hip_lib().nimble_call_counters(self.h, c))
         return dict(reads=c[0], unique_keys=c[1], probes=c[2], nodes=c[3], class_entries=c[4], seeded=c[5],
                     prefiltered=c[6], dynamic_classes=c[7])
+
+    def residual_dedup_reads(self):
+        reads, claimed = C.c_uint64(0), C.c_int(0)
+        _check(hip_lib().nimble_residual_dedup_reads(self.h, C.byref(reads), C.byref(claimed)))
+        return int(reads.value) if claimed.value else None
 
     def timing(self):
         t = (C.c_float * 6)()
diff --git a/nimble-aligner_amd/csrc/capi.cpp b/nimble-aligner_amd/csrc/capi.cpp
--- a/nimble-aligner_amd/csrc/capi.cpp
+++ b/nimble-aligner_amd/csrc/capi.cpp
@@ -177,6 +177,8 @@
   bool finished = true;
   bool skip_pack = false;
   bool counted_marked = true;
+  bool from_stream = false;
+  bool claimed = false;
   int attempt = 0;
   std::vector<uint64_t> h_state = std::vector<uint64_t>(16, 0);
   std::vector<uint32_t> h_c1, h_c2;
@@ -403,9 +405,10 @@
   return NIMBLE_OK;
 }
 
-int enqueue_tail(nimble_ctx *c) {
+int enqueue_tail(nimble_ctx *c, bool sweep = false) {
   hipStream_t s = c->stream;
   CallBuffers &cb = c->cb;
+  c->claimed = sweep;
   HIPCHK(hipEventRecord(c->ev[2], s));
   {
     int rc = enqueue_intern_round(c, 0);
@@ -423,7 +426,7 @@
     t = c->copy_stream;
     HIPCHK(hipStreamWaitEvent(t, c->ev[3], 0));
   }
-  launch_dedup(t, c->prm, cb, c->tail_aside ? aside_grid : 0u);
+  launch_dedup(t, c->prm, cb, c->tail_aside ? aside_grid : 0u, sweep);
   HIPCHK(hipEventRecord(c->ev[4], t));
   if (!cb.fuse_count) launch_count(t, cb);
   c->counted_marked = !cb.fuse_count;
@@ -452,8 +455,11 @@
     rc = enqueue_route(c);
     if (rc) return rc;
   }
-  launch_align(s, c->ix->dev, c->prm, cb, c->want_counters, c->align_grid_pct, c->stream_cus);
-  return enqueue_tail(c);
+  static const bool claims_on = env_u64("NIMBLE_ALIGN_CLAIMS", 1) != 0;
+  const bool claim = claims_on && !cb.paired && cb.fuse_count == 1 && !cb.seg && !cb.hist_rep && !cb.skip[0] && !cb.skip[1] &&
+                     !cb.rec && !c->defer.active && !c->streaming && !c->from_stream;
+  const bool claimed = launch_align(s, c->ix->dev, c->prm, cb, c->want_counters, c->align_grid_pct, c->stream_cus, claim);
+  return enqueue_tail(c, claimed);
 }
 
 int redo_dedup_count(nimble_ctx *c) {
@@ -466,6 +472,7 @@
   HIPCHK(hipMemsetAsync((uint64_t *)c->b_state.p + 10, 0, 8, s));
   HIPCHK(hipEventRecord(c->ev[3], s));
   if (c->defer.active) return enqueue_count_verdicts(c);
+  c->claimed = false;
   launch_dedup(s, c->prm, c->cb);
   HIPCHK(hipEventRecord(c->ev[4], s));
   if (!c->cb.fuse_count) launch_count(s, c->cb);
@@ -1126,6 +1133,7 @@
   HIPCHK(hipMemcpyAsync(c->p_dyn, c->ix->b_dyn_state.p, 4 * sizeof(uint32_t), hipMemcpyDeviceToHost, c->stream));
   c->finished = false;
   c->attempt = 0;
+  c->from_stream = false;
   c->defer.active = c->defer.world != 0;
   c->defer.routed = c->defer.counted = false;
   c->defer.verdict = nullptr;
@@ -1575,6 +1583,7 @@
   rc = enqueue_head(c);
   if (rc) return rc;
   c->streaming = true;
+  c->from_stream = true;
   c->finished = true;
   c->called = false;
   return NIMBLE_OK;
@@ -1934,6 +1943,18 @@
   out[1] = uniq;
   for (int i = 2; i <= 6; ++i) out[i] = c->h_state[i];
   out[7] = dst[0] - c->dyn_before;
+  return NIMBLE_OK;
+}
+
+int nimble_residual_dedup_reads(nimble_ctx *c, uint64_t *reads, int *claimed) {
+  DRAIN_STALE_HIP_ERROR();
+  if (!c || !reads || !claimed) return fail(NIMBLE_E_INVALID, "NULL argument");
+  if (!c->called) return fail(NIMBLE_E_INVALID, "nimble_residual_dedup_reads: no call has been made");
+  HIPCHK(hipSetDevice(c->ix->device));
+  int rc = finish_count_stage(c);
+  if (rc) return rc;
+  *claimed = c->claimed ? 1 : 0;
+  *reads = c->claimed ? c->h_state[12] : c->cb.n;
   return NIMBLE_OK;
 }
 
diff --git a/nimble-aligner_amd/csrc/kernels.h b/nimble-aligner_amd/csrc/kernels.h
--- a/nimble-aligner_amd/csrc/kernels.h
+++ b/nimble-aligner_amd/csrc/kernels.h
@@ -10,6 +10,7 @@
 constexpr uint32_t CLS_NONE = 0xFFFFFFFFu;
 constexpr uint32_t CLS_PENDING = 0xFFFFFFFEu;
 constexpr uint32_t SLOT_NONE = 0xFFFFFFFFu;
+constexpr uint32_t SLOT_TODO = 0xFFFFFFFEu;
 constexpr uint32_t HOT_KEYS = 4096;
 constexpr uint64_t HIST_EMPTY = ~0ULL;
 constexpr uint32_t R_TODO = 255;
@@ -98,11 +99,11 @@
 void launch_pack_words(hipStream_t s, const uint64_t *w1, const uint32_t *len1, uint32_t stride1, const uint64_t *w2,
                        const uint32_t *len2, uint32_t stride2, uint32_t max_len, uint32_t min_len, const double *plog,
                        const CallBuffers &cb);
-void launch_align(hipStream_t s, const DevIndex &ix, const nimble_align_params &p, const CallBuffers &cb,
-                  int want_counters, int grid_pct = 100, int n_cus = 0);
+bool launch_align(hipStream_t s, const DevIndex &ix, const nimble_align_params &p, const CallBuffers &cb,
+                  int want_counters, int grid_pct = 100, int n_cus = 0, bool claim = false);
 void launch_intern_claim(hipStream_t s, const DevIndex &ix, const CallBuffers &cb, int round);
 void launch_intern_verify(hipStream_t s, const DevIndex &ix, const CallBuffers &cb);
-void launch_dedup(hipStream_t s, const nimble_align_params &p, const CallBuffers &cb, uint32_t grid = 0);
+void launch_dedup(hipStream_t s, const nimble_align_params &p, const CallBuffers &cb, uint32_t grid = 0, bool sweep = false);
 void launch_count(hipStream_t s, const CallBuffers &cb);
 void launch_hist_compact(hipStream_t s, const CallBuffers &cb, uint32_t *c1, uint32_t *c2, uint64_t *cnt,
                          uint64_t cap, uint32_t *seg = nullptr, uint32_t *rep = nullptr);
diff --git a/nimble-aligner_amd/csrc/kernels.hip b/nimble-aligner_amd/csrc/kernels.hip
--- a/nimble-aligner_amd/csrc/kernels.hip
+++ b/nimble-aligner_amd/csrc/kernels.hip
@@ -1331,7 +1331,54 @@
 #ifndef NIMBLE_RESULT_STAGED
 #define NIMBLE_RESULT_STAGED 1
 #endif
-template <bool PAIRED, bool COUNTERS, bool WIDE, int MODE>
+constexpr uint32_t ELECT_ENTRIES = ALIGN_BLOCK + ALIGN_BLOCK / 8;
+struct AlignCls {
+  uint64_t key;
+  uint32_t state, count;
+};
+constexpr uint32_t align_cls_entries(bool fast) { return fast ? 64u : 16u; }
+constexpr size_t align_claim_lds(bool fast) {
+  return (size_t)ELECT_ENTRIES * 4 + (size_t)align_cls_entries(fast) * sizeof(AlignCls) + (fast ? (size_t)ALIGN_BLOCK * 12 : 0);
+}
+constexpr size_t karg_up(size_t x, size_t a) { return (x + a - 1) / a * a; }
+constexpr size_t ALIGN_KARG_CB =
+    karg_up(karg_up(sizeof(DevIndex), alignof(nimble_align_params)) + sizeof(nimble_align_params), alignof(CallBuffers));
+typedef const __attribute__((address_space(4))) CallBuffers *LateArgs;
+__device__ __forceinline__ LateArgs late_args() {
+  const __attribute__((address_space(4))) char *ka =
+      (const __attribute__((address_space(4))) char *)__builtin_amdgcn_kernarg_segment_ptr();
+  asm volatile("" : "+s"(ka));
+  return (LateArgs)(ka + ALIGN_KARG_CB);
+}
+__device__ __forceinline__ CallBuffers late_hist(LateArgs a) {
+  CallBuffers t{};
+  t.hist_keys = a->hist_keys;
+  t.hist_cnt = a->hist_cnt;
+  t.hist_mask = a->hist_mask;
+  t.hist_rep = nullptr;
+  t.cls_bits = a->cls_bits;
+  t.state = a->state;
+  return t;
+}
+__device__ __forceinline__ uint64_t hist_key(const CallBuffers &cb, uint32_t seg, uint32_t c1, uint32_t c2);
+__device__ __forceinline__ void hist_add_n(const CallBuffers &cb, uint64_t key, uint64_t count, uint32_t read);
+__device__ __forceinline__ void hist_add_lds(const CallBuffers &cb, AlignCls *tab, uint32_t entries, uint64_t key) {
+  volatile AlignCls *e = tab + (mix64(key) & (uint64_t)(entries - 1));
+  const uint32_t st = e->state;
+  if (st == 0u && atomicCAS((uint32_t *)&e->state, 0u, 1u) == 0u) {
+    e->key = key;
+    e->count = 1u;
+    __threadfence_block();
+    e->state = 2u;
+    return;
+  }
+  if (st == 2u && e->key == key) {
+    atomicAdd((uint32_t *)&e->count, 1u);
+    return;
+  }
+  hist_add_n(cb, key, 1ULL, 0u);
+}
+template <bool PAIRED, bool COUNTERS, bool WIDE, int MODE, bool CLAIM>
 #ifndef NIMBLE_FAST_WAVES
 #define NIMBLE_FAST_WAVES 7
 #endif
@@ -1391,6 +1438,17 @@
   uint64_t *s_seed = reinterpret_cast<uint64_t *>(extra + 16 + 64);
   uint16_t *s_perm = reinterpret_cast<uint16_t *>(extra + 16 + 64 + ALIGN_BLOCK * 8);
   uint64_t *s_meta = reinterpret_cast<uint64_t *>(extra + 16 + 64 + ALIGN_BLOCK * 8 + ALIGN_BLOCK * 2);
+  static_assert(!CLAIM || (!PAIRED && NIMBLE_RESULT_STAGED), "claims: single-end launches whose results are staged in LDS");
+  constexpr bool claim = CLAIM;
+  constexpr uint32_t ACLS = align_cls_entries(MODE == 1);
+  constexpr bool PREFETCH = CLAIM && MODE == 1;
+  constexpr uint32_t LOOK_OTHER = 0xFFFFFFFFu;
+  __shared__ uint64_t s_hash[PREFETCH ? ALIGN_BLOCK : 1];
+  __shared__ uint32_t s_look[PREFETCH ? ALIGN_BLOCK : 1];
+  __shared__ uint32_t s_elect[CLAIM ? ELECT_ENTRIES : 1];
+  __shared__ AlignCls s_acls[CLAIM ? ACLS : 1];
+  if (claim)
+    for (uint32_t e = tid; e < ACLS; e += ALIGN_BLOCK) s_acls[e].state = 0u;
   uint64_t prev_tile = ~0ULL;
   const unsigned long long tiles_per_counter = (n_tiles + TILE_COUNTERS - 1) / TILE_COUNTERS;
   unsigned long long &s_next = *reinterpret_cast<unsigned long long *>(extra + 8);
@@ -1436,10 +1494,17 @@
           st_stream(&cb.mism[m][rp], (uint32_t)((v >> 16) & 0xFFFFu));
           st_stream(&cb.cls[m][rp], (uint32_t)(v >> 32));
         }
+        if (claim) {
+          const LateArgs cbl = late_args();
+          st_stream(&cbl->slot[rp], (uint32_t)(rs >> 32));
+          st_stream(&cbl->counted[rp], (uint8_t)0);
+        }
       }
 #endif
     }
 #endif
+    if (claim)
+      for (uint32_t e = tid; e < ELECT_ENTRIES; e += ALIGN_BLOCK) s_elect[e] = 0u;
     if (tid == 0) {
 #ifdef NIMBLE_STATIC_TILES
       s_tile = prev_tile == ~0ULL ? (unsigned long long)blockIdx.x : prev_tile + gridDim.x;
@@ -1485,6 +1550,13 @@
           if (w0 + j < kw) col[(w0 + j) * ALIGN_BLOCK] = w0 + j < nw ? v[j] : 0ULL;
       }
       col[kw * ALIGN_BLOCK] = 0ULL;
+      uint64_t hv = 0;
+      unsigned long long seen = 0;
+      if (PREFETCH && pre0 == R_TODO) {
+        const LateArgs cbl = late_args();
+        hv = cbl->key_hash[r_own];
+        seen = cbl->dedup[__umulhi((uint32_t)hv, cbl->dedup_slots)];
+      }
       if (pre0 == R_TODO && l0 >= KMER) {
         uint32_t nd = 0, of = 0;
         ln.rd = col;
@@ -1494,6 +1566,10 @@
         } else {
           kind = 0;
         }
+      }
+      if (PREFETCH && pre0 == R_TODO) {
+        s_hash[tid] = hv;
+        s_look[tid] = seen == 0 ? 0u : ((uint32_t)(seen >> 32) == ((uint32_t)(hv >> 32) | 1u) ? (uint32_t)seen + 1u : LOOK_OTHER);
       }
     }
     PROF(1)
@@ -1668,12 +1744,85 @@
       }
 #endif
     }
+    uint32_t dslot = SLOT_NONE;
+    if (claim) {
+      const LateArgs cbl = late_args();
+      const uint32_t cls0 = (uint32_t)(res_v[0] >> 32);
+      const bool settled = active && cls0 != CLS_NONE && cls0 != CLS_PENDING;
+      if (active && cls0 != CLS_NONE) dslot = SLOT_TODO;
+      uint64_t h = 0;
+      uint32_t total = 0;
+      if (settled) {
+        if (PREFETCH) {
+          h = s_hash[slot];
+          total = (uint32_t)(s_meta[slot] >> 32) & 0xFFFFu;
+        } else {
+          h = cbl->key_hash[r];
+          total = cbl->len[0][r];
+        }
+      }
+      static_assert(ALIGN_BLOCK <= 512, "the election entries keep the read's index in the tile in 9 bits");
+      const uint32_t etag = (uint32_t)(h >> 41) | 1u;
+      const uint32_t emine = (etag << 9) | slot;
+      uint32_t e = __umulhi((uint32_t)h, ELECT_ENTRIES);
+      if (settled) {
+        for (;;) {
+          const uint32_t cur = atomicCAS(&s_elect[e], 0u, emine);
+          if (cur == 0u) break;
+          if ((cur >> 9) == etag) {
+            atomicMax(&s_elect[e], emine);
+            break;
+          }
+          e = e + 1 == ELECT_ENTRIES ? 0u : e + 1;
+        }
+      }
+      __syncthreads();
+      if (settled && *(volatile uint32_t *)&s_elect[e] == emine) {
+        const uint32_t tag = (uint32_t)(h >> 32) | 1u;
+        const unsigned long long mine = ((unsigned long long)tag << 32) | (uint32_t)r;
+        const uint32_t nw = (total + 31u) >> 5;
+        const uint64_t *own = lds64 + slot;
+        uint32_t pos = __umulhi((uint32_t)h, cbl->dedup_slots);
+        bool look = true;
+        bool parked = PREFETCH;
+        for (;;) {
+          unsigned long long cur;
+          if (parked) {
+            parked = false;
+            const uint32_t lk = s_look[slot];
+            cur = lk == 0u ? 0ULL : (lk == LOOK_OTHER ? (unsigned long long)(tag ^ 2u) << 32 :((unsigned long long)tag << 32) | (lk - 1u));
+          } else if (look) cur = cbl->dedup[pos];
+          else cur = atomicCAS((unsigned long long *)&cbl->dedup[pos], 0ULL, mine);
+          if (cur == 0) {
+            if (look) {
+              look = false;
+              continue;
+            }
+            const CallBuffers ch = late_hist(cbl);
+            hist_add_lds(ch, s_acls, ACLS, hist_key(ch, 0u, cls0, CLS_NONE));
+            break;
+          }
+          if ((uint32_t)(cur >> 32) == tag) {
+            const uint64_t j = (uint32_t)cur;
+            uint64_t diff = (uint64_t)(cbl->len[0][j] ^ total);
+            for (uint32_t w = 0; w < nw; ++w) diff |= own[w * ALIGN_BLOCK] ^ cbl->keys[(uint64_t)w * cbl->key_stride + j];
+            if (diff == 0) {
+              if (j < r) atomicMax((unsigned long long *)&cbl->dedup[pos], mine);
+              break;
+            }
+          }
+          pos = pos + 1 == cbl->dedup_slots ? 0u : pos + 1;
+          look = true;
+        }
+        dslot = pos;
+      }
+    }
 #if NIMBLE_RESULT_STAGED
     if (active) {
       uint64_t *c = lds64 + slot;
 #pragma unroll
       for (int m = 0; m < nm; ++m) c[m * ALIGN_BLOCK] = res_v[m];
-      c[nm * ALIGN_BLOCK] = res_r;
+      c[nm * ALIGN_BLOCK] = claim ? res_r | ((uint64_t)dslot << 32) : res_r;
     }
 #endif
     if (any_walk) c_seeded++;
@@ -1683,6 +1832,9 @@
     for (int i = 0; i < 10; ++i) atomicAdd(&g_prof[i], prof_acc[i]);
 #endif
   if (ln.overflow) atomicOr((unsigned long long *)&cb.state[10], (unsigned long long)ERR_SCRATCH);
+  if (claim)
+    for (uint32_t e = tid; e < ACLS; e += ALIGN_BLOCK)
+      if (s_acls[e].state == 2u) hist_add_n(late_hist(late_args()), s_acls[e].key, (uint64_t)s_acls[e].count, 0u);
   if (want_counters) {
     uint64_t v2 = wave_sum64(ln.probes), v3 = wave_sum64(ln.nodes), v4 = wave_sum64(ln.entries);
     uint64_t v5 = wave_sum64(c_seeded), v6 = wave_sum64(c_pre);
@@ -1912,7 +2064,7 @@
 }
 
 __global__ __launch_bounds__(256) void k_dedup(nimble_align_params p, CallBuffers cb, uint64_t g_begin,
-                                               uint64_t g_end, int block_counters) {
+                                               uint64_t g_end, int block_counters, int sweep) {
   __shared__ HotEntry s_hot[HC_ENTRIES];
   for (uint32_t e = threadIdx.x; e < HC_ENTRIES; e += blockDim.x) s_hot[e].state = 0u;
   __syncthreads();
@@ -1924,9 +2076,19 @@
   HotCls *hcls = (block_counters && cb.fuse_count && !cb.hist_rep && !is_sample) ? s_cls : nullptr;
   for (uint32_t e = threadIdx.x; e < HCLS_ENTRIES; e += blockDim.x) s_cls[e].state = 0u;
   __syncthreads();
+  uint32_t handled = 0;
   for (uint64_t g = g_begin + (uint64_t)blockIdx.x * blockDim.x + threadIdx.x; g < g_end;
-       g += (uint64_t)gridDim.x * blockDim.x)
+       g += (uint64_t)gridDim.x * blockDim.x) {
+    if (sweep) {
+      if (cb.slot[n - 1 - g] != SLOT_TODO) continue;
+      ++handled;
+    }
     dedup_one(p, cb, n - 1 - g, hc, hcls, mode);
+  }
+  if (sweep) {
+    const uint64_t in_wave = wave_sum64(handled);
+    if ((threadIdx.x & 63u) == 0 && in_wave) atomicAdd((unsigned long long *)&cb.state[12], (unsigned long long)in_wave);
+  }
   if (hcls) {
     __syncthreads();
     for (uint32_t e = threadIdx.x; e < HCLS_ENTRIES; e += blockDim.x)
@@ -2331,34 +2493,42 @@
   return per_cu;
 }
 
-static const void *align_kernel(bool paired, bool counters, bool wide, int mode) {
-#define NIMBLE_PICK(P, C)                                    \
-  (mode == 1 ? (const void *)k_align<P, C, false, 1>          \
-             : (wide ? (const void *)k_align<P, C, true, 0> : (const void *)k_align<P, C, false, 0>))
-  return paired ? (counters ? NIMBLE_PICK(true, true) : NIMBLE_PICK(true, false))
-                : (counters ? NIMBLE_PICK(false, true) : NIMBLE_PICK(false, false));
+static const void *align_kernel(bool paired, bool counters, bool wide, int mode, bool claim) {
+#define NIMBLE_PICK(P, C, K)                                    \
+  (mode == 1 ? (const void *)k_align<P, C, false, 1, K>          \
+             : (wide ? (const void *)k_align<P, C, true, 0, K> : (const void *)k_align<P, C, false, 0, K>))
+  if (paired) return counters ? NIMBLE_PICK(true, true, false) : NIMBLE_PICK(true, false, false);
+#if NIMBLE_RESULT_STAGED
+  if (claim) return counters ? NIMBLE_PICK(false, true, true) : NIMBLE_PICK(false, false, true);
+#endif
+  return counters ? NIMBLE_PICK(false, true, false) : NIMBLE_PICK(false, false, false);
 #undef NIMBLE_PICK
 }
 
-static void launch_align_kernel(hipStream_t s, const void *fn, size_t lds, const DevIndex &ix, const nimble_align_params &p,
-                                const CallBuffers &cb, uint64_t tiles, int grid_pct, int n_cus, uint64_t want_blocks) {
+static std::pair<int, int> align_residency(const void *fn, size_t lds) {
   int dev = 0;
   (void)hipGetDevice(&dev);
   static std::mutex mu;
   static std::map<std::tuple<int, const void *, size_t>, std::pair<int, int>> resident_cache;
+  std::lock_guard<std::mutex> g(mu);
+  auto key = std::make_tuple(dev, fn, lds);
+  auto it = resident_cache.find(key);
+  if (it == resident_cache.end()) {
+    if (lds > 48 * 1024) (void)hipFuncSetAttribute(fn, hipFuncAttributeMaxDynamicSharedMemorySize, 160 * 1024);
+    int cus = 0;
+    const int per_cu = resident_blocks(fn, lds, &cus);
+    it = resident_cache.emplace(key, std::make_pair(per_cu, cus)).first;
+  }
+  return it->second;
+}
+
+static void launch_align_kernel(hipStream_t s, const void *fn, size_t lds, const DevIndex &ix, const nimble_align_params &p,
+                                const CallBuffers &cb, uint64_t tiles, int grid_pct, int n_cus, uint64_t want_blocks) {
   int resident_blocks_now;
   {
-    std::lock_guard<std::mutex> g(mu);
-    auto key = std::make_tuple(dev, fn, lds);
-    auto it = resident_cache.find(key);
-    if (it == resident_cache.end()) {
-      if (lds > 48 * 1024) (void)hipFuncSetAttribute(fn, hipFuncAttributeMaxDynamicSharedMemorySize, 160 * 1024);
-      int cus = 0;
-      const int per_cu = resident_blocks(fn, lds, &cus);
-      it = resident_cache.emplace(key, std::make_pair(per_cu, cus)).first;
-    }
-    const int cus = n_cus > 0 && n_cus < it->second.second ? n_cus : it->second.second;
-    resident_blocks_now = it->second.first * cus;
+    const std::pair<int, int> res = align_residency(fn, lds);
+    const int cus = n_cus > 0 && n_cus < res.second ? n_cus : res.second;
+    resident_blocks_now = res.first * cus;
     if (resident_blocks_now > ALIGN_GRID) resident_blocks_now = ALIGN_GRID;
   }
   uint64_t resident = (uint64_t)resident_blocks_now * (uint64_t)(grid_pct < 10 ? 10 : (grid_pct > 100 ? 100 : grid_pct)) / 100;
@@ -2378,16 +2548,27 @@
          (wide ? (size_t)ix.window_words * ALIGN_BLOCK * 8 : 0);
 }
 
-void launch_align(hipStream_t s, const DevIndex &ix, const nimble_align_params &p, const CallBuffers &cb,
-                  int want_counters, int grid_pct, int n_cus) {
-  if (cb.n == 0) return;
+bool launch_align(hipStream_t s, const DevIndex &ix, const nimble_align_params &p, const CallBuffers &cb,
+                  int want_counters, int grid_pct, int n_cus, bool claim) {
+  if (cb.n == 0) return false;
   const uint64_t tiles = (cb.n + ALIGN_BLOCK - 1) / ALIGN_BLOCK;
   const bool wide = ix.all_local == 0;
   static const bool fast_on = !(getenv("NIMBLE_FAST_ALIGN") && atoi(getenv("NIMBLE_FAST_ALIGN")) == 0);
   const bool fast = fast_on && !wide && ix.srec && ix.mleft;
+  const void *fn = align_kernel(cb.paired != 0, want_counters != 0, wide, fast ? 1 : 0, false);
+  const size_t lds = align_lds(ix, cb, fast);
+  bool claims = false;
+  if (claim && NIMBLE_RESULT_STAGED && !cb.paired && cb.fuse_count && !cb.seg && !cb.hist_rep && !cb.skip[0] && !cb.skip[1] && !cb.rec &&
+      lds + align_claim_lds(fast) <= 160 * 1024) {
+    const void *fn_claim = align_kernel(false, want_counters != 0, wide, fast ? 1 : 0, true);
+    if (want_counters || align_residency(fn_claim, lds).first >= align_residency(fn, lds).first) {
+      fn = fn_claim;
+      claims = true;
+    }
+  }
   (void)hipMemsetAsync(cb.tile_ctr, 0, (size_t)TILE_COUNTERS * TILE_COUNTER_STRIDE, s);
-  launch_align_kernel(s, align_kernel(cb.paired != 0, want_counters != 0, wide, fast ? 1 : 0), align_lds(ix, cb, fast), ix, p, cb, tiles,
-                      grid_pct, n_cus, 0);
+  launch_align_kernel(s, fn, lds, ix, p, cb, tiles, grid_pct, n_cus, 0);
+  return claims;
 }
 
 void launch_intern_claim(hipStream_t s, const DevIndex &ix, const CallBuffers &cb, int round) {
@@ -2400,20 +2581,20 @@
   const uint32_t full = blocks_for(cb.n, 256);
   hipLaunchKernelGGL(k_intern_verify, dim3(full < 1024u ? full : 1024u, cb.paired ? 2 : 1), dim3(256), 0, s, ix, cb);
 }
-void launch_dedup(hipStream_t s, const nimble_align_params &p, const CallBuffers &cb, uint32_t grid) {
+void launch_dedup(hipStream_t s, const nimble_align_params &p, const CallBuffers &cb, uint32_t grid, bool sweep) {
   if (cb.n == 0) return;
   static const uint64_t min_reads = getenv("NIMBLE_HOT_MIN_READS") ? strtoull(getenv("NIMBLE_HOT_MIN_READS"), nullptr, 10)
                                                                      : (1ull << 18);
   const uint64_t sample = cb.hot && cb.n > min_reads && cb.n >= 8 ? (cb.n / 4 < (1u << 14) ? cb.n / 4 : (1u << 14)) : 0;
   if (sample)
-    hipLaunchKernelGGL(k_dedup, dim3(blocks_for(sample, 256)), dim3(256), 0, s, p, cb, (uint64_t)0, sample, 0);
+    hipLaunchKernelGGL(k_dedup, dim3(blocks_for(sample, 256)), dim3(256), 0, s, p, cb, (uint64_t)0, sample, 0, sweep ? 1 : 0);
   const uint32_t full = blocks_for(cb.n - sample, 256);
   static const uint32_t persistent = (uint32_t)(getenv("NIMBLE_DEDUP_GRID") ? atoi(getenv("NIMBLE_DEDUP_GRID")) : 4096);
   const uint32_t cap = grid ? grid : persistent;
   static const uint32_t min_tiles = (uint32_t)(getenv("NIMBLE_HCLS_MIN_TILES") ? atoi(getenv("NIMBLE_HCLS_MIN_TILES")) : 4);
   const uint32_t blocks = cap < full ? cap : full;
   hipLaunchKernelGGL(k_dedup, dim3(blocks), dim3(256), 0, s, p, cb, sample, cb.n,
-                     (uint64_t)blocks * min_tiles <= (uint64_t)full ? 1 : 0);
+                     (uint64_t)blocks * min_tiles <= (uint64_t)full ? 1 : 0, sweep ? 1 : 0);
 }
 void launch_count(hipStream_t s, const CallBuffers &cb) {
   if (cb.n == 0) return;
```

After: 4.866 billion. -9.2%, worse.
